# IvanPopov/video-flow-ml

Hardware: AMD Instinct MI355X
Metric: flow-fields/sec @1080p seq5 MOF_sintel (higher is better)
Workload: dtype mixed (per-layer MFMA count, f32 accumulate): {"corr": 1, "update_block.encoder.convf1": 1, "update_block.encoder.convf2": 1, "update_block.gru.convq1.iter": "2a", "update_block.gru.convzr1.iter": 1, "update_block.gru.convzr2.iter": 1, "update_block.mask.0": 1, "update_block.mask.2": 1, "update_bloc

## Files before the change

include/vfml.h:

```cpp
#ifndef VFML_H
#define VFML_H
#include <stddef.h>
#include <stdint.h>

#ifdef __cplusplus
extern "C" {
#endif

#define VFML_ABI_VERSION 27

enum {
  VFML_EPI_NONE = 0,
  VFML_EPI_RELU = 1,
  VFML_EPI_TANH = 2,
  VFML_EPI_SIGMOID = 3,
  VFML_EPI_TANH_RELU = 4,
  VFML_EPI_GRU_ZR = 5,
  VFML_EPI_GRU_Q = 6,
  VFML_EPI_ADD_AUX = 7,
};

enum { VFML_FMT_F32 = 0, VFML_FMT_S16 = 1,
       VFML_FMT_F16 = 2 };

typedef struct vfml_conv_desc {
  const float* in0; int32_t c0; int32_t ld0;
  const float* in1; int32_t c1; int32_t ld1;
  int32_t n, h, w;
  const float* weight;
  const float* bias;
  int32_t cout, kh, kw, stride, pad_h, pad_w;
  float* out; int32_t ldo;
  int32_t epilogue; int32_t split; float out_scale;
  const float* aux0; int32_t ld_aux0;
  const float* aux1; int32_t ld_aux1;
  const float* addend; int32_t ld_addend;
  float* out_t; int32_t ld_out_t;
  int32_t flags;
  double* stats_part;
  float* ksplit_ws;
  const void* proj_hi; const void* proj_lo; int32_t proj_n; int32_t proj_kp; float proj_scale;
  float* proj_out; int32_t ld_proj;
  const float* const* addend_ind;
} vfml_conv_desc;

enum { VFML_STATS_ROWS_F32 = 128, VFML_STATS_ROWS_S16 = 32 };
enum { VFML_CONV_SWAP_CROSS = 1,
       VFML_CONV_MFMA2 = 2, VFML_CONV_MFMA1 = 4, VFML_CONV_MFMA2A = 8,
       VFML_CONV_PER_TAP = 16 };

int vfml_conv2d(const vfml_conv_desc* d, void* stream);

int vfml_conv2d_variant(const vfml_conv_desc* d, char* buf, int len);
int vfml_conv2d_split_variant(const vfml_conv_desc* d, const void* w_hi, const void* w_lo, int kp, float w_scale,
                              int in_fmt, int out_fmt, int aux_fmt, int k_order, char* buf, int len);
int vfml_conv2d_split_variant_at(int index, char* buf, int len);

int vfml_conv2d_split(const vfml_conv_desc* d, const void* w_hi, const void* w_lo, int kp, float w_scale,
                      int in_fmt, int out_fmt, int aux_fmt, int k_order, void* stream);
enum { VFML_KORDER_TAP = 0, VFML_KORDER_CBLOCK = 1, VFML_KORDER_CBLOCK64 = 2 };

int vfml_to_s16(const float* src, int64_t rows, int c, int ld_src, float* dst, int ld_dst, float scale, void* stream);

int vfml_split_f16(const float* src, int64_t rows, int k, int ld, float scale, void* hi, void* lo, int kp,
                   void* stream);

int vfml_softmax_rows_s16(const float* x, int64_t rows, int cols, int64_t ld_in, float* out, int64_t ld_out, float scale,
                          void* stream);

int vfml_softmax_rows_f16(const float* x, int64_t rows, int cols, int64_t ld_in, void* out, int64_t ld_out, float scale,
                          void* stream);

int64_t vfml_attention_plane_workspace_bytes(int p);
int vfml_attention_plane_f16(const float* q, int64_t ld_q, const float* k, int64_t ld_k, int p, int d, float score_scale,
                             float prob_scale, void* plane, int64_t ld_plane, void* workspace, void* stream);

int vfml_attention_bank_planes_f16(const float* q, int64_t ld_q, const float* const* keys, int64_t ld_k, int n_seg, int p, int d,
                                   float score_scale, float prob_scale, void* const* planes, int64_t ld_plane, void* workspace,
                                   void* stream);

int vfml_axpy_f32(const float* x, float* y, int64_t n, float scale, void* stream);

int vfml_transpose_to_s16(const float* src, int rows, int c, int ld, float scale, float* dst, int64_t ld_dst, void* stream);

enum { VFML_DW_RESIDUAL = 1, VFML_DW_GELU = 2 };
int vfml_dwconv2d(const float* x, int64_t ld_x, int n, int h, int w, int c, int k, const float* weight, const float* bias,
                  float* out, int64_t ld_out, int in_fmt, int out_fmt, int flags, void* stream);

int vfml_gelu_rows(const float* x, int64_t ld_x, float* out, int64_t ld_out, int64_t rows, int c, int in_fmt, int out_fmt,
                   void* stream);

int vfml_layernorm_rows(const float* x, int64_t ld_x, float* out, int64_t ld_out, int64_t rows, int c, const float* gamma,
                        const float* beta, float eps, int in_fmt, int out_fmt, void* stream);

int vfml_window_attention(const float* qkv, int64_t ld, int n, int h, int w, int c, int heads, int ws, const float* pad_row,
                          float* out, int64_t ld_out, int in_fmt, int out_fmt, void* stream);

int vfml_attention_shared_keys(const float* q, int64_t ld_q, const float* kv, int64_t ld_kv, int n, int p, int pk, int c, int heads,
                               float* out, int64_t ld_out, int q_fmt, int kv_fmt, int out_fmt, void* stream);

int vfml_add_to_s16(const float* x, int64_t ldx, const float* aux, int64_t ld_aux, float* out, int64_t ld_out, int64_t rows,
                    int c, float scale, void* stream);

int vfml_transpose_split_f16(const float* src, int rows, int c, int ld, float scale, void* hi, void* lo, int kp,
                             void* stream);

int vfml_frames_to_nhwc4(const void* src, int kind, int n, int H, int W,
                         float scale, float shift, float* dst, void* stream);

int64_t vfml_instnorm_workspace_bytes(int n, int hw, int c);
int vfml_instnorm_stats(const float* x, int n, int hw, int c, float eps,
                        float* stats, void* workspace, void* stream);
int vfml_instnorm_apply(const float* x, const float* stats, const float* res,
                        const float* res_stats, int n, int hw, int c, float* out, int out_fmt, void* stream);

int vfml_avgpool2x2(const float* x, int n, int h, int w, int c, float* out, void* stream);

int vfml_corr_lookup(const float* const* pyr, const int32_t* hl, const int32_t* wl,
                     const int32_t* ld, int levels, int radius, int nmaps, int q_per_map,
                     const float* coords, int ld_coords, float* out, int ld_out, int out_fmt, int vol_fmt, int vol_tile,
                     void* stream);
#define VFML_VOL_F16_LEVELS(m) (0x100 | (m))

int vfml_corr_lookup_indirect(const float* const* table, const int32_t* hl, const int32_t* wl, const int32_t* ld,
                              int levels, int radius, int nmaps, int q_per_map, const float* coords, int ld_coords,
                              float* out, int ld_out, int out_fmt, int vol_fmt, int vol_tile, void* stream);
int vfml_corr_lookup_indirect_bidir(const float* const* table, const int32_t* hl, const int32_t* wl, const int32_t* ld,
                                    int levels, int radius, int nmaps, int q_per_map, const float* coords, int ld_coords,
                                    int dir_coords, float* out, int ld_out, int dir_out, int dir_tab, int out_fmt, int vol_fmt,
                                    int vol_tile, void* stream);
int vfml_ptr_table_set(void* table, const void* const* ptrs, int n, void* stream);

int vfml_corr_level0_ensure(const vfml_conv_desc* d, const void* w_hi, const void* w_lo, int kp, float w_scale, int in_fmt,
                            int out_fmt, int k_order, const void* const* cells, int centres, int dirs, int dir_cells,
                            const float* coords, int ld_coords, int dir_coords, int h, int w, int radius, int vol_tile,
                            uint32_t* counter, void* stream);

#define VFML_SEED_NONE 0
#define VFML_SEED_LOAD 1
#define VFML_SEED_STORE 2
int vfml_window_seed(const void* cells, int ncentres, int rows, int cols, float* state, int ld_state, int h_off, int mf_off,
                     int ld_ctx, void* stream);

int vfml_flow_rows7(const float* flow, int n, int h, int w, float* rows, void* stream);

int vfml_conv3x3_c64(const float* in, int ld_in, int n, int h, int w, const void* w_hi, const void* w_lo, int kp, float w_scale,
                     const float* bias, float* out, int ldo, double* stats_part, void* stream);

int vfml_flow_half(const float* flow, int n, int h, int w, const void* w1_hi, int kp1, float w1_scale, const float* b1,
                   const void* w2_hi, int kp2, float w2_scale, const float* b2, float* out, int ld_out, void* stream);

int vfml_tapsum3x3(const float* t, int ld_t, const float* bias, int n, int h, int w, float* out, int parts, int64_t part_stride,
                   void* stream);
int vfml_tapsum3x3_update(const float* t, int ld_t, const float* bias, int n, int h, int w, int parts, int64_t part_stride,
                          float* coords1, float* flow_a, int ld_a, float* flow_b, int ld_b, int fmt_b, void* stream);

int vfml_coords_update(float* coords1, const float* delta, int n, int h, int w,
                       float* flow_a, int ld_a, float* flow_b, int ld_b, int fmt_b, void* stream);

int64_t vfml_flow_forward_interpolate_workspace_bytes(int n, int h, int w);
int vfml_flow_forward_interpolate(const float* flow, int ld_in, int n, int h, int w, float* out, int ld_out, int32_t* index,
                                  void* workspace, int64_t workspace_bytes, void* stream);
int vfml_coords_init(float* coords1, int n, int h, int w, void* stream);

int vfml_convex_upsample(const float* coords1, int ch, const float* mask, int ld_mask,
                         int h, int w, float* out, void* stream);

int64_t vfml_instnorm_finalize_workspace_bytes(int chunks, int c);
int vfml_instnorm_finalize(const double* part, int n, int chunks, int c, int hw, float eps, float* stats,
                           void* workspace, int64_t workspace_bytes, void* stream);

int vfml_stem7x7s2_chunks(int h, int w);
int vfml_stem7x7s2(const float* frames, int n, int h, int w, const void* w_hi, const void* w_lo, float w_scale,
                   const float* bias, float* out, double* stats_part, void* stream);

int vfml_flow_lod(const float* flow, int h, int w, float* out, void* stream);

enum { VFML_ENCODE_GAMEDEV = 0, VFML_ENCODE_RG8 = 1, VFML_ENCODE_RGB8 = 2 };
int vfml_flow_encode(const float* flow, int h, int w, int mode, float width, float height, float scale,
                     float clamp, float two_clamp, unsigned char* out, void* stream);

enum { VFML_TAA_SIMPLE = 0, VFML_TAA_BILINEAR = 1, VFML_TAA_BILATERAL = 2 };
enum { VFML_PIX_U8 = 0, VFML_PIX_F32 = 1, VFML_PIX_F64 = 2 };
int vfml_taa_blend(const void* current, int cur_type, const float* flow, const void* history, int hist_type,
                   void* out, int out_type, int h, int w, int mode, double alpha, double sigma_color, void* stream);

int vfml_flow_quality_map(const unsigned char* frame1, const unsigned char* frame2, const float* flow, int fh, int fw,
                          int h, int w, float threshold, unsigned char* out, void* stream);

#define VFML_CORRECT_RECORD 16
size_t vfml_flow_correct_workspace_bytes(int h, int w);
int vfml_flow_correct(const unsigned char* frame1, const unsigned char* frame2, const float* flow, const float* lod,
                      int lh, int lw, int h, int w, const double* twiddles, double good_threshold,
                      double fine_threshold, double region_radius, double template_radius, double search_radius,
                      float* out_flow, int* counts, double* records, int64_t record_capacity, void* workspace,
                      size_t workspace_bytes, void* stream);

enum { VFML_COLORIZE_HSV = 0, VFML_COLORIZE_WHEEL = 1 };
int vfml_flow_colorize(const float* flow, int h, int w, int mode, void* workspace, unsigned char* out, void* stream);

int vfml_flow_decode(const unsigned char* encoded, int h, int w, int mode, float clamp, float* flow, void* stream);

int vfml_flow_diff_overlay(const float* flow_a, const float* flow_b, int h, int w, unsigned char* out, void* stream);

enum { VFML_COMPOSE_SIDE_BY_SIDE = 0, VFML_COMPOSE_STACKED = 1, VFML_COMPOSE_GRID_2X2 = 2,
       VFML_COMPOSE_GRID_2X3 = 3 };
enum { VFML_COMPOSE_BGR = 1, VFML_COMPOSE_BOTTOM_UP = 2 };
int vfml_compose_frame(const void* const* tiles, const int* tile_types, int h, int w, int layout, int flags,
                       int64_t row_stride, unsigned char* out, void* stream);

int vfml_text_draw(const int32_t* plan, int plan_words, unsigned char* img, int h, int w, int64_t row_stride, int flags,
                   void* stream);

size_t vfml_flow_turbulence_workspace_bytes(int h, int w);
int vfml_flow_turbulence_map(const float* flow, int fh, int fw, int h, int w, int ksize, void* workspace,
                             unsigned char* out_bgr, unsigned char* out_index, float* out_tv, float* out_lohi,
                             void* stream);

int vfml_resize_u8(const unsigned char* src, int n, int H, int W, int64_t src_frame_stride, unsigned char* dst, int h,
                   int w, int64_t dst_frame_stride, const int32_t* xtab, const int32_t* ytab, void* stream);

int64_t vfml_jpeg_workspace_bytes(int h, int w);
int64_t vfml_jpeg_scan_capacity(int h, int w);
int vfml_jpeg_encode_rgb(const unsigned char* rgb, int h, int w, int64_t row_stride, const unsigned char* qtables,
                         void* workspace, unsigned char* scan, int64_t scan_capacity, uint32_t* scan_bytes, void* stream);

enum {
  VFML_JPEG_ERR_INTERVALS = 1,
  VFML_JPEG_ERR_SEQUENCE = 2,
  VFML_JPEG_ERR_CODE = 4,
  VFML_JPEG_ERR_INDEX = 8,
  VFML_JPEG_ERR_DATA = 16
};
int64_t vfml_jpeg_decode_workspace_bytes(int h, int w, int64_t scan_bytes);
int vfml_jpeg_decode_rgb(const unsigned char* scan, int64_t scan_bytes, int h, int w, int restart_interval,
                         const unsigned char* qtables, const int32_t* tables, int y0, int y1, void* workspace,
                         unsigned char* rgb, int64_t row_stride, int32_t* status, void* stream);

int64_t vfml_jpeg_decode_sync_workspace_bytes(int h, int w, int64_t scan_bytes, int subseq_bytes);
int vfml_jpeg_decode_rgb_sync(const unsigned char* scan, int64_t scan_bytes, int h, int w, int restart_interval,
                              const unsigned char* qtables, const int32_t* tables, int y0, int y1, int subseq_bytes,
                              void* workspace, unsigned char* rgb, int64_t row_stride, int32_t* status, void* stream);

enum { VFML_JPEG_420 = 0, VFML_JPEG_422 = 1, VFML_JPEG_444 = 2, VFML_JPEG_GREY = 3 };
int64_t vfml_jpeg_decode_sampled_workspace_bytes(int h, int w, int sampling, int64_t scan_bytes);
int vfml_jpeg_decode_rgb_sampled(const unsigned char* scan, int64_t scan_bytes, int h, int w, int sampling,
                                 int restart_interval, const unsigned char* qtables, const int32_t* tables, int y0, int y1,
                                 void* workspace, unsigned char* rgb, int64_t row_stride, int32_t* status, void* stream);
int64_t vfml_jpeg_decode_sync_sampled_workspace_bytes(int h, int w, int sampling, int64_t scan_bytes, int subseq_bytes);
int vfml_jpeg_decode_rgb_sync_sampled(const unsigned char* scan, int64_t scan_bytes, int h, int w, int sampling,
                                      int restart_interval, const unsigned char* qtables, const int32_t* tables, int y0,
                                      int y1, int subseq_bytes, void* workspace, unsigned char* rgb, int64_t row_stride,
                                      int32_t* status, void* stream);

int64_t vfml_jpeg_sampled_workspace_bytes(int h, int w, int sampling);
int64_t vfml_jpeg_sampled_scan_capacity(int h, int w, int sampling);
int vfml_jpeg_encode_rgb_sampled(const unsigned char* rgb, int h, int w, int64_t row_stride, int sampling,
                                 const unsigned char* qtables, void* workspace, unsigned char* scan,
                                 int64_t scan_capacity, uint32_t* scan_bytes, void* stream);

int64_t vfml_deflate_capacity(int64_t raw_bytes, int chunk_bytes);
int64_t vfml_deflate_workspace_bytes(int64_t raw_bytes, int chunk_bytes);
int vfml_deflate_huffman(const unsigned char* raw, int64_t raw_bytes, int chunk_bytes, uint32_t crc_init, void* workspace,
                         unsigned char* out, int64_t capacity, uint32_t* offsets, uint32_t* stream_bytes, uint32_t* crc,
                         void* stream);

enum {
  VFML_INFLATE_ERR_CODE = 1,
  VFML_INFLATE_ERR_MATCH = 2,
  VFML_INFLATE_ERR_LENGTH = 4,
  VFML_INFLATE_ERR_BITS = 8,
  VFML_INFLATE_ERR_STORED = 16,
  VFML_INFLATE_ERR_CHUNK = 32
};
int64_t vfml_inflate_workspace_bytes(int64_t raw_bytes, int chunk_bytes);
int vfml_inflate_chunks(const unsigned char* data, int64_t data_bytes, const uint32_t* offsets, int n_chunks, int chunk_bytes,
                        int64_t raw_bytes, uint32_t crc_init, void* workspace, unsigned char* raw, uint32_t* crc,
                        int32_t* status, void* stream);

const char* vfml_last_error(void);
int vfml_abi_version(void);

#ifdef __cplusplus
}
#endif
#endif
```

video-flow-ml_amd/vfml/csrc/corr_ensure.hip:

```cpp
#include "gemm_resident_walk.h"
#include "corr_window.h"

namespace {

constexpr int ENSURE_MASK_WORDS = 64;

struct EnsureArgs {
  SplitArgs g;
  const void* const* cells;
  const float* coords;
  unsigned* counter;
  int ld_coords, dir_coords;
  int centres, dirs, dir_cells;
  int q_per_map;
  int h, w, radius, tws, ths;
  int wpr;
};

struct MaskCols {
  unsigned v;
  int nw;
  __device__ __forceinline__ unsigned word(int w) const {
    return (unsigned)__builtin_amdgcn_readlane((int)v, __builtin_amdgcn_readfirstlane(w));
  }
  __device__ __forceinline__ int from(int at) const {
    int w = at >> 5;
    if (w >= nw) return -1;
    unsigned m = word(w) & (~0u << (at & 31));
    while (!m) {
      if (++w >= nw) return -1;
      m = word(w);
    }
    return w * 32 + __builtin_ctz(m);
  }
  __device__ __forceinline__ int first() const { return from(0); }
  __device__ __forceinline__ int next(int nt) const { return from(nt + 1); }
};

__device__ __forceinline__ const void* uniform_cell(const void* const* cell) {
  const uint64_t v = reinterpret_cast<uint64_t>(*cell);
  const unsigned lo = (unsigned)__builtin_amdgcn_readfirstlane((int)(unsigned)v);
  const unsigned hi = (unsigned)__builtin_amdgcn_readfirstlane((int)(unsigned)(v >> 32));
  return reinterpret_cast<const void*>(((uint64_t)hi << 32) | lo);
}

typedef __attribute__((address_space(1))) unsigned* gu32ptr;
typedef const __attribute__((address_space(1))) float* gf32cptr;

__global__ __launch_bounds__(256, 2) void corr_ensure_kernel(const EnsureArgs e) {
  extern __shared__ __attribute__((aligned(16))) char smem[];
  unsigned* mask = reinterpret_cast<unsigned*>(smem);
  const int t = threadIdx.x, lane = t & 63;
  const int mtiles = e.g.mtiles;
  const int units = e.centres * e.dirs * mtiles;
  const int tsh = e.tws + e.ths;
  const int tpr = (e.w + (1 << e.tws) - 1) >> e.tws;
  const int side = 2 * e.radius + 2;
  for (int u = blockIdx.x; u < units; u += gridDim.x) {
    const int k = u / mtiles, mt = u - k * mtiles;
    const int dir = k / e.centres, c = k - dir * e.centres;
    const void* const* cell = e.cells + (dir * e.dir_cells + c) * 4;
    const gu32ptr bitmap = (gu32ptr)uniform_cell(cell + 3) + mt * e.wpr;
    lds_barrier();
    if (t < ENSURE_MASK_WORDS) mask[t] = 0u;
    lds_barrier();
    if (t < 128) {
      const int row = mt * 128 + t;
      const int tile = row >> tsh, in = row & ((1 << tsh) - 1);
      const int ty = tile / tpr, tx = tile - ty * tpr;
      const int y = (ty << e.ths) + (in >> e.tws), x = (tx << e.tws) + (in & ((1 << e.tws) - 1));
      if (row < e.g.M && y < e.h && x < e.w) {
        const gf32cptr cr = (gf32cptr)e.coords + ((int64_t)c * e.q_per_map + y * e.w + x) * e.ld_coords + dir * e.dir_coords;
        const int x0 = window_origin(cr[0], e.radius);
        const int y0 = window_origin(cr[1], e.radius);
        const int xlo = max(x0, 0), xhi = min(x0 + side - 1, e.w - 1);
        const int ylo = max(y0, 0), yhi = min(y0 + side - 1, e.h - 1);
        if (xlo <= xhi && ylo <= yhi) {
          for (int yy = ylo; yy <= yhi; yy = ((yy >> e.ths) + 1) << e.ths)
            for (int xx = xlo; xx <= xhi; xx = ((xx >> e.tws) + 1) << e.tws) {
              const int ct = tiled_at(yy, xx, e.w, e.tws, e.ths) >> 6;
              atomicOr(&mask[ct >> 5], 1u << (ct & 31));
            }
        }
      }
    }
    lds_barrier();
    if (t < e.wpr) mask[t] &= ~bitmap[t];
    lds_barrier();
    const unsigned need = lane < e.wpr ? mask[lane] : 0u;
    const MaskCols cols{need, e.wpr};
    int cnt = 0;
    for (int w = 0; w < e.wpr; ++w) cnt += __builtin_popcount(cols.word(w));
    if (cnt == 0) continue;

    SplitArgs a = e.g;
    a.in0 = a.in1 = reinterpret_cast<const float*>(uniform_cell(cell));
    a.wbase = reinterpret_cast<const char*>(uniform_cell(cell + 1));
    a.out = reinterpret_cast<float*>(const_cast<void*>(uniform_cell(cell + 2)));
    gemm_resident_unit<false, false>(a, smem, mt, cols);

    asm volatile("s_waitcnt vmcnt(0)" ::: "memory");
    lds_barrier();
    if (t < e.wpr && need) atomicOr((unsigned*)bitmap + t, need);
    if (t == 0 && e.counter) atomicAdd(e.counter, (unsigned)cnt);
  }
}

}

extern "C" int vfml_corr_level0_ensure(const vfml_conv_desc* d, const void* w_hi, const void* w_lo, int kp, float w_scale,
                                       int in_fmt, int out_fmt, int k_order, const void* const* cells, int centres, int dirs,
                                       int dir_cells, const float* coords, int ld_coords, int dir_coords, int h, int w,
                                       int radius, int vol_tile, uint32_t* counter, void* stream) {
  const char* who = "vfml_corr_level0_ensure";
  VFML_REQUIRE(d && cells && coords, "%s: null desc / cells / coords", who);
  EnsureArgs e;
  if (const int rc = vfml_detail::prepare_resident_gemm(d, w_hi, w_lo, kp, w_scale, in_fmt, out_fmt, k_order, who, &e.g)) return rc;
  const SplitArgs& a = e.g;
  VFML_REQUIRE(!a.bias && !a.out_t && a.epilogue == VFML_EPI_NONE && a.whi_off == 0 && a.d0off == 0 && a.tilebase,
               "%s: the level-0 call has no bias, twin or activation, its hi plane leads its planes and its rows are one "
               "split-row source", who);
  e.tws = vol_tile & 15;
  e.ths = vol_tile >> 4;
  VFML_REQUIRE(vol_tile >= 0 && e.ths <= 6 && e.tws + e.ths <= 6, "%s: vol_tile: tiles of at most 64 texels", who);
  VFML_REQUIRE(h > 0 && w > 0 && radius >= 1 && radius <= 4, "%s: empty level image, or radius outside 1..4", who);
  const int64_t tiled = (int64_t)(((h - 1) >> e.ths) + 1) * (((w - 1) >> e.tws) + 1) << (e.tws + e.ths);
  VFML_REQUIRE(tiled == a.M && tiled == a.cout, "%s: the call's rows (%d) and columns (%d) must be the %lld positions of the "
               "tiled %d x %d level image", who, a.M, a.cout, (long long)tiled, h, w);
  e.wpr = (a.ntiles + 31) / 32;
  VFML_REQUIRE(e.wpr <= ENSURE_MASK_WORDS, "%s: at most %d column tiles per volume row", who, ENSURE_MASK_WORDS * 32);
  VFML_REQUIRE(centres >= 1 && (dirs == 1 || dirs == 2) && dir_cells >= (dirs == 2 ? centres : 0) && ld_coords >= 2 &&
               dir_coords >= 0, "%s: centres >= 1, one or two directions, the second direction's cells behind the first's", who);
  VFML_REQUIRE((reinterpret_cast<uintptr_t>(cells) & 7u) == 0 && (!counter || (reinterpret_cast<uintptr_t>(counter) & 3u) == 0),
               "%s: cells are 8-byte aligned, the counter 4-byte", who);
  e.cells = cells; e.coords = coords; e.counter = counter;
  e.ld_coords = ld_coords; e.dir_coords = dir_coords;
  e.centres = centres; e.dirs = dirs; e.dir_cells = dir_cells;
  e.q_per_map = h * w; e.h = h; e.w = w; e.radius = radius;
  if (const int rc = vfml_lds_cap(reinterpret_cast<const void*>(&corr_ensure_kernel), VFML_RESIDENT_LDS, who)) return rc;
  const int64_t units = (int64_t)centres * dirs * a.mtiles;
  hipLaunchKernelGGL(corr_ensure_kernel, dim3((int)(units > 512 ? 512 : units)), dim3(256), VFML_RESIDENT_LDS,
                     reinterpret_cast<hipStream_t>(stream), e);
  return vfml_check_launch(who);
}
```

video-flow-ml_amd/vfml/csrc/corr_window.h:

```cpp
#pragma once
#include "vfml_common.h"

namespace {

__device__ __forceinline__ int tiled_at(int y, int x, int w, int tws, int ths) {
  const int tpr = (w + (1 << tws) - 1) >> tws;
  return ((((y >> ths) * tpr + (x >> tws)) << (tws + ths)) + ((y & ((1 << ths) - 1)) << tws) + (x & ((1 << tws) - 1)));
}

__device__ __forceinline__ int window_origin(float c, int radius) {
  return (int)fminf(fmaxf(floorf(c), -65536.f), 65536.f) - radius;
}

}
```

video-flow-ml_amd/vfml/csrc/flow_ops.hip:

```cpp
#include <stdlib.h>
#include "vfml_common.h"
#include "corr_window.h"

namespace {

constexpr int MAX_LEVELS = 6;
constexpr int MAX_MAPS = 8;
constexpr int MAX_RADIUS = 4;
constexpr int PATCH = 2 * MAX_RADIUS + 2;
#ifndef VFML_LOOKUP_WAVES
#define VFML_LOOKUP_WAVES 4
#endif
constexpr int LOOKUP_WAVES = VFML_LOOKUP_WAVES;
constexpr int FIXED_LEVELS = 4;
static_assert(FIXED_LEVELS == 4, "corr_lookup_fixed_kernel selects among four levels");

struct LookupArgs {
  const float* pyr[MAX_MAPS][MAX_LEVELS];
  const float* const* table;
  int hl[MAX_LEVELS], wl[MAX_LEVELS], ld[MAX_LEVELS];
  int levels, radius, nq, q_per_map;
  const float* coords; int ld_coords;
  float* out; int ld_out;
  int out16;
  int vol16;
  int tws, ths;
  int qw;
  int dir_maps, dir_coords, dir_out;
  int dir_tab;
};

__device__ __forceinline__ void lookup_rows(const LookupArgs& a, int q, int& map, int64_t& crow, int64_t& orow) {
  const int dir = a.dir_maps && map >= a.dir_maps;
  const int64_t qd = q - (dir ? a.dir_maps * a.q_per_map : 0);
  if (dir) map += a.dir_tab - a.dir_maps;
  crow = qd * a.ld_coords + (dir ? a.dir_coords : 0);
  orow = qd * a.ld_out + (dir ? a.dir_out : 0);
}


__device__ __forceinline__ float bilinear4(float nw, float ne, float sw, float se, float wx0, float fx, float wy0, float fy) {
  float v = ne * (fx * wy0);
  v = __builtin_fmaf(nw, wx0 * wy0, v);
  v = __builtin_fmaf(sw, wx0 * fy, v);
  v = __builtin_fmaf(se, fx * fy, v);
  return v;
}

__global__ __launch_bounds__(64 * LOOKUP_WAVES) void corr_lookup_kernel(const LookupArgs a) {
  __shared__ float patch[LOOKUP_WAVES][MAX_LEVELS][PATCH * PATCH];
  __shared__ float frac[LOOKUP_WAVES][MAX_LEVELS][2];
  const int lane = threadIdx.x & 63;
  const int wv = threadIdx.x >> 6;
  const int q = blockIdx.x * LOOKUP_WAVES + wv;
  const bool live = q < a.nq;
  int map = live ? q / a.q_per_map : 0;
  const int qq = q - map * a.q_per_map;
  const int side = 2 * a.radius + 2;
  const int win = 2 * a.radius + 1;
  const int psz = side * side;
  int64_t crow = 0, orow = 0;
  if (live) lookup_rows(a, q, map, crow, orow);
  if (live) {
    const float cx = a.coords[crow + 0];
    const float cy = a.coords[crow + 1];
    const int total = a.levels * psz;
    const int qrow = (a.tws | a.ths) ? tiled_at(qq / a.qw, qq % a.qw, a.qw, a.tws, a.ths) : qq;
    for (int e = lane; e < total; e += 64) {
      const int l = e / psz;
      const int idx = e - l * psz;
      const int py = idx / side, px = idx - py * side;
      const float inv = 1.0f / (float)(1 << l);
      const float x = cx * inv, y = cy * inv;
      const float fx0 = floorf(x), fy0 = floorf(y);
      const int x0 = window_origin(x, a.radius);
      const int y0 = window_origin(y, a.radius);
      const int xx = x0 + px, yy = y0 + py;
      float v = 0.f;
      if (xx >= 0 && xx < a.wl[l] && yy >= 0 && yy < a.hl[l])
        v = (a.table ? a.table[map * a.levels + l] : a.pyr[map][l])[(int64_t)qrow * a.ld[l] + tiled_at(yy, xx, a.wl[l], a.tws, a.ths)];
      patch[wv][l][idx] = v;
      if (idx == 0) {
        frac[wv][l][0] = x - fx0;
        frac[wv][l][1] = y - fy0;
      }
    }
  }
  __syncthreads();
  if (!live) return;
  const int nout = a.levels * win * win;
  float* o = a.out + orow;
  const int nwrite = a.out16 ? (nout + 7) & ~7 : nout;
  for (int c = lane; c < nwrite; c += 64) {
    if (c >= nout) {
      _Float16* u = reinterpret_cast<_Float16*>(o + (c & ~7));
      u[c & 7] = (_Float16)0.f;
      u[8 + (c & 7)] = (_Float16)0.f;
      continue;
    }
    const int l = c / (win * win);
    const int rem = c - l * win * win;
    const int i = rem / win, j = rem - i * win;
    const float fx = frac[wv][l][0], fy = frac[wv][l][1];
    const float* p = &patch[wv][l][j * side + i];
    const float wx0 = 1.f - fx, wy0 = 1.f - fy;
    const float v = bilinear4(p[0], p[1], p[side], p[side + 1], wx0, fx, wy0, fy);
    if (a.out16) {
      vfml_h16x2 hh, ll;
      vfml_split2(v, 0.f, hh, ll);
      _Float16* u = reinterpret_cast<_Float16*>(o + (c & ~7));
      u[c & 7] = hh[0];
      u[8 + (c & 7)] = ll[0];
    } else {
      o[c] = v;
    }
  }
}

__device__ __forceinline__ float bilinear4w(float nw, float ne, float sw, float se, float w00, float w10, float w01, float w11) {
  float v = ne * w10;
  v = __builtin_fmaf(nw, w00, v);
  v = __builtin_fmaf(sw, w01, v);
  v = __builtin_fmaf(se, w11, v);
  return v;
}

__device__ __forceinline__ void wave_lds_sync() {
  __builtin_amdgcn_fence(__ATOMIC_RELEASE, "workgroup");
  __builtin_amdgcn_wave_barrier();
  __builtin_amdgcn_fence(__ATOMIC_ACQUIRE, "workgroup");
}

template <int R, bool OUT16, int V16 = 0>
__global__ __launch_bounds__(64 * LOOKUP_WAVES) void corr_lookup_fixed_kernel(const LookupArgs a) {
  constexpr int SIDE = 2 * R + 2, PSZ = SIDE * SIDE, WIN = 2 * R + 1, WW = WIN * WIN;
  constexpr int NOUTPAD = (FIXED_LEVELS * WW + 7) & ~7;
  static_assert(PSZ <= 128 && FIXED_LEVELS * WIN <= 64 && NOUTPAD / 8 <= 64, "one wave: at most two gather passes per level");
  __shared__ float patch[LOOKUP_WAVES][FIXED_LEVELS][PSZ];
  __shared__ __attribute__((aligned(16))) float outs[LOOKUP_WAVES][NOUTPAD];
  const int lane = threadIdx.x & 63;
  const int wv = __builtin_amdgcn_readfirstlane(threadIdx.x >> 6);
  const int q = blockIdx.x * LOOKUP_WAVES + wv;
  if (q >= a.nq) return;
  int map = __builtin_amdgcn_readfirstlane(q / a.q_per_map);
  const int qq = q - map * a.q_per_map;
  const int qrow = __builtin_amdgcn_readfirstlane((a.tws | a.ths) ? tiled_at(qq / a.qw, qq % a.qw, a.qw, a.tws, a.ths) : qq);
  int64_t crow, orow;
  lookup_rows(a, q, map, crow, orow);
  const float cx = a.coords[crow + 0];
  const float cy = a.coords[crow + 1];
  const int pyA = lane / SIDE, pxA = lane - pyA * SIDE;
  const int pyB = (lane + 64) / SIDE, pxB = (lane + 64) - pyB * SIDE;
  const bool inB = lane + 64 < PSZ;
  const float* pl[FIXED_LEVELS];
  if (a.table) {
#pragma unroll
    for (int l = 0; l < FIXED_LEVELS; ++l) pl[l] = a.table[map * a.levels + (l < a.levels ? l : 0)];
  } else {
#pragma unroll
    for (int l = 0; l < FIXED_LEVELS; ++l) pl[l] = a.pyr[map][l < a.levels ? l : 0];
  }
  float va[FIXED_LEVELS], vb[FIXED_LEVELS];
  bool oka[FIXED_LEVELS], okb[FIXED_LEVELS];
#pragma unroll
  for (int l = 0; l < FIXED_LEVELS; ++l) {
    const bool have = l < a.levels;
    const int ll = have ? l : 0;
    const bool v16 = (V16 >> l) & 1;
    const int ES = v16 ? 2 : 4;
    const char* base = reinterpret_cast<const char*>(pl[l]) + (int64_t)qrow * a.ld[ll] * ES;
    const int wl = a.wl[ll], hl = a.hl[ll];
    const float inv = __builtin_bit_cast(float, (127 - l) << 23);
    const float x = cx * inv, y = cy * inv;
    const int x0 = window_origin(x, R);
    const int y0 = window_origin(y, R);
    auto texel = [&](int px, int py, bool in, float& out, bool& ok) {
      const int xx = x0 + px, yy = y0 + py;
      ok = have && in && xx >= 0 && xx < wl && yy >= 0 && yy < hl;
      const int at = tiled_at(min(max(yy, 0), hl - 1), min(max(xx, 0), wl - 1), wl, a.tws, a.ths);
      if (v16) out = (float)((const __attribute__((address_space(1))) _Float16*)base)[at];
      else out = ((const __attribute__((address_space(1))) float*)base)[at];
    };
    texel(pxA, pyA, true, va[l], oka[l]);
    if constexpr (PSZ > 64) texel(pxB, pyB, inB, vb[l], okb[l]);
    else { vb[l] = 0.f; okb[l] = false; }
  }
#pragma unroll
  for (int l = 0; l < FIXED_LEVELS; ++l) {
    va[l] = oka[l] ? va[l] : 0.f;
    vb[l] = okb[l] ? vb[l] : 0.f;
  }
#pragma unroll
  for (int l = 0; l < FIXED_LEVELS; ++l) {
    if (l < a.levels) {
      if (PSZ > 64 || lane < PSZ) patch[wv][l][lane] = va[l];
      if constexpr (PSZ > 64) if (inB) patch[wv][l][lane + 64] = vb[l];
    }
  }
  const int nout = a.levels * WW;
  const int nunits = (nout + 7) >> 3;
  if (lane >= 56 && nout + (lane - 56) < nunits * 8) outs[wv][nout + (lane - 56)] = 0.f;
  wave_lds_sync();
  if (lane < a.levels * WIN) {
    const int l = lane / WIN, i = lane - l * WIN;
    const float inv = __builtin_bit_cast(float, (127 - l) << 23);
    const float x = cx * inv, y = cy * inv;
    const float fx = x - floorf(x), fy = y - floorf(y);
    const float wx0 = 1.f - fx, wy0 = 1.f - fy;
    const float w00 = wx0 * wy0, w10 = fx * wy0, w01 = wx0 * fy, w11 = fx * fy;
    const float* p = &patch[wv][l][i];
    float* o = &outs[wv][l * WW + i * WIN];
    float nw = p[0], ne = p[1];
#pragma unroll
    for (int j = 0; j < WIN; ++j) {
      const float sw = p[(j + 1) * SIDE], se = p[(j + 1) * SIDE + 1];
      o[j] = bilinear4w(nw, ne, sw, se, w00, w10, w01, w11);
      nw = sw; ne = se;
    }
  }
  wave_lds_sync();
  if (lane < nunits) {
    float* o = a.out + orow + lane * 8;
    const f32x4 v0 = *reinterpret_cast<const f32x4*>(&outs[wv][lane * 8]);
    const f32x4 v1 = *reinterpret_cast<const f32x4*>(&outs[wv][lane * 8 + 4]);
    if (OUT16) {
      vfml_h16x2 h0, h1, h2, h3, l0, l1, l2, l3;
      vfml_split2(v0[0], v0[1], h0, l0);
      vfml_split2(v0[2], v0[3], h1, l1);
      vfml_split2(v1[0], v1[1], h2, l2);
      vfml_split2(v1[2], v1[3], h3, l3);
      uint4 hv, lv;
      hv.x = __builtin_bit_cast(unsigned, h0); hv.y = __builtin_bit_cast(unsigned, h1);
      hv.z = __builtin_bit_cast(unsigned, h2); hv.w = __builtin_bit_cast(unsigned, h3);
      lv.x = __builtin_bit_cast(unsigned, l0); lv.y = __builtin_bit_cast(unsigned, l1);
      lv.z = __builtin_bit_cast(unsigned, l2); lv.w = __builtin_bit_cast(unsigned, l3);
      *reinterpret_cast<uint4*>(o) = hv;
      *reinterpret_cast<uint4*>(o + 4) = lv;
    } else {
#pragma unroll
      for (int h = 0; h < 2; ++h) {
        const int c = lane * 8 + 4 * h;
        const f32x4 w = h ? v1 : v0;
        if (c + 3 < nout && (((uintptr_t)(o + 4 * h)) & 15u) == 0) {
          *reinterpret_cast<f32x4*>(o + 4 * h) = w;
        } else {
#pragma unroll
          for (int k = 0; k < 4; ++k)
            if (c + k < nout) o[4 * h + k] = w[k];
        }
      }
    }
  }
}

__global__ void coords_init_kernel(f32x4* __restrict__ coords, int h, int w, int64_t total) {
  for (int64_t p = (int64_t)blockIdx.x * blockDim.x + threadIdx.x; p < total; p += (int64_t)gridDim.x * blockDim.x) {
    const int x = (int)(p % w);
    const int y = (int)((p / w) % h);
    f32x4 v = {(float)x, (float)y, (float)x, (float)y};
    coords[p] = v;
  }
}

__global__ void flow_rows7_kernel(const f32x4* __restrict__ flow, int w, int64_t total, char* __restrict__ rows) {
  for (int64_t i = (int64_t)blockIdx.x * blockDim.x + threadIdx.x; i < total * 4; i += (int64_t)gridDim.x * blockDim.x) {
    const int64_t p = i >> 2;
    const int u = (int)(i & 3);
    const int x = (int)(p % w);
    f32x4 t0 = {0.f, 0.f, 0.f, 0.f}, t1 = {0.f, 0.f, 0.f, 0.f};
    const int x0 = x + 2 * u - 3, x1 = x0 + 1;
    if (x0 >= 0 && x0 < w) t0 = flow[p + 2 * u - 3];
    if (u < 3 && x1 >= 0 && x1 < w) t1 = flow[p + 2 * u - 2];
    vfml_h16x2 h[4], l[4];
    vfml_split2(t0[0], t0[1], h[0], l[0]);
    vfml_split2(t0[2], t0[3], h[1], l[1]);
    vfml_split2(t1[0], t1[1], h[2], l[2]);
    vfml_split2(t1[2], t1[3], h[3], l[3]);
    uint4 hv, lv;
    hv.x = __builtin_bit_cast(unsigned, h[0]); hv.y = __builtin_bit_cast(unsigned, h[1]);
    hv.z = __builtin_bit_cast(unsigned, h[2]); hv.w = __builtin_bit_cast(unsigned, h[3]);
    lv.x = __builtin_bit_cast(unsigned, l[0]); lv.y = __builtin_bit_cast(unsigned, l[1]);
    lv.z = __builtin_bit_cast(unsigned, l[2]); lv.w = __builtin_bit_cast(unsigned, l[3]);
    char* o = rows + p * 128 + u * 32;
    *reinterpret_cast<uint4*>(o) = hv;
    *reinterpret_cast<uint4*>(o + 16) = lv;
  }
}

__device__ __forceinline__ void emit_flow(int64_t p, const f32x4 c, int h, int w, float* __restrict__ fa, int lda,
                                          float* __restrict__ fb, int ldb, int b16) {
  const float x = (float)(int)(p % w);
  const float y = (float)(int)((p / w) % h);
  const f32x4 f = {c[0] - x, c[1] - y, c[2] - x, c[3] - y};
  if (fa) *reinterpret_cast<f32x4*>(fa + p * lda) = f;
  if (fb) {
    if (b16) {
      typedef vfml_h16x2 fp16x2_;
      fp16x2_ h0, h1, l0, l1;
      vfml_split2(f[0], f[1], h0, l0);
      vfml_split2(f[2], f[3], h1, l1);
      char* u = reinterpret_cast<char*>(fb + p * ldb) - 16;
      *reinterpret_cast<fp16x2_*>(u + 8) = h0;
      *reinterpret_cast<fp16x2_*>(u + 12) = h1;
      *reinterpret_cast<fp16x2_*>(u + 24) = l0;
      *reinterpret_cast<fp16x2_*>(u + 28) = l1;
    } else {
      *reinterpret_cast<f32x4*>(fb + p * ldb) = f;
    }
  }
}

__global__ void tapsum3x3_kernel(const float* __restrict__ t, int ld, const float* __restrict__ bias, int h, int w,
                                 int64_t total, f32x4* __restrict__ out, int parts, int64_t part_stride,
                                 f32x4* __restrict__ coords, float* __restrict__ fa, int lda, float* __restrict__ fb, int ldb,
                                 int b16) {
  for (int64_t p = (int64_t)blockIdx.x * blockDim.x + threadIdx.x; p < total; p += (int64_t)gridDim.x * blockDim.x) {
    const int x = (int)(p % w), y = (int)((p / w) % h);
    f32x4 s = {0.f, 0.f, 0.f, 0.f};
    if (bias) s = f32x4{bias[0], bias[1], bias[2], bias[3]};
#pragma unroll
    for (int ky = 0; ky < 3; ++ky)
#pragma unroll
      for (int kx = 0; kx < 3; ++kx) {
        const int yy = y + ky - 1, xx = x + kx - 1;
        if (yy >= 0 && yy < h && xx >= 0 && xx < w) {
          const float* q = t + (p + (int64_t)(ky - 1) * w + (kx - 1)) * ld + (ky * 3 + kx) * 4;
          f32x4 v = *reinterpret_cast<const f32x4*>(q);
          for (int k = 1; k < parts; ++k) v = v + *reinterpret_cast<const f32x4*>(q + k * part_stride);
          s = s + v;
        }
      }
    if (out) out[p] = s;
    if (coords) {
      const f32x4 c = coords[p] + s;
      coords[p] = c;
      emit_flow(p, c, h, w, fa, lda, fb, ldb, b16);
    }
  }
}

__global__ void coords_update_kernel(f32x4* __restrict__ coords, const f32x4* __restrict__ delta, int h, int w,
                                     int64_t total, float* __restrict__ fa, int lda, float* __restrict__ fb, int ldb,
                                     int b16) {
  for (int64_t p = (int64_t)blockIdx.x * blockDim.x + threadIdx.x; p < total; p += (int64_t)gridDim.x * blockDim.x) {
    f32x4 c = coords[p];
    if (delta) {
      c = c + delta[p];
      coords[p] = c;
    }
    emit_flow(p, c, h, w, fa, lda, fb, ldb, b16);
  }
}

__global__ __launch_bounds__(256) void convex_upsample_kernel(const float* __restrict__ coords, int ch,
                                                             const float* __restrict__ mask, int ld_mask, int h,
                                                             int w, float* __restrict__ out) {
  const int lane = threadIdx.x & 63;
  const int p = blockIdx.x * 4 + (threadIdx.x >> 6);
  if (p >= h * w) return;
  const int y = p / w, x = p - y * w;
  const float* m = mask + (int64_t)p * ld_mask + lane;
  float logit[9], fxv[9], fyv[9];
  float mx = -INFINITY;
#pragma unroll
  for (int k = 0; k < 9; ++k) {
    logit[k] = m[k * 64];
    mx = fmaxf(mx, logit[k]);
    const int yy = y + k / 3 - 1, xx = x + k % 3 - 1;
    float u = 0.f, v = 0.f;
    if (yy >= 0 && yy < h && xx >= 0 && xx < w) {
      const float* c = coords + ((int64_t)yy * w + xx) * 4 + ch;
      u = 8.f * (c[0] - (float)xx);
      v = 8.f * (c[1] - (float)yy);
    }
    fxv[k] = u;
    fyv[k] = v;
  }
  float s = 0.f;
#pragma unroll
  for (int k = 0; k < 9; ++k) {
    logit[k] = expf(logit[k] - mx);
    s += logit[k];
  }
  float ax = 0.f, ay = 0.f;
#pragma unroll
  for (int k = 0; k < 9; ++k) {
    const float pk = logit[k] / s;
    ax += pk * fxv[k];
    ay += pk * fyv[k];
  }
  const int sy = lane >> 3, sx = lane & 7;
  float2* o = reinterpret_cast<float2*>(out) + ((int64_t)(8 * y + sy) * (8 * w) + 8 * x + sx);
  *o = make_float2(ax, ay);
}

__global__ void flow_lod_kernel(const float2* __restrict__ flow, int h, int w, int ho, int wo, float2* __restrict__ out) {
  for (int64_t i = (int64_t)blockIdx.x * blockDim.x + threadIdx.x; i < (int64_t)ho * wo;
       i += (int64_t)gridDim.x * blockDim.x) {
    const int oy = (int)(i / wo), ox = (int)(i - (int64_t)oy * wo);
    const int y0 = 2 * oy, x0 = 2 * ox;
    const bool y1 = y0 + 1 < h, x1 = x0 + 1 < w;
    const float2 a = flow[(int64_t)y0 * w + x0];
    const float2 b = x1 ? flow[(int64_t)y0 * w + x0 + 1] : make_float2(0.f, 0.f);
    const float2 c = y1 ? flow[(int64_t)(y0 + 1) * w + x0] : make_float2(0.f, 0.f);
    const float2 d = (y1 && x1) ? flow[(int64_t)(y0 + 1) * w + x0 + 1] : make_float2(0.f, 0.f);
    const float wt = ((1.f + (x1 ? 1.f : 0.f)) + (y1 ? 1.f : 0.f)) + ((y1 && x1) ? 1.f : 0.f);
    const float sx = ((a.x + b.x) + c.x) + d.x, sy = ((a.y + b.y) + c.y) + d.y;
    out[i] = make_float2(sx / wt * 0.5f, sy / wt * 0.5f);
  }
}

inline int grid_for(int64_t items, int block) {
  int64_t g = (items + block - 1) / block;
  return (int)(g < 1 ? 1 : (g > 8192 ? 8192 : g));
}

constexpr int MAX_TABLE = MAX_MAPS * MAX_LEVELS;
struct PtrTable { const void* p[MAX_TABLE]; };
__global__ void ptr_table_kernel(const PtrTable t, int n, const void** dst) {
  if ((int)threadIdx.x < n) dst[threadIdx.x] = t.p[threadIdx.x];
}

__global__ void window_seed_kernel(const int64_t* __restrict__ cells, int rows, int quads, float* __restrict__ state,
                                   int ld_state, int h_off, int mf_off, int ld_ctx) {
  const int c = blockIdx.y;
  const float* ctx = reinterpret_cast<const float*>(cells[3 * c]);
  float* slot = reinterpret_cast<float*>(cells[3 * c + 1]);
  const int64_t mode = slot ? cells[3 * c + 2] : 0;
  const int total = rows * quads;
  for (int i = blockIdx.x * blockDim.x + threadIdx.x; i < total; i += gridDim.x * blockDim.x) {
    const int r = i / quads, k = 4 * (i - r * quads);
    float* srow = state + ((int64_t)c * rows + r) * ld_state;
    if (ctx) *reinterpret_cast<f32x4*>(srow + h_off + k) = *reinterpret_cast<const f32x4*>(ctx + (int64_t)r * ld_ctx + k);
    if (mode == VFML_SEED_LOAD)
      *reinterpret_cast<f32x4*>(srow + mf_off + k) = *reinterpret_cast<const f32x4*>(slot + (int64_t)r * 4 * quads + k);
    else if (mode == VFML_SEED_STORE)
      *reinterpret_cast<f32x4*>(slot + (int64_t)r * 4 * quads + k) = *reinterpret_cast<const f32x4*>(srow + mf_off + k);
  }
}

}

extern "C" int vfml_ptr_table_set(void* table, const void* const* ptrs, int n, void* stream) {
  VFML_REQUIRE(table && ptrs && n >= 1 && n <= MAX_TABLE, "vfml_ptr_table_set: 1..%d pointers", MAX_TABLE);
  PtrTable t;
  for (int i = 0; i < MAX_TABLE; ++i) t.p[i] = i < n ? ptrs[i] : nullptr;
  hipLaunchKernelGGL(ptr_table_kernel, dim3(1), dim3(64), 0, reinterpret_cast<hipStream_t>(stream), t, n,
                     reinterpret_cast<const void**>(table));
  return vfml_check_launch("vfml_ptr_table_set");
}

extern "C" int vfml_window_seed(const void* cells, int ncentres, int rows, int cols, float* state, int ld_state, int h_off,
                                int mf_off, int ld_ctx, void* stream) {
  VFML_REQUIRE(cells && (reinterpret_cast<uintptr_t>(cells) & 7u) == 0, "vfml_window_seed: null / misaligned cells");
  VFML_REQUIRE(ncentres >= 1 && 3 * ncentres <= MAX_TABLE, "vfml_window_seed: ncentres=%d out of [1,%d]", ncentres, MAX_TABLE / 3);
  VFML_REQUIRE(state && vfml_aligned16(state), "vfml_window_seed: null / misaligned state");
  VFML_REQUIRE(rows >= 1 && cols >= 4 && cols % 4 == 0 && (int64_t)rows * (cols / 4) <= (1 << 30),
               "vfml_window_seed: rows >= 1, cols a multiple of 4, rows * cols / 4 <= 2^30");
  VFML_REQUIRE(ld_state % 4 == 0 && h_off >= 0 && mf_off >= 0 && h_off % 4 == 0 && mf_off % 4 == 0 && h_off + cols <= ld_state &&
               mf_off + cols <= ld_state && (h_off + cols <= mf_off || mf_off + cols <= h_off),
               "vfml_window_seed: the two column blocks lie apart inside a state row, at multiples of 4 floats");
  VFML_REQUIRE(ld_ctx >= cols && ld_ctx % 4 == 0, "vfml_window_seed: ld_ctx=%d (>= cols, a multiple of 4)", ld_ctx);
  const int quads = cols / 4;
  hipLaunchKernelGGL(window_seed_kernel, dim3(grid_for((int64_t)rows * quads, 256), ncentres), dim3(256), 0,
                     reinterpret_cast<hipStream_t>(stream), reinterpret_cast<const int64_t*>(cells), rows, quads, state,
                     ld_state, h_off, mf_off, ld_ctx);
  return vfml_check_launch("vfml_window_seed");
}

static int corr_lookup_impl(const float* const* pyr, const float* const* table, const int32_t* hl, const int32_t* wl,
                            const int32_t* ld, int levels, int radius, int nmaps, int q_per_map, const float* coords,
                            int ld_coords, float* out, int ld_out, int out_fmt, int vol_fmt, int vol_tile, void* stream,
                            int dir_maps = 0, int dir_coords = 0, int dir_out = 0, int dir_tab = 0);

extern "C" int vfml_corr_lookup(const float* const* pyr, const int32_t* hl, const int32_t* wl, const int32_t* ld,
                                int levels, int radius, int nmaps, int q_per_map, const float* coords, int ld_coords,
                                float* out, int ld_out, int out_fmt, int vol_fmt, int vol_tile, void* stream) {
  VFML_REQUIRE(pyr, "vfml_corr_lookup: null pointer");
  return corr_lookup_impl(pyr, nullptr, hl, wl, ld, levels, radius, nmaps, q_per_map, coords, ld_coords, out, ld_out, out_fmt,
                          vol_fmt, vol_tile, stream);
}

extern "C" int vfml_corr_lookup_indirect(const float* const* table, const int32_t* hl, const int32_t* wl, const int32_t* ld,
                                         int levels, int radius, int nmaps, int q_per_map, const float* coords,
                                         int ld_coords, float* out, int ld_out, int out_fmt, int vol_fmt, int vol_tile, void* stream) {
  VFML_REQUIRE(table && (reinterpret_cast<uintptr_t>(table) & 7u) == 0, "vfml_corr_lookup_indirect: null / misaligned table");
  return corr_lookup_impl(nullptr, table, hl, wl, ld, levels, radius, nmaps, q_per_map, coords, ld_coords, out, ld_out,
                          out_fmt, vol_fmt, vol_tile, stream);
}

extern "C" int vfml_corr_lookup_indirect_bidir(const float* const* table, const int32_t* hl, const int32_t* wl, const int32_t* ld,
                                               int levels, int radius, int nmaps, int q_per_map, const float* coords,
                                               int ld_coords, int dir_coords, float* out, int ld_out, int dir_out, int dir_tab,
                                               int out_fmt, int vol_fmt, int vol_tile, void* stream) {
  VFML_REQUIRE(table && (reinterpret_cast<uintptr_t>(table) & 7u) == 0, "vfml_corr_lookup_indirect_bidir: null / misaligned table");
  VFML_REQUIRE(nmaps >= 1 && 2 * nmaps <= MAX_MAPS, "vfml_corr_lookup_indirect_bidir: nmaps=%d out of [1,%d]", nmaps, MAX_MAPS / 2);
  VFML_REQUIRE(dir_coords >= 0 && dir_coords + 2 <= ld_coords && dir_out >= 0 && (out_fmt != VFML_FMT_S16 || dir_out % 8 == 0),
               "vfml_corr_lookup_indirect_bidir: dir_coords within a coords row, dir_out >= 0 (a multiple of 8 floats for split rows)");
  VFML_REQUIRE(dir_tab >= nmaps && (dir_tab + nmaps) * levels <= MAX_TABLE,
               "vfml_corr_lookup_indirect_bidir: dir_tab=%d (the second direction's first map in the table) out of range", dir_tab);
  return corr_lookup_impl(nullptr, table, hl, wl, ld, levels, radius, 2 * nmaps, q_per_map, coords, ld_coords, out, ld_out,
                          out_fmt, vol_fmt, vol_tile, stream, nmaps, dir_coords, dir_out, dir_tab);
}

static int corr_lookup_impl(const float* const* pyr, const float* const* table, const int32_t* hl, const int32_t* wl,
                            const int32_t* ld, int levels, int radius, int nmaps, int q_per_map, const float* coords,
                            int ld_coords, float* out, int ld_out, int out_fmt, int vol_fmt, int vol_tile, void* stream,
                            int dir_maps, int dir_coords, int dir_out, int dir_tab) {
  VFML_REQUIRE(nmaps >= 1 && nmaps <= MAX_MAPS && q_per_map > 0, "vfml_corr_lookup: nmaps=%d out of [1,%d] or empty maps", nmaps, MAX_MAPS);
// ... 232 lines not shown
```

video-flow-ml_amd/vfml/hip.py:

```python
import ctypes
import os
import subprocess
from ctypes import POINTER, c_char_p, c_double, c_float, c_int, c_int32, c_int64, c_void_p

import torch

_HERE = os.path.dirname(os.path.abspath(__file__))
LIB_PATH = os.environ.get("VFML_LIB") or os.path.join(_HERE, "libvfml_hip.so")
CSRC = os.path.join(_HERE, "csrc")
SOURCES = ["api.hip", "conv_gemm.hip", "conv_gemm_split.hip", "corr_ensure.hip", "conv_gemm_tapx.hip", "conv_split_plan.hip", "stem.hip", "flow_half.hip", "enc_conv.hip", "norm_pool.hip", "flow_ops.hip", "effects.hip", "correct.hip", "render.hip", "text.hip", "turbulence.hip", "resize.hip", "jpeg.hip", "jpeg_decode.hip", "jpeg_decode_sync.hip", "deflate.hip", "attention.hip", "dwconv.hip", "twins.hip", "warm_start.hip"]

STATS_ROWS_F32, STATS_ROWS_S16 = 128, 32
EPI_NONE, EPI_RELU, EPI_TANH, EPI_SIGMOID, EPI_TANH_RELU, EPI_GRU_ZR, EPI_GRU_Q, EPI_ADD_AUX = range(8)
FMT_F32, FMT_S16, FMT_F16 = 0, 1, 2


def vol_f16_levels(mask):
    return 0x100 | mask


def _vol_mask(vol_fmt, levels):
    return (15 if vol_fmt == FMT_F16 else (vol_fmt & 15 if vol_fmt & 0x100 else 0)) & ((1 << levels) - 1)

KORDER_TAP, KORDER_CBLOCK, KORDER_CBLOCK64 = 0, 1, 2
CONV_SWAP_CROSS, CONV_MFMA2, CONV_MFMA1, CONV_MFMA2A, CONV_PER_TAP = 1, 2, 4, 8, 16


class ConvDesc(ctypes.Structure):
    _fields_ = [
        ("in0", c_void_p), ("c0", c_int32), ("ld0", c_int32),
        ("in1", c_void_p), ("c1", c_int32), ("ld1", c_int32),
        ("n", c_int32), ("h", c_int32), ("w", c_int32),
        ("weight", c_void_p), ("bias", c_void_p),
        ("cout", c_int32), ("kh", c_int32), ("kw", c_int32), ("stride", c_int32),
        ("pad_h", c_int32), ("pad_w", c_int32),
        ("out", c_void_p), ("ldo", c_int32),
        ("epilogue", c_int32), ("split", c_int32), ("out_scale", c_float),
        ("aux0", c_void_p), ("ld_aux0", c_int32),
        ("aux1", c_void_p), ("ld_aux1", c_int32),
        ("addend", c_void_p), ("ld_addend", c_int32),
        ("out_t", c_void_p), ("ld_out_t", c_int32),
        ("flags", c_int32),
        ("stats_part", c_void_p),
        ("ksplit_ws", c_void_p),
        ("proj_hi", c_void_p), ("proj_lo", c_void_p), ("proj_n", c_int32), ("proj_kp", c_int32), ("proj_scale", c_float),
        ("proj_out", c_void_p), ("ld_proj", c_int32),
        ("addend_ind", c_void_p),
    ]


COMMON_FLAGS = ["-fno-slp-vectorize"]
EXTRA_FLAGS = {}


def build(force=False, verbose=False):
    srcs = [os.path.join(CSRC, s) for s in SOURCES]
    hdrs = [os.path.join(CSRC, "vfml_common.h"), os.path.join(CSRC, "conv_split_common.h"),
            os.path.join(CSRC, "gemm_resident_walk.h"), os.path.join(CSRC, "corr_window.h"),
            os.path.join(CSRC, "jet_table.inc"), os.path.join(CSRC, "jpeg_tables.inc"), os.path.join(CSRC, "jpeg_decode_common.h"),
            os.path.join(CSRC, "jpeg_sync_steps.h"), os.path.join(CSRC, "deflate_code.h"), os.path.join(_HERE, "..", "..", "include", "vfml.h")]
    deps = srcs + hdrs
    if not force and os.path.exists(LIB_PATH) and all(
            os.path.getmtime(LIB_PATH) >= os.path.getmtime(d) for d in deps):
        return LIB_PATH
    objdir = os.path.join(CSRC, "_obj")
    os.makedirs(objdir, exist_ok=True)
    newest_hdr = max(os.path.getmtime(h) for h in hdrs)
    jobs = []
    for src in srcs:
        obj = os.path.join(objdir, os.path.basename(src) + ".o")
        if force or not os.path.exists(obj) or os.path.getmtime(obj) < max(os.path.getmtime(src), newest_hdr):
            cmd = ["hipcc", "--offload-arch=gfx950", "-O3", "-std=c++17", "-fPIC"] + COMMON_FLAGS + EXTRA_FLAGS.get(os.path.basename(src), []) + [
                "-c", src, "-o", obj]
            if verbose:
                print(" ".join(cmd))
            jobs.append((cmd, subprocess.Popen(cmd)))
    for cmd, p in jobs:
        if p.wait() != 0:
            raise subprocess.CalledProcessError(p.returncode, cmd)
    cmd = ["hipcc", "--offload-arch=gfx950", "-fPIC", "-shared", "-o", LIB_PATH] + [
        os.path.join(objdir, os.path.basename(src) + ".o") for src in srcs]
    if verbose:
        print(" ".join(cmd))
    subprocess.run(cmd, check=True)
    return LIB_PATH


_lib = None


def lib():
    global _lib
    if _lib is not None:
        return _lib
    if not os.path.exists(LIB_PATH):
        raise RuntimeError(
            f"vfml HIP extension not built: {LIB_PATH} is missing. Run `python -c 'import __graft_entry__ as g; "
            f"g.build()'` (needs hipcc). There is no CPU fallback for the flow engine.")
    L = ctypes.CDLL(LIB_PATH)
    L.vfml_last_error.restype = c_char_p
    L.vfml_abi_version.restype = c_int
    L.vfml_conv2d.argtypes = [POINTER(ConvDesc), c_void_p]
    L.vfml_conv2d_split.argtypes = [POINTER(ConvDesc), c_void_p, c_void_p, c_int, c_float, c_int, c_int, c_int, c_int,
                                    c_void_p]
    L.vfml_conv2d_variant.argtypes = [POINTER(ConvDesc), c_char_p, c_int]
    L.vfml_conv2d_split_variant.argtypes = L.vfml_conv2d_split.argtypes[:-1] + [c_char_p, c_int]
    L.vfml_conv2d_split_variant_at.argtypes = [c_int, c_char_p, c_int]
    L.vfml_to_s16.argtypes = [c_void_p, c_int64, c_int, c_int, c_void_p, c_int, c_float, c_void_p]
    L.vfml_softmax_rows_s16.argtypes = [c_void_p, c_int64, c_int, c_int64, c_void_p, c_int64, c_float, c_void_p]
    L.vfml_transpose_split_f16.argtypes = [c_void_p, c_int, c_int, c_int, c_float, c_void_p, c_void_p, c_int, c_void_p]
    L.vfml_split_f16.argtypes = [c_void_p, c_int64, c_int, c_int, c_float, c_void_p, c_void_p, c_int, c_void_p]
    L.vfml_frames_to_nhwc4.argtypes = [c_void_p, c_int, c_int, c_int, c_int, c_float, c_float, c_void_p, c_void_p]
    L.vfml_instnorm_workspace_bytes.restype = c_int64
    L.vfml_instnorm_workspace_bytes.argtypes = [c_int, c_int, c_int]
    L.vfml_instnorm_stats.argtypes = [c_void_p, c_int, c_int, c_int, c_float, c_void_p, c_void_p, c_void_p]
    L.vfml_softmax_rows_f16.argtypes = [c_void_p, c_int64, c_int, c_int64, c_void_p, c_int64, c_float, c_void_p]
    L.vfml_attention_plane_workspace_bytes.restype = c_int64
    L.vfml_attention_plane_workspace_bytes.argtypes = [c_int]
    L.vfml_attention_plane_f16.argtypes = [c_void_p, c_int64, c_void_p, c_int64, c_int, c_int, c_float, c_float, c_void_p, c_int64,
                                           c_void_p, c_void_p]
    L.vfml_attention_bank_planes_f16.argtypes = [c_void_p, c_int64, POINTER(c_void_p), c_int64, c_int, c_int, c_int, c_float, c_float,
                                                 POINTER(c_void_p), c_int64, c_void_p, c_void_p]
    L.vfml_axpy_f32.argtypes = [c_void_p, c_void_p, c_int64, c_float, c_void_p]
    L.vfml_dwconv2d.argtypes = [c_void_p, c_int64, c_int, c_int, c_int, c_int, c_int, c_void_p, c_void_p, c_void_p, c_int64, c_int, c_int,
                                c_int, c_void_p]
    L.vfml_gelu_rows.argtypes = [c_void_p, c_int64, c_void_p, c_int64, c_int64, c_int, c_int, c_int, c_void_p]
    L.vfml_layernorm_rows.argtypes = [c_void_p, c_int64, c_void_p, c_int64, c_int64, c_int, c_void_p, c_void_p, c_float, c_int, c_int,
                                      c_void_p]
    L.vfml_window_attention.argtypes = [c_void_p, c_int64, c_int, c_int, c_int, c_int, c_int, c_int, c_void_p, c_void_p, c_int64,
                                        c_int, c_int, c_void_p]
    L.vfml_attention_shared_keys.argtypes = [c_void_p, c_int64, c_void_p, c_int64, c_int, c_int, c_int, c_int, c_int, c_void_p,
                                             c_int64, c_int, c_int, c_int, c_void_p]
    L.vfml_transpose_to_s16.argtypes = [c_void_p, c_int, c_int, c_int, c_float, c_void_p, c_int64, c_void_p]
    L.vfml_add_to_s16.argtypes = [c_void_p, c_int64, c_void_p, c_int64, c_void_p, c_int64, c_int64, c_int, c_float, c_void_p]
    L.vfml_instnorm_finalize.argtypes = [c_void_p, c_int, c_int, c_int, c_int, c_float, c_void_p, c_void_p, c_int64, c_void_p]
    L.vfml_instnorm_finalize_workspace_bytes.restype = c_int64
    L.vfml_instnorm_finalize_workspace_bytes.argtypes = [c_int, c_int]
    L.vfml_stem7x7s2_chunks.argtypes = [c_int, c_int]
    L.vfml_stem7x7s2.argtypes = [c_void_p, c_int, c_int, c_int, c_void_p, c_void_p, c_float, c_void_p, c_void_p, c_void_p, c_void_p]
    L.vfml_instnorm_apply.argtypes = [c_void_p, c_void_p, c_void_p, c_void_p, c_int, c_int, c_int, c_void_p, c_int, c_void_p]
    L.vfml_avgpool2x2.argtypes = [c_void_p, c_int, c_int, c_int, c_int, c_void_p, c_void_p]
    L.vfml_corr_lookup.argtypes = [POINTER(c_void_p), POINTER(c_int32), POINTER(c_int32), POINTER(c_int32),
                                   c_int, c_int, c_int, c_int, c_void_p, c_int, c_void_p, c_int, c_int, c_int, c_int, c_void_p]
    L.vfml_corr_lookup_indirect.argtypes = [c_void_p, POINTER(c_int32), POINTER(c_int32), POINTER(c_int32),
                                            c_int, c_int, c_int, c_int, c_void_p, c_int, c_void_p, c_int, c_int, c_int, c_int,
                                            c_void_p]
    L.vfml_corr_lookup_indirect_bidir.argtypes = [c_void_p, POINTER(c_int32), POINTER(c_int32), POINTER(c_int32),
                                                  c_int, c_int, c_int, c_int, c_void_p, c_int, c_int, c_void_p, c_int, c_int,
                                                  c_int, c_int, c_int, c_int, c_void_p]
    L.vfml_ptr_table_set.argtypes = [c_void_p, POINTER(c_void_p), c_int, c_void_p]
    L.vfml_corr_level0_ensure.argtypes = L.vfml_conv2d_split.argtypes[:5] + [c_int, c_int, c_int] + [
        c_void_p, c_int, c_int, c_int, c_void_p, c_int, c_int, c_int, c_int, c_int, c_int, c_void_p, c_void_p]
    L.vfml_window_seed.argtypes = [c_void_p, c_int, c_int, c_int, c_void_p, c_int, c_int, c_int, c_int, c_void_p]
    L.vfml_tapsum3x3_update.argtypes = [c_void_p, c_int, c_void_p, c_int, c_int, c_int, c_int, ctypes.c_int64, c_void_p, c_void_p,
                                        c_int, c_void_p, c_int, c_int, c_void_p]
    L.vfml_conv3x3_c64.argtypes = [c_void_p, c_int, c_int, c_int, c_int, c_void_p, c_void_p, c_int, c_float, c_void_p, c_void_p,
                                   c_int, c_void_p, c_void_p]
    L.vfml_flow_half.argtypes = [c_void_p, c_int, c_int, c_int, c_void_p, c_int, c_float, c_void_p, c_void_p, c_int, c_float,
                                 c_void_p, c_void_p, c_int, c_void_p]
    L.vfml_coords_init.argtypes = [c_void_p, c_int, c_int, c_int, c_void_p]
    L.vfml_flow_rows7.argtypes = [c_void_p, c_int, c_int, c_int, c_void_p, c_void_p]
    L.vfml_tapsum3x3.argtypes = [c_void_p, c_int, c_void_p, c_int, c_int, c_int, c_void_p, c_int, ctypes.c_int64, c_void_p]
    L.vfml_coords_update.argtypes = [c_void_p, c_void_p, c_int, c_int, c_int, c_void_p, c_int, c_void_p, c_int,
                                     c_int, c_void_p]
    L.vfml_flow_forward_interpolate_workspace_bytes.restype = c_int64
    L.vfml_flow_forward_interpolate_workspace_bytes.argtypes = [c_int, c_int, c_int]
    L.vfml_flow_forward_interpolate.argtypes = [c_void_p, c_int, c_int, c_int, c_int, c_void_p, c_int, c_void_p, c_void_p, c_int64,
                                                c_void_p]
    L.vfml_flow_lod.argtypes = [c_void_p, c_int, c_int, c_void_p, c_void_p]
    L.vfml_flow_encode.argtypes = [c_void_p, c_int, c_int, c_int, c_float, c_float, c_float, c_float, c_float, c_void_p,
                                   c_void_p]
    L.vfml_taa_blend.argtypes = [c_void_p, c_int, c_void_p, c_void_p, c_int, c_void_p, c_int, c_int, c_int, c_int, c_double,
                                 c_double, c_void_p]
    L.vfml_flow_quality_map.argtypes = [c_void_p, c_void_p, c_void_p, c_int, c_int, c_int, c_int, c_float, c_void_p, c_void_p]
    L.vfml_flow_correct_workspace_bytes.argtypes = [c_int, c_int]
    L.vfml_flow_correct_workspace_bytes.restype = ctypes.c_size_t
    L.vfml_flow_correct.argtypes = [c_void_p, c_void_p, c_void_p, c_void_p, c_int, c_int, c_int, c_int, c_void_p,
                                    c_double, c_double, c_double, c_double, c_double, c_void_p, c_void_p, c_void_p,
                                    ctypes.c_int64, c_void_p, ctypes.c_size_t, c_void_p]
    L.vfml_flow_colorize.argtypes = [c_void_p, c_int, c_int, c_int, c_void_p, c_void_p, c_void_p]
    L.vfml_flow_decode.argtypes = [c_void_p, c_int, c_int, c_int, c_float, c_void_p, c_void_p]
    L.vfml_flow_diff_overlay.argtypes = [c_void_p, c_void_p, c_int, c_int, c_void_p, c_void_p]
    L.vfml_compose_frame.argtypes = [POINTER(c_void_p), POINTER(c_int32), c_int, c_int, c_int, c_int, c_int64, c_void_p,
                                     c_void_p]
    L.vfml_text_draw.argtypes = [c_void_p, c_int, c_void_p, c_int, c_int, c_int64, c_int, c_void_p]
    L.vfml_flow_turbulence_workspace_bytes.argtypes = [c_int, c_int]
    L.vfml_flow_turbulence_workspace_bytes.restype = ctypes.c_size_t
    L.vfml_flow_turbulence_map.argtypes = [c_void_p, c_int, c_int, c_int, c_int, c_int, c_void_p, c_void_p, c_void_p, c_void_p,
                                           c_void_p, c_void_p]
    L.vfml_resize_u8.argtypes = [c_void_p, c_int, c_int, c_int, c_int64, c_void_p, c_int, c_int, c_int64, c_void_p, c_void_p,
                                 c_void_p]
    L.vfml_jpeg_workspace_bytes.restype = c_int64
    L.vfml_jpeg_workspace_bytes.argtypes = [c_int, c_int]
    L.vfml_jpeg_scan_capacity.restype = c_int64
    L.vfml_jpeg_scan_capacity.argtypes = [c_int, c_int]
    L.vfml_jpeg_encode_rgb.argtypes = [c_void_p, c_int, c_int, c_int64, c_void_p, c_void_p, c_void_p, c_int64, c_void_p,
                                       c_void_p]
    L.vfml_jpeg_sampled_workspace_bytes.restype = c_int64
    L.vfml_jpeg_sampled_workspace_bytes.argtypes = [c_int, c_int, c_int]
    L.vfml_jpeg_sampled_scan_capacity.restype = c_int64
    L.vfml_jpeg_sampled_scan_capacity.argtypes = [c_int, c_int, c_int]
    L.vfml_jpeg_encode_rgb_sampled.argtypes = [c_void_p, c_int, c_int, c_int64, c_int, c_void_p, c_void_p, c_void_p, c_int64,
                                               c_void_p, c_void_p]
    L.vfml_jpeg_decode_workspace_bytes.restype = c_int64
    L.vfml_jpeg_decode_workspace_bytes.argtypes = [c_int, c_int, c_int64]
    L.vfml_jpeg_decode_rgb.argtypes = [c_void_p, c_int64, c_int, c_int, c_int, c_void_p, c_void_p, c_int, c_int, c_void_p,
                                       c_void_p, c_int64, c_void_p, c_void_p]
    L.vfml_jpeg_decode_sync_workspace_bytes.restype = c_int64
    L.vfml_jpeg_decode_sync_workspace_bytes.argtypes = [c_int, c_int, c_int64, c_int]
    L.vfml_jpeg_decode_rgb_sync.argtypes = [c_void_p, c_int64, c_int, c_int, c_int, c_void_p, c_void_p, c_int, c_int, c_int,
                                            c_void_p, c_void_p, c_int64, c_void_p, c_void_p]
    L.vfml_jpeg_decode_sampled_workspace_bytes.restype = c_int64
    L.vfml_jpeg_decode_sampled_workspace_bytes.argtypes = [c_int, c_int, c_int, c_int64]
    L.vfml_jpeg_decode_rgb_sampled.argtypes = [c_void_p, c_int64, c_int, c_int, c_int, c_int, c_void_p, c_void_p, c_int, c_int,
                                               c_void_p, c_void_p, c_int64, c_void_p, c_void_p]
    L.vfml_jpeg_decode_sync_sampled_workspace_bytes.restype = c_int64
    L.vfml_jpeg_decode_sync_sampled_workspace_bytes.argtypes = [c_int, c_int, c_int, c_int64, c_int]
    L.vfml_jpeg_decode_rgb_sync_sampled.argtypes = [c_void_p, c_int64, c_int, c_int, c_int, c_int, c_void_p, c_void_p, c_int,
                                                    c_int, c_int, c_void_p, c_void_p, c_int64, c_void_p, c_void_p]
    for fn in (L.vfml_deflate_capacity, L.vfml_deflate_workspace_bytes, L.vfml_inflate_workspace_bytes):
        fn.restype = c_int64
        fn.argtypes = [c_int64, c_int]
    L.vfml_deflate_huffman.argtypes = [c_void_p, c_int64, c_int, ctypes.c_uint32, c_void_p, c_void_p, c_int64, c_void_p, c_void_p,
                                       c_void_p, c_void_p]
    L.vfml_inflate_chunks.argtypes = [c_void_p, c_int64, c_void_p, c_int, c_int, c_int64, ctypes.c_uint32, c_void_p, c_void_p,
                                      c_void_p, c_void_p, c_void_p]
    L.vfml_convex_upsample.argtypes = [c_void_p, c_int, c_void_p, c_int, c_int, c_int, c_void_p, c_void_p]
    for name in EXPORTS:
        getattr(L, name)
    if L.vfml_abi_version() != 27:
        raise RuntimeError("libvfml_hip.so ABI version mismatch")
    _lib = L
    return L


EXPORTS = [
    "vfml_conv2d", "vfml_conv2d_split", "vfml_conv2d_variant", "vfml_conv2d_split_variant", "vfml_conv2d_split_variant_at", "vfml_split_f16", "vfml_to_s16", "vfml_softmax_rows_s16", "vfml_softmax_rows_f16", "vfml_attention_plane_workspace_bytes", "vfml_attention_plane_f16", "vfml_attention_bank_planes_f16", "vfml_axpy_f32", "vfml_dwconv2d", "vfml_gelu_rows", "vfml_layernorm_rows", "vfml_window_attention", "vfml_attention_shared_keys", "vfml_transpose_to_s16", "vfml_add_to_s16",
    "vfml_transpose_split_f16", "vfml_frames_to_nhwc4", "vfml_instnorm_workspace_bytes", "vfml_instnorm_stats",
    "vfml_instnorm_apply", "vfml_instnorm_finalize", "vfml_instnorm_finalize_workspace_bytes", "vfml_avgpool2x2", "vfml_corr_lookup", "vfml_corr_lookup_indirect", "vfml_corr_lookup_indirect_bidir",
    "vfml_ptr_table_set", "vfml_corr_level0_ensure", "vfml_window_seed", "vfml_coords_update", "vfml_coords_init", "vfml_tapsum3x3", "vfml_tapsum3x3_update", "vfml_flow_rows7", "vfml_flow_half", "vfml_conv3x3_c64",
    "vfml_flow_forward_interpolate_workspace_bytes", "vfml_flow_forward_interpolate",
    "vfml_convex_upsample", "vfml_stem7x7s2", "vfml_stem7x7s2_chunks", "vfml_flow_lod", "vfml_flow_encode", "vfml_taa_blend", "vfml_flow_quality_map", "vfml_flow_correct_workspace_bytes", "vfml_flow_correct",
    "vfml_flow_colorize", "vfml_compose_frame", "vfml_flow_decode", "vfml_flow_diff_overlay", "vfml_text_draw",
    "vfml_flow_turbulence_workspace_bytes", "vfml_flow_turbulence_map", "vfml_resize_u8",
    "vfml_jpeg_workspace_bytes", "vfml_jpeg_scan_capacity", "vfml_jpeg_encode_rgb",
    "vfml_jpeg_sampled_workspace_bytes", "vfml_jpeg_sampled_scan_capacity", "vfml_jpeg_encode_rgb_sampled",
    "vfml_jpeg_decode_workspace_bytes", "vfml_jpeg_decode_rgb",
    "vfml_jpeg_decode_sync_workspace_bytes", "vfml_jpeg_decode_rgb_sync",
    "vfml_jpeg_decode_sampled_workspace_bytes", "vfml_jpeg_decode_rgb_sampled",
    "vfml_jpeg_decode_sync_sampled_workspace_bytes", "vfml_jpeg_decode_rgb_sync_sampled",
    "vfml_deflate_capacity", "vfml_deflate_workspace_bytes", "vfml_deflate_huffman",
    "vfml_inflate_workspace_bytes", "vfml_inflate_chunks",
    "vfml_last_error", "vfml_abi_version",
]


def _check(rc, what):
    if rc != 0:
        raise RuntimeError(f"{what} failed (rc={rc}): {lib().vfml_last_error().decode()}")


def _stream():
    return c_void_p(torch.cuda.current_stream().cuda_stream)


def _ptr(t, offset=0):
    if t is None:
        return None
    return c_void_p(t.data_ptr() + 4 * offset)


def _dev(t, dtype=torch.float32):
    if not (t.is_cuda and t.dtype == dtype and t.is_contiguous()):
        raise ValueError(f"expected a contiguous {dtype} device tensor, got {t.dtype} {t.device} "
                         f"contiguous={t.is_contiguous()}")
    return t


_PROFILE = None


_PROFILE_HBM = None


def profile_begin():
    global _PROFILE, _PROFILE_HBM
    _PROFILE = []
    _PROFILE_HBM = []


def profile_end_hbm():
    rec = _PROFILE_HBM or []
    torch.cuda.synchronize()
    out = {}
    for name, nbytes, e0, e1 in rec:
        d = out.setdefault(name, {"launches": 0, "bytes": 0.0, "ms": 0.0})
        d["launches"] += 1
        d["bytes"] += nbytes
        d["ms"] += e0.elapsed_time(e1)
    return out


def profile_end():
    global _PROFILE, _PROFILE_HBM
    rec, _PROFILE = _PROFILE or [], None
    _PROFILE_HBM = None
    torch.cuda.synchronize()
    out = {}
    for variant, flops, nbytes, e0, e1, shape in rec:
        d = out.setdefault(variant, {"launches": 0, "flops": 0.0, "bytes": 0.0, "ms": 0.0, "shapes": {}})
        ms = e0.elapsed_time(e1)
        for t in (d, d["shapes"].setdefault(shape, {"launches": 0, "flops": 0.0, "bytes": 0.0, "ms": 0.0})):
            t["launches"] += 1
            t["flops"] += flops
            t["bytes"] += nbytes
            t["ms"] += ms
    return out


class SplitWeight:

    def __init__(self, rows, k, device):
        self.rows, self.k, self.kp = rows, k, (k + 31) // 32 * 32
        self.scale = 1.0
        self.order = KORDER_TAP
        self.planes = torch.empty(2 * rows * self.kp, dtype=torch.float16, device=device)
        self.hi, self.lo = self.planes[:rows * self.kp], self.planes[rows * self.kp:]

    @staticmethod
    def auto_scale(absmax):
        import math
        if not (absmax > 0.0) or not math.isfinite(absmax):
            return 1.0
        return 2.0 ** math.floor(math.log2(16384.0 / absmax))

    def fill_transposed(self, src, rows_src, ld=None, scale=1.0, src_off=0):
        self.scale = float(scale)
        _check(lib().vfml_transpose_split_f16(_ptr(_dev(src), src_off), rows_src, self.rows, ld or self.rows,
                                              self.scale, c_void_p(self.hi.data_ptr()), c_void_p(self.lo.data_ptr()),
                                              self.kp, _stream()), "vfml_transpose_split_f16")
        return self

    def fill(self, src, src_off=0, ld=None, scale=1.0):
        self.scale = float(scale)
        _check(lib().vfml_split_f16(_ptr(_dev(src), src_off), self.rows, self.k, ld or self.k, self.scale,
                                    c_void_p(self.hi.data_ptr()), c_void_p(self.lo.data_ptr()), self.kp, _stream()),
               "vfml_split_f16")
        return self


def conv2d(in0, c0, ld0, n, h, w, weight, bias, cout, kh, kw, out, ldo, *, stride=1, pad_h=0, pad_w=0,
           in0_off=0, weight_off=0, in1=None, c1=0, ld1=0, in1_off=0, out_off=0, epilogue=EPI_NONE, split=0, out_scale=1.0,
           aux0=None, ld_aux0=0, aux0_off=0, aux1=None, ld_aux1=0, aux1_off=0,
           in_fmt=FMT_F32, out_fmt=FMT_F32, aux_fmt=FMT_F32, addend=None, ld_addend=0, addend_off=0,
           out_t=None, ld_out_t=0, out_t_off=0, swap_cross=False, stats_part=None, mfma=3, per_tap=False, ksplit_ws=None,
           proj=None, proj_out=None, ld_proj=0, addend_ind=None, variant_only=False):
    d = ConvDesc()
    d.in0, d.c0, d.ld0 = _ptr(_dev(in0), in0_off), c0, ld0
    d.in1, d.c1, d.ld1 = (_ptr(_dev(in1), in1_off) if in1 is not None else None), c1, ld1
    d.n, d.h, d.w = n, h, w
    is_split = isinstance(weight, (SplitWeight, PlainWeight))
    d.weight = None if is_split else _ptr(_dev(weight), weight_off)
    d.bias = _ptr(_dev(bias)) if bias is not None else None
    d.cout, d.kh, d.kw, d.stride, d.pad_h, d.pad_w = cout, kh, kw, stride, pad_h, pad_w
    d.out, d.ldo = _ptr(_dev(out), out_off), ldo
    d.epilogue, d.split, d.out_scale = epilogue, split, out_scale
    d.aux0, d.ld_aux0 = (_ptr(_dev(aux0), aux0_off) if aux0 is not None else None), ld_aux0
    d.aux1, d.ld_aux1 = (_ptr(_dev(aux1), aux1_off) if aux1 is not None else None), ld_aux1
    d.addend, d.ld_addend = (_ptr(_dev(addend), addend_off) if addend is not None else None), ld_addend
    d.out_t, d.ld_out_t = (_ptr(_dev(out_t), out_t_off) if out_t is not None else None), ld_out_t
    if mfma == "2w":
        mfma = 2
    if mfma not in (1, 2, 3, "2a") or (swap_cross and mfma != 3):
        raise ValueError(f"mfma={mfma!r}: 1, 2 ('2w'), '2a' or 3 (3 with swap_cross)")
    d.flags = (CONV_SWAP_CROSS if swap_cross else 0) | {3: 0, 2: CONV_MFMA2, "2a": CONV_MFMA2A, 1: CONV_MFMA1}[mfma] | (CONV_PER_TAP if per_tap else 0)
    d.stats_part = c_void_p(stats_part.data_ptr()) if stats_part is not None else None
    d.ksplit_ws = _ptr(_dev(ksplit_ws)) if ksplit_ws is not None else None
    if addend_ind is not None:
        tab, ent = addend_ind
        d.addend_ind = c_void_p(tab.data_ptr() + 8 * ent)
    if proj is not None:
        if not isinstance(proj, SplitWeight) or proj.lo is None or proj_out is None:
            raise ValueError("proj: a SplitWeight with both planes, and proj_out")
        d.proj_hi, d.proj_lo = c_void_p(proj.hi.data_ptr()), c_void_p(proj.lo.data_ptr())
        d.proj_n, d.proj_kp, d.proj_scale = proj.rows, proj.kp, proj.scale
        d.proj_out, d.ld_proj = _ptr(_dev(proj_out)), ld_proj
    if is_split:
        wargs = (c_void_p(weight.hi.data_ptr() + 2 * weight_off * weight.kp),
                 c_void_p(weight.lo.data_ptr() + 2 * weight_off * weight.kp) if weight.lo is not None else None, weight.kp,
                 weight.scale, in_fmt, out_fmt, aux_fmt, weight.order)

        def launch():
            _check(lib().vfml_conv2d_split(ctypes.byref(d), *wargs, _stream()), "vfml_conv2d_split")

        def variant():
            buf = ctypes.create_string_buffer(160)
            _check(lib().vfml_conv2d_split_variant(ctypes.byref(d), *wargs, buf, len(buf)), "vfml_conv2d_split_variant")
            return buf.value.decode()
    else:
        if in_fmt != FMT_F32 or out_fmt != FMT_F32 or aux_fmt != FMT_F32:
            raise ValueError("the exact-f32 kernel (vfml_conv2d) takes and writes plain f32 activations only")

        def launch():
            _check(lib().vfml_conv2d(ctypes.byref(d), _stream()), "vfml_conv2d")

        def variant():
            buf = ctypes.create_string_buffer(160)
            _check(lib().vfml_conv2d_variant(ctypes.byref(d), buf, len(buf)), "vfml_conv2d_variant")
            return buf.value.decode()
    if variant_only:
        return variant()
    if _PROFILE is None:
        launch()
        return
    ho = (h + 2 * pad_h - kh) // stride + 1
    wo = (w + 2 * pad_w - kw) // stride + 1
    e0, e1 = torch.cuda.Event(enable_timing=True), torch.cuda.Event(enable_timing=True)
    e0.record()
    launch()
    e1.record()
    _PROFILE.append((variant(),
                     2.0 * n * ho * wo * (kh * kw * (c0 + c1) * cout + (cout * proj.rows if proj is not None else 0)),
                     4.0 * (n * h * w * (c0 + c1) + n * ho * wo * cout * (2 if out_t is not None else 1)
                            + cout * kh * kw * (c0 + c1) * (0.5 if is_split and weight.lo is None else 1.0)), e0, e1,
                     f"{kh}x{kw} {c0 + c1}->{cout}" + (f"->{proj.rows}" if proj is not None else "")))


def frames_to_nhwc4(src, n, H, W, scale, shift, dst):
    if src.dtype == torch.uint8:
        kind = 0
    elif src.dtype == torch.float32:
        kind = 1
    else:
        raise ValueError(f"frames must be uint8 HWC or float32 CHW, got {src.dtype}")
    if not (src.is_cuda and src.is_contiguous()):
        raise ValueError("frames must be a contiguous device tensor")
    _check(lib().vfml_frames_to_nhwc4(c_void_p(src.data_ptr()), kind, n, H, W, scale, shift, _ptr(_dev(dst)),
                                      _stream()), "vfml_frames_to_nhwc4")


def instnorm_workspace_bytes(n, hw, c):
    return int(lib().vfml_instnorm_workspace_bytes(n, hw, c))


def instnorm_stats(x, n, hw, c, stats, workspace, eps=1e-5):
    _check(lib().vfml_instnorm_stats(_ptr(_dev(x)), n, hw, c, eps, _ptr(_dev(stats)),
                                     c_void_p(workspace.data_ptr()), _stream()), "vfml_instnorm_stats")


def instnorm_finalize_workspace_bytes(chunks, c):
    return int(lib().vfml_instnorm_finalize_workspace_bytes(chunks, c))


def instnorm_finalize(part, n, chunks, c, hw, stats, eps=1e-5, workspace=None):
    need = instnorm_finalize_workspace_bytes(chunks, c)
    if need and (workspace is None or workspace.numel() * 8 < need):
        workspace = torch.empty(min(n, 8) * need // 8, dtype=torch.float64, device=stats.device)
    _check(lib().vfml_instnorm_finalize(c_void_p(part.data_ptr()), n, chunks, c, hw, eps, _ptr(_dev(stats)),
                                        c_void_p(workspace.data_ptr()) if workspace is not None else None,
                                        workspace.numel() * 8 if workspace is not None else 0, _stream()),
           "vfml_instnorm_finalize")


def stem_chunks(h, w):
    return int(lib().vfml_stem7x7s2_chunks(h, w))


def pack_stem_weight(w, device):
    w = w.detach().to(device=device, dtype=torch.float32)
    cout, cin = w.shape[0], w.shape[1]
    if cout != 64 or cin not in (3, 4) or tuple(w.shape[2:]) != (7, 7):
        raise ValueError(f"pack_stem_weight: a [64, 3|4, 7, 7] weight expected, got {tuple(w.shape)}")
    k = torch.zeros(cout, 7, 8, 4, device=device)
    k[:, :, :7, :cin] = w.permute(0, 2, 3, 1)
    sw = SplitWeight(cout, 224, device)
    return sw.fill(k.reshape(-1).contiguous(), scale=SplitWeight.auto_scale(float(w.abs().max())))


def stem7x7s2(frames, n, h, w, weight, bias, out, stats_part=None):
    if not isinstance(weight, SplitWeight) or weight.rows != 64 or weight.kp != 224:
        raise ValueError("stem7x7s2: weight must come from pack_stem_weight")
    _check(lib().vfml_stem7x7s2(_ptr(_dev(frames)), n, h, w, c_void_p(weight.hi.data_ptr()), c_void_p(weight.lo.data_ptr()),
                                weight.scale, _ptr(_dev(bias)) if bias is not None else None, _ptr(_dev(out)),
                                c_void_p(stats_part.data_ptr()) if stats_part is not None else None, _stream()), "vfml_stem7x7s2")


def instnorm_apply(x, stats, n, hw, c, out, res=None, res_stats=None, out_fmt=FMT_F32):
    _check(lib().vfml_instnorm_apply(_ptr(_dev(x)), _ptr(_dev(stats)), _ptr(res), _ptr(res_stats), n, hw, c,
                                     _ptr(_dev(out)), out_fmt, _stream()), "vfml_instnorm_apply")


def avgpool2x2(x, n, h, w, c, out):
    _check(lib().vfml_avgpool2x2(_ptr(_dev(x)), n, h, w, c, _ptr(_dev(out)), _stream()), "vfml_avgpool2x2")


def softmax_rows_s16(x, rows, cols, ld_in, out, ld_out, x_off=0, out_off=0, scale=1.0):
    _check(lib().vfml_softmax_rows_s16(_ptr(_dev(x), x_off), rows, cols, ld_in, _ptr(_dev(out), out_off), ld_out,
                                       float(scale), _stream()), "vfml_softmax_rows_s16")


class PlainWeight:
    lo = None
    order = KORDER_TAP

    def __init__(self, rows, kp, device, scale=1.0):
        if kp % 32:
            raise ValueError("PlainWeight: kp must be a multiple of 32")
        self.rows, self.k, self.kp, self.scale = rows, kp, kp, float(scale)
        self.hi = torch.empty(rows * kp, dtype=torch.float16, device=device)


def softmax_rows_f16(x, rows, cols, ld_in, weight, x_off=0):
    _check(lib().vfml_softmax_rows_f16(_ptr(_dev(x), x_off), rows, cols, ld_in, c_void_p(weight.hi.data_ptr()), weight.kp,
                                       weight.scale, _stream()), "vfml_softmax_rows_f16")


def attention_plane_workspace_bytes(p):
    return int(lib().vfml_attention_plane_workspace_bytes(p))


def attention_plane(q, k, p, plane, score_scale=None, d=128, ld_q=None, ld_k=None, q_off=0, k_off=0, workspace=None):
    if not isinstance(plane, PlainWeight):
        raise ValueError("attention_plane: plane must be a PlainWeight")
    if workspace is None:
        workspace = torch.empty(max(1, attention_plane_workspace_bytes(p) // 4), dtype=torch.float32, device=plane.hi.device)
    if workspace.dtype != torch.float32 or workspace.numel() * 4 < attention_plane_workspace_bytes(p) or plane.rows < p:
        raise ValueError("attention_plane: workspace of 2 p floats and a plane of at least p rows")
    _check(lib().vfml_attention_plane_f16(_ptr(_dev(q), q_off), ld_q or d, _ptr(_dev(k), k_off), ld_k or d, p, d,
                                          float(score_scale if score_scale is not None else 1.0 / d ** 0.5), plane.scale,
                                          c_void_p(plane.hi.data_ptr()), plane.kp, c_void_p(workspace.data_ptr()), _stream()),
           "vfml_attention_plane_f16")


ATT_BANK_MAX = 9


def attention_bank_planes(q, keys, p, planes, score_scale=None, d=128, ld_q=None, ld_k=None, q_off=0, k_offs=None,
                          workspace=None):
    n = len(keys)
    if len(planes) != n or not all(isinstance(a, PlainWeight) for a in planes):
        raise ValueError("attention_bank_planes: one PlainWeight per key set")
    if n and any(a.kp != planes[0].kp or a.scale != planes[0].scale or a.rows < p for a in planes):
        raise ValueError("attention_bank_planes: planes of one row stride and one scale, at least p rows each")
    dev = planes[0].hi.device if n else q.device
    if workspace is None:
        workspace = torch.empty(max(1, attention_plane_workspace_bytes(p) // 4), dtype=torch.float32, device=dev)
    if workspace.dtype != torch.float32 or workspace.numel() * 4 < attention_plane_workspace_bytes(p):
        raise ValueError("attention_bank_planes: workspace of 2 p floats")
    k_offs = k_offs or [0] * n
    kptr = (c_void_p * max(1, n))(*[_dev(k).data_ptr() + 4 * o for k, o in zip(keys, k_offs)])
    pptr = (c_void_p * max(1, n))(*[a.hi.data_ptr() for a in planes])
    _check(lib().vfml_attention_bank_planes_f16(_ptr(_dev(q), q_off), ld_q or d, kptr, ld_k or d, n, p, d,
                                                float(score_scale if score_scale is not None else 1.0 / d ** 0.5),
                                                planes[0].scale if n else 1.0, pptr, planes[0].kp if n else 0,
                                                c_void_p(workspace.data_ptr()), _stream()),
           "vfml_attention_bank_planes_f16")


def axpy_f32(x, y, n, scale=1.0, x_off=0, y_off=0):
    _check(lib().vfml_axpy_f32(_ptr(_dev(x), x_off), _ptr(_dev(y), y_off), n, float(scale), _stream()), "vfml_axpy_f32")


DW_RESIDUAL, DW_GELU = 1, 2


def dwconv2d(x, ld_x, n, h, w, c, k, weight, bias, out, ld_out, x_off=0, out_off=0, in_fmt=FMT_F32, out_fmt=FMT_F32,
             residual=False, gelu=False):
    _check(lib().vfml_dwconv2d(_ptr(_dev(x), x_off), ld_x, n, h, w, c, k, _ptr(_dev(weight)), _ptr(_dev(bias)),
                               _ptr(_dev(out), out_off), ld_out, in_fmt, out_fmt,
                               (DW_RESIDUAL if residual else 0) | (DW_GELU if gelu else 0), _stream()), "vfml_dwconv2d")


def gelu_rows(x, ld_x, out, ld_out, rows, c, x_off=0, out_off=0, in_fmt=FMT_F32, out_fmt=FMT_F32):
    _check(lib().vfml_gelu_rows(_ptr(_dev(x), x_off), ld_x, _ptr(_dev(out), out_off), ld_out, rows, c, in_fmt, out_fmt,
                                _stream()), "vfml_gelu_rows")


def layernorm_rows(x, ld_x, out, ld_out, rows, c, gamma, beta, eps=1e-5, x_off=0, out_off=0, in_fmt=FMT_F32, out_fmt=FMT_F32):
    _check(lib().vfml_layernorm_rows(_ptr(_dev(x), x_off), ld_x, _ptr(_dev(out), out_off), ld_out, rows, c, _ptr(_dev(gamma)),
                                     _ptr(_dev(beta)), float(eps), in_fmt, out_fmt, _stream()), "vfml_layernorm_rows")


def window_attention(qkv, ld, n, h, w, c, heads, ws, pad_row, out, ld_out, qkv_off=0, out_off=0, in_fmt=FMT_F32, out_fmt=FMT_F32):
    _check(lib().vfml_window_attention(_ptr(_dev(qkv), qkv_off), ld, n, h, w, c, heads, ws, _ptr(_dev(pad_row)),
                                       _ptr(_dev(out), out_off), ld_out, in_fmt, out_fmt, _stream()), "vfml_window_attention")


def attention_shared_keys(q, ld_q, kv, ld_kv, n, p, pk, c, heads, out, ld_out, q_off=0, kv_off=0, out_off=0, q_fmt=FMT_F32,
                          kv_fmt=FMT_F32, out_fmt=FMT_F32):
    _check(lib().vfml_attention_shared_keys(_ptr(_dev(q), q_off), ld_q, _ptr(_dev(kv), kv_off), ld_kv, n, p, pk, c, heads,
                                            _ptr(_dev(out), out_off), ld_out, q_fmt, kv_fmt, out_fmt, _stream()),
           "vfml_attention_shared_keys")


def transpose_to_s16(src, rows, c, ld, dst, ld_dst, scale=1.0, src_off=0, dst_off=0):
    _check(lib().vfml_transpose_to_s16(_ptr(_dev(src), src_off), rows, c, ld, float(scale), _ptr(_dev(dst), dst_off), ld_dst,
                                       _stream()), "vfml_transpose_to_s16")


def add_to_s16(x, ldx, aux, ld_aux, out, ld_out, rows, c, scale=1.0, x_off=0, aux_off=0, out_off=0):
    _check(lib().vfml_add_to_s16(_ptr(_dev(x), x_off), ldx, _ptr(_dev(aux), aux_off), ld_aux, _ptr(_dev(out), out_off), ld_out,
                                 rows, c, float(scale), _stream()), "vfml_add_to_s16")


def to_s16(src, rows, c, ld_src, dst, ld_dst, src_off=0, dst_off=0, scale=1.0):
    _check(lib().vfml_to_s16(_ptr(_dev(src), src_off), rows, c, ld_src, _ptr(_dev(dst), dst_off), ld_dst, float(scale),
                             _stream()), "vfml_to_s16")


def ptr_table_set(table, tensors):
    n = len(tensors)
    if not (table.is_cuda and table.dtype == torch.int64 and table.numel() >= n):
        raise ValueError("ptr_table_set: table must be an int64 device tensor with room for the pointers")
    ptrs = (c_void_p * n)(*[t if isinstance(t, int) else t.data_ptr() for t in tensors])
    _check(lib().vfml_ptr_table_set(c_void_p(table.data_ptr()), ptrs, n, _stream()), "vfml_ptr_table_set")


def corr_bitmap_words(rows, cols):
    return ((rows + 127) // 128) * (((cols + 63) // 64 + 31) // 32)


def corr_level0_ensure(rows, c, weight, level0, n_rows, n_cols, ldo, out_scale, cells, centres, dirs, dir_cells, coords,
                       coords_off, ld_coords, dir_coords, h, w, radius, vol_tile, counter=None, in_fmt=FMT_S16, mfma=1):
    if not isinstance(weight, SplitWeight) or weight.lo is None:
        raise ValueError("corr_level0_ensure: the target operand is a SplitWeight")
    ndirs = 2 if dirs == 2 else 1
    if not (cells.is_cuda and cells.dtype == torch.int64 and cells.numel() >= 4 * ((ndirs - 1) * dir_cells + centres)):
        raise ValueError("corr_level0_ensure: cells must be an int64 device tensor, four per direction and centre frame")
    if counter is not None and not (counter.is_cuda and counter.dtype == torch.int32):
        raise ValueError("corr_level0_ensure: the counter is an int32 device tensor")
    d = ConvDesc()
    d.in0, d.c0, d.ld0 = _ptr(_dev(rows)), c, c
    d.n, d.h, d.w = 1, 1, n_rows
    d.cout, d.kh, d.kw, d.stride, d.pad_h, d.pad_w = n_cols, 1, 1, 1, 0, 0
    d.out, d.ldo = _ptr(_dev(level0)), ldo
    d.epilogue, d.split, d.out_scale = EPI_NONE, 0, out_scale
    d.flags = {3: 0, 2: CONV_MFMA2, 1: CONV_MFMA1}[mfma]
    _check(lib().vfml_corr_level0_ensure(ctypes.byref(d), c_void_p(weight.hi.data_ptr()), c_void_p(weight.lo.data_ptr()),
                                         weight.kp, weight.scale, in_fmt, FMT_F32, weight.order, c_void_p(cells.data_ptr()),
                                         centres, ndirs, dir_cells, _ptr(_dev(coords), coords_off), ld_coords, dir_coords, h, w,
                                         radius, vol_tile, c_void_p(counter.data_ptr()) if counter is not None else None,
                                         _stream()), "vfml_corr_level0_ensure")


SEED_NONE, SEED_LOAD, SEED_STORE = 0, 1, 2


def window_seed(cells, ncentres, rows, cols, state, ld_state, h_off, mf_off, ld_ctx):
    if not (cells.is_cuda and cells.dtype == torch.int64 and cells.numel() >= 3 * ncentres):
        raise ValueError("window_seed: cells must be an int64 device tensor, three per centre frame")
    _check(lib().vfml_window_seed(c_void_p(cells.data_ptr()), ncentres, rows, cols, _ptr(_dev(state)), ld_state, h_off, mf_off,
                                  ld_ctx, _stream()), "vfml_window_seed")


def corr_lookup(pyrs, hl, wl, ld, radius, q_per_map, coords, coords_off, ld_coords, out, out_off, ld_out,
                out_fmt=FMT_F32, table=None, nmaps=None, vol_fmt=FMT_F32, vol_tile=0, bidir=None):
    L = len(hl)
    if bidir is not None:
        dir_coords, dir_out, dir_tab = bidir

        def launch():
            _check(lib().vfml_corr_lookup_indirect_bidir(c_void_p(table.data_ptr()), (c_int32 * L)(*hl), (c_int32 * L)(*wl),
                                                         (c_int32 * L)(*ld), L, radius, nmaps, q_per_map,
                                                         _ptr(_dev(coords), coords_off), ld_coords, dir_coords,
                                                         _ptr(_dev(out), out_off), ld_out, dir_out, dir_tab, out_fmt, vol_fmt,
                                                         vol_tile, _stream()), "vfml_corr_lookup_indirect_bidir")
    elif table is not None:
        def launch():
            _check(lib().vfml_corr_lookup_indirect(c_void_p(table.data_ptr()), (c_int32 * L)(*hl), (c_int32 * L)(*wl),
                                                   (c_int32 * L)(*ld), L, radius, nmaps, q_per_map,
                                                   _ptr(_dev(coords), coords_off), ld_coords, _ptr(_dev(out), out_off),
                                                   ld_out, out_fmt, vol_fmt, vol_tile, _stream()), "vfml_corr_lookup_indirect")
    else:
        if pyrs and torch.is_tensor(pyrs[0]):
            pyrs = [pyrs]
        nmaps, L = len(pyrs), len(pyrs[0])
        ptrs = (c_void_p * (nmaps * L))(*[p.data_ptr() for m in pyrs for p in m])

        def launch():
            _check(lib().vfml_corr_lookup(ptrs, (c_int32 * L)(*hl), (c_int32 * L)(*wl), (c_int32 * L)(*ld), L, radius,
                                          nmaps, q_per_map, _ptr(_dev(coords), coords_off), ld_coords,
                                          _ptr(_dev(out), out_off), ld_out, out_fmt, vol_fmt, vol_tile, _stream()), "vfml_corr_lookup")
    if _PROFILE_HBM is None:
        launch()
        return
    e0, e1 = torch.cuda.Event(enable_timing=True), torch.cuda.Event(enable_timing=True)
    e0.record()
    launch()
    e1.record()
    q = (2 if bidir is not None else 1) * nmaps * q_per_map
    m16 = _vol_mask(vol_fmt, L)
    texel_bytes = sum(2.0 if (m16 >> l) & 1 else 4.0 for l in range(L))
    _PROFILE_HBM.append(("corr_lookup", q * ((2 * radius + 2) ** 2 * texel_bytes + L * (2 * radius + 1) ** 2 * 4.0), e0, e1))


class VolTile:

    def __init__(self, tws, ths):
        self.tws, self.ths = tws, ths
        self.code = tws + 16 * ths
        self._pos = {}

    def count(self, h, w):
        return ((((h - 1) >> self.ths) + 1) * (((w - 1) >> self.tws) + 1)) << (self.tws + self.ths)

    def position(self, h, w, dev):
        key = (h, w, str(dev))
        if key not in self._pos:
            y = torch.arange(h, device=dev, dtype=torch.int64).view(h, 1)
            x = torch.arange(w, device=dev, dtype=torch.int64).view(1, w)
            tpr = ((w - 1) >> self.tws) + 1
            pos = ((((y >> self.ths) * tpr + (x >> self.tws)) << (self.tws + self.ths))
                   + ((y & ((1 << self.ths) - 1)) << self.tws) + (x & ((1 << self.tws) - 1)))
            self._pos[key] = pos.reshape(-1).contiguous()
        return self._pos[key]

    def rows(self, x, h, w, c):
        n = self.count(h, w)
        out = torch.zeros(n, c, device=x.device, dtype=x.dtype)
        out.index_copy_(0, self.position(h, w, x.device), x.view(h * w, c))
        return out.view(-1)


def coords_init(coords1, n, h, w):
    _check(lib().vfml_coords_init(_ptr(_dev(coords1)), n, h, w, _stream()), "vfml_coords_init")


def flow_rows7(flow, n, h, w, rows):
    _check(lib().vfml_flow_rows7(_ptr(_dev(flow)), n, h, w, _ptr(_dev(rows)), _stream()), "vfml_flow_rows7")


def tapsum3x3(t, ld_t, bias, n, h, w, out, parts=1, part_stride=0):
    _check(lib().vfml_tapsum3x3(_ptr(_dev(t)), ld_t, _ptr(bias) if bias is not None else None, n, h, w, _ptr(_dev(out)),
                                parts, part_stride, _stream()), "vfml_tapsum3x3")


def conv3x3_c64(src, ld_in, n, h, w, weight, bias, out, ldo, stats_part=None, src_off=0):
    _check(lib().vfml_conv3x3_c64(_ptr(_dev(src), src_off), ld_in, n, h, w, c_void_p(weight.hi.data_ptr()),
                                  c_void_p(weight.lo.data_ptr()), weight.kp, weight.scale,
                                  _ptr(_dev(bias)) if bias is not None else None, _ptr(_dev(out)), ldo,
                                  c_void_p(stats_part.data_ptr()) if stats_part is not None else None, _stream()),
           "vfml_conv3x3_c64")


def flow_half(flow, n, h, w, w1, b1, w2, b2, out, ld_out, out_off=0):
    _check(lib().vfml_flow_half(_ptr(_dev(flow)), n, h, w, c_void_p(w1.hi.data_ptr()), w1.kp, w1.scale, _ptr(_dev(b1)),
                                c_void_p(w2.hi.data_ptr()), w2.kp, w2.scale, _ptr(_dev(b2)), _ptr(_dev(out), out_off), ld_out,
                                _stream()), "vfml_flow_half")


def tapsum3x3_update(t, ld_t, bias, n, h, w, coords1, parts=1, part_stride=0, flow_a=None, ld_a=0, flow_a_off=0, flow_b=None,
                     ld_b=0, flow_b_off=0, fmt_b=FMT_F32):
    _check(lib().vfml_tapsum3x3_update(_ptr(_dev(t)), ld_t, _ptr(bias) if bias is not None else None, n, h, w, parts, part_stride,
                                       _ptr(_dev(coords1)), _ptr(flow_a, flow_a_off), ld_a, _ptr(flow_b, flow_b_off), ld_b,
                                       fmt_b, _stream()), "vfml_tapsum3x3_update")


def coords_update(coords1, delta, n, h, w, flow_a=None, ld_a=0, flow_a_off=0, flow_b=None, ld_b=0, flow_b_off=0,
                  fmt_b=FMT_F32):
    _check(lib().vfml_coords_update(_ptr(_dev(coords1)), _ptr(delta), n, h, w,
                                    _ptr(flow_a, flow_a_off), ld_a, _ptr(flow_b, flow_b_off), ld_b, fmt_b, _stream()),
           "vfml_coords_update")


def flow_forward_interpolate_workspace(n, h, w, device):
    nbytes = lib().vfml_flow_forward_interpolate_workspace_bytes(n, h, w)
    return torch.empty(max(1, nbytes // 8), dtype=torch.int64, device=device)


def flow_forward_interpolate(flow, h=None, w=None, n=1, ld_in=None, out=None, ld_out=None, index=None, workspace=None):
    _dev(flow)
    shape = None
    if h is None or w is None:
        if flow.dim() not in (3, 4) or flow.shape[-1] not in (2, 4):
            raise ValueError(f"flow_forward_interpolate: flow [h, w, 2] or [n, h, w, c] expected (or flat rows with h, w), "
                             f"got {tuple(flow.shape)}")
        shape = tuple(flow.shape)
        h, w, ld_in = shape[-3], shape[-2], shape[-1]
        n = shape[0] if flow.dim() == 4 else 1
    ld_in = ld_in or 2
    ld_out = ld_out or ld_in
    if flow.numel() < n * h * w * ld_in:
        raise ValueError(f"flow_forward_interpolate: flow holds {flow.numel()} floats, {n} x {h} x {w} x {ld_in} expected")
    if out is None:
        out = torch.empty(shape[:-1] + (ld_out,) if shape else (n * h * w * ld_out,), dtype=torch.float32, device=flow.device)
    if _dev(out).device != flow.device or out.numel() < n * h * w * ld_out:
        raise ValueError(f"flow_forward_interpolate: out of {n} x {h} x {w} x {ld_out} floats on {flow.device} expected")
    if index is not None and (_dev(index, torch.int32).device != flow.device or index.numel() < n * h * w):
        raise ValueError(f"flow_forward_interpolate: index of {n} x {h} x {w} int32 on {flow.device} expected")
    if workspace is None:
        workspace = flow_forward_interpolate_workspace(n, h, w, flow.device)
    if _dev(workspace, torch.int64).device != flow.device:
        raise ValueError(f"flow_forward_interpolate: workspace on {flow.device} expected")
    _check(lib().vfml_flow_forward_interpolate(_ptr(flow), ld_in, n, h, w, _ptr(out), ld_out,
                                               None if index is None else c_void_p(index.data_ptr()),
                                               c_void_p(workspace.data_ptr()), workspace.numel() * 8, _stream()),
           "vfml_flow_forward_interpolate")
    return out


def flow_lods(flow, num_lods=5):
    lods = [_dev(flow.contiguous())]
    for _ in range(1, num_lods):
        h, w = lods[-1].shape[:2]
        out = torch.empty((h + 1) // 2, (w + 1) // 2, 2, device=flow.device, dtype=torch.float32)
        _check(lib().vfml_flow_lod(_ptr(lods[-1]), h, w, _ptr(out), _stream()), "vfml_flow_lod")
        lods.append(out)
    return lods


ENCODE_GAMEDEV, ENCODE_RG8, ENCODE_RGB8 = 0, 1, 2


def flow_encode(flow, mode, clamp_range, width=1.0, height=1.0, scale=1.0):
    import numpy as np
    f = _dev(flow.contiguous())
    h, w = f.shape[:2]
    out = torch.empty((h, w, 3), dtype=torch.uint8, device=f.device)
    _check(lib().vfml_flow_encode(_ptr(f), h, w, mode, float(np.float32(width)), float(np.float32(height)),
                                  float(np.float32(scale)), float(np.float32(clamp_range)),
                                  float(np.float32(2 * clamp_range)), c_void_p(out.data_ptr()), _stream()),
           "vfml_flow_encode")
    return out


TAA_SIMPLE, TAA_BILINEAR, TAA_BILATERAL = 0, 1, 2
_PIX = {torch.uint8: 0, torch.float32: 1, torch.float64: 2}


def taa_blend(current, flow, history, mode, alpha, sigma_color=25.0):
    cur, hist = current.contiguous(), history.contiguous()
    if not (cur.is_cuda and hist.is_cuda and cur.dtype in (torch.uint8, torch.float32)
            and hist.dtype in (torch.float32, torch.float64)):
        raise ValueError(f"taa_blend: device tensors u8/f32 + f32/f64 expected, got {cur.dtype} {hist.dtype}")
    h, w = cur.shape[:2]
    if tuple(cur.shape) != (h, w, 3) or tuple(hist.shape) != (h, w, 3):
        raise ValueError(f"taa_blend: [H,W,3] images expected, got {tuple(cur.shape)} {tuple(hist.shape)}")
    if mode != TAA_SIMPLE:
        flow = _dev(flow.contiguous())
        if tuple(flow.shape) != (h, w, 2):
            raise ValueError(f"taa_blend: flow {tuple(flow.shape)} does not match the frame {h}x{w}")
    out_dtype = hist.dtype if mode == TAA_SIMPLE else (torch.float32 if mode == TAA_BILINEAR else torch.float64)
    out = torch.empty((h, w, 3), dtype=out_dtype, device=cur.device)
    _check(lib().vfml_taa_blend(c_void_p(cur.data_ptr()), _PIX[cur.dtype], None if mode == TAA_SIMPLE else _ptr(flow),
                                c_void_p(hist.data_ptr()), _PIX[hist.dtype], c_void_p(out.data_ptr()), _PIX[out_dtype],
                                h, w, mode, float(alpha), float(sigma_color), _stream()), "vfml_taa_blend")
    return out


COLORIZE_HSV, COLORIZE_WHEEL = 0, 1


def flow_colorize(flow, mode):
    f = _dev(flow.contiguous())
    if f.dim() != 3 or f.shape[2] != 2:
        raise ValueError(f"flow_colorize: [H,W,2] flow expected, got {tuple(f.shape)}")
    h, w = f.shape[:2]
    out = torch.empty((h, w, 3), dtype=torch.uint8, device=f.device)
    cell = torch.empty(1, dtype=torch.int32, device=f.device)
    _check(lib().vfml_flow_colorize(_ptr(f), h, w, mode, c_void_p(cell.data_ptr()), c_void_p(out.data_ptr()), _stream()),
           "vfml_flow_colorize")
    return out


def flow_decode(encoded, mode, clamp_range):
    import numpy as np
    e = _dev(encoded, torch.uint8)
    if e.dim() != 3 or e.shape[2] != 3:
        raise ValueError(f"flow_decode: [H,W,3] picture expected, got {tuple(e.shape)}")
    h, w = e.shape[:2]
    out = torch.empty((h, w, 2), dtype=torch.float32, device=e.device)
    _check(lib().vfml_flow_decode(c_void_p(e.data_ptr()), h, w, mode, float(np.float32(clamp_range)), _ptr(out),
                                  _stream()), "vfml_flow_decode")
    return out


def flow_diff_overlay(flow_a, flow_b):
    a, b = _dev(flow_a.contiguous()), _dev(flow_b.contiguous())
    if a.dim() != 3 or a.shape[2] != 2 or a.shape != b.shape:
        raise ValueError(f"flow_diff_overlay: two [H,W,2] flows of one size expected, got {tuple(a.shape)} "
                         f"{tuple(b.shape)}")
    h, w = a.shape[:2]
    out = torch.empty((h, w, 3), dtype=torch.uint8, device=a.device)
    _check(lib().vfml_flow_diff_overlay(_ptr(a), _ptr(b), h, w, c_void_p(out.data_ptr()), _stream()),
           "vfml_flow_diff_overlay")
    return out


COMPOSE_SIDE_BY_SIDE, COMPOSE_STACKED, COMPOSE_GRID_2X2, COMPOSE_GRID_2X3 = 0, 1, 2, 3
COMPOSE_BGR, COMPOSE_BOTTOM_UP = 1, 2


def compose_frame(tiles, layout, bgr=True, bottom_up=False, row_stride=None, out=None):
    nt = {COMPOSE_GRID_2X2: 4, COMPOSE_GRID_2X3: 6}.get(layout, 2)
    if len(tiles) != nt:
        raise ValueError(f"compose_frame: layout {layout} takes {nt} tiles, got {len(tiles)}")
    ts = [t.contiguous() for t in tiles]
    h, w = ts[0].shape[:2]
    for t in ts:
        if not (t.is_cuda and t.dtype in _PIX and tuple(t.shape) == (h, w, 3)):
            raise ValueError(f"compose_frame: device [H,W,3] u8/f32/f64 tiles of one size expected, got "
                             f"{t.dtype} {tuple(t.shape)} on {t.device}")
    ow = w if layout == COMPOSE_STACKED else 2 * w
    oh = h if layout == COMPOSE_SIDE_BY_SIDE else (3 * h if layout == COMPOSE_GRID_2X3 else 2 * h)
    stride = 3 * ow if row_stride is None else int(row_stride)
    if out is None:
        out = torch.empty((oh, stride), dtype=torch.uint8, device=ts[0].device)
    elif not (out.is_cuda and out.dtype == torch.uint8 and out.is_contiguous() and out.numel() >= oh * stride):
        raise ValueError(f"compose_frame: out must be a contiguous uint8 device tensor of >= {oh * stride} bytes")
    ptrs = (c_void_p * nt)(*[t.data_ptr() for t in ts])
    types = (c_int32 * nt)(*[_PIX[t.dtype] for t in ts])
    flags = (COMPOSE_BGR if bgr else 0) | (COMPOSE_BOTTOM_UP if bottom_up else 0)
    _check(lib().vfml_compose_frame(ptrs, types, h, w, layout, flags, stride, c_void_p(out.data_ptr()), _stream()),
           "vfml_compose_frame")
    return out


class TextPlan:

    def __init__(self, words, device):
        import numpy as np
        self.host = np.array(words, dtype=np.int32)
        if self.host.ndim != 1 or self.host.size < 8:
            raise ValueError("TextPlan: a one-dimensional int32 plan of at least 8 words expected")
        self.dev = torch.empty(self.host.size, dtype=torch.int32, device=device)
        addr = self.dev.data_ptr()
        self.host[2:4] = np.array([addr & 0xffffffff, addr >> 32], dtype=np.uint32).view(np.int32)
        self.dev.copy_(torch.from_numpy(self.host))

    @property
    def boxes(self):
        return int(self.host[4])


def text_draw(plan, img, h, w, row_stride=None, bottom_up=False):
    stride = 3 * w if row_stride is None else int(row_stride)
    if not (img.is_cuda and img.dtype == torch.uint8 and img.is_contiguous() and img.numel() >= h * stride):
        raise ValueError(f"text_draw: img must be a contiguous uint8 device tensor of >= {h * stride} bytes")
    if plan.dev.device != img.device:
        raise ValueError(f"text_draw: the plan lives on {plan.dev.device}, the frame on {img.device}")
    _check(lib().vfml_text_draw(plan.host.ctypes.data_as(c_void_p), plan.host.size, c_void_p(img.data_ptr()), h, w, stride,
                                COMPOSE_BOTTOM_UP if bottom_up else 0, _stream()), "vfml_text_draw")
    return img


# ... 439 lines not shown
```

video-flow-ml_amd/vfml/network.py:

```python
import os
import types

import torch
import torch.nn as nn

from . import hip, update_block
from .weights import (BASE_CORR_LEVELS, BASE_CORR_RADIUS, GMA_NO_BIAS, TWINS_STAGES, TWINS_WS, conv_spec, corr_channel_subset,
                      is_depthwise, pack_conv_weight, pcblock_hidden, sk_blocks, twins_spec)

ATT_SCALE = 16384.0


def cor_pad(cor, split):
    return (cor + 15) // 16 * 16 if split else (cor + 3) // 4 * 4


def take_frames(src, idx):
    idx = list(idx)
    if all(b == a + 1 for a, b in zip(idx, idx[1:])):
        return src[idx[0]:idx[0] + len(idx)]
    return torch.stack([src[i] for i in idx])


class _Holder(nn.Module):
# ... 570 lines not shown
        st = self._att_store
        if st is None or st["key"] != (str(dev), Pn) or st["R"] < M + 2:
            self._join_prefetch()
            self._graphs.clear()
            self._att_store = None
            P8, ldA, plain = self._attention_geometry(Pn)
            R = M + 2
            st = self._att_store = {
                "key": (str(dev), Pn), "R": R, "next": 0, "owner": [None] * R, "live": set(), "plain": plain,
                "P8": P8, "ldA": ldA, "serial": getattr(self, "_att_serial", 0) + 1,
                "k": None if plain else hip.SplitWeight(Pn, self.ATT_DIM, dev),
                "vt": None if plain else hip.SplitWeight(self.ATT_DIM, P8, dev),
                "A": [hip.PlainWeight(Pn, ldA, dev, scale=ATT_SCALE) if plain else torch.empty(Pn * ldA, device=dev)
                      for _ in range(R)]}
            self._att_serial = st["serial"]
        return st

    def _attention_slot(self, st, cache_key, busy):
        busy = set(busy) | st["live"]
        for _ in range(st["R"]):
            s = st["next"]
            st["next"] = (s + 1) % st["R"]
            if s not in busy:
                break
        else:
            raise RuntimeError("attention store: every slot is in use by the current window")
        old = st["owner"][s]
        if old is not None and old != cache_key:
            self._feat_cache.pop(old, None)
        st["owner"][s] = cache_key
        return s

    def _build_attention(self, st, slot, cx, h8, w8, Pn, P, dev, AF):
        AD, ldA = self.ATT_DIM, st["ldA"]
        wgt, _ = P["att.to_qk"]
        nmq = self._nm("att.to_qk")
        if st["plain"]:
            qk = self._buf("att_qk", Pn * 2 * AD, dev)
            hip.conv2d(cx, 128, 256, 1, h8, w8, wgt, None, 2 * AD, 1, 1, qk, 2 * AD, in0_off=128, in_fmt=AF, mfma=nmq)
            hip.attention_plane(qk, qk, Pn, st["A"][slot], score_scale=1.0 / float(AD) ** 0.5, d=AD, ld_q=2 * AD, ld_k=2 * AD,
                                k_off=AD, workspace=self._buf("att_stats", 2 * Pn, dev))
            return
        qmap = self._buf("att_q", Pn * AD, dev)
        kmap = self._buf("att_k", Pn * AD, dev)
        hip.conv2d(cx, 128, 256, 1, h8, w8, wgt, None, AD, 1, 1, qmap, AD, in0_off=128, in_fmt=AF, out_fmt=AF, mfma=nmq)
        hip.conv2d(cx, 128, 256, 1, h8, w8, wgt, None, AD, 1, 1, kmap, AD, in0_off=128, weight_off=AD, in_fmt=AF, mfma=nmq)
        kw_ = st["k"].fill(kmap, scale=16.0)
        scores = self._buf("att_scores", Pn * ldA, dev)
        hip.conv2d(qmap, AD, AD, 1, 1, Pn, kw_, None, Pn, 1, 1, scores, ldA, out_scale=1.0 / float(AD) ** 0.5, in_fmt=AF)
        hip.softmax_rows_s16(scores, Pn, Pn, ldA, st["A"][slot], ldA, scale=ATT_SCALE)

    ITER0_RING = 8
    iter0_store = True

    def _iter0_store(self, dev, Pn, M):
        st = getattr(self, "_it0_store", None)
        if st is None or st["key"] != (str(dev), Pn) or st["ring"].R < M + 1:
            self._join_prefetch()
            for k in [k for k in self._feat_cache if k[0] == "m"]:
                del self._feat_cache[k]
            R = max(self.ITER0_RING, M + 1)
            st = self._it0_store = {"key": (str(dev), Pn), "ring": Iter0Ring(R, self._feat_cache),
                                    "S": torch.empty(R * Pn * 128, device=dev)}
        return st

    GRAPHS_KEPT = 8

    def _use_graph(self):
        use = getattr(self.cfg, "use_graph", None)
        if use is None:
            use = os.environ.get("VFML_GRAPH", "1") != "0"
        return bool(use) and hip._PROFILE is None

    def _run_body(self, body, key, dev):
        if not self._use_graph():
            body()
            return
        st = self._graphs.get(key)
        if st is None:
            body()
            while len(self._graphs) >= self.GRAPHS_KEPT:
                self._graphs.pop(next(iter(self._graphs)))
            self._graphs[key] = "seen"
            return
        if st == "seen":
            g = torch.cuda.CUDAGraph()
            with torch.cuda.graph(g, capture_error_mode="thread_local"):
                body()
            self._graphs[key] = st = g
        st.replay()

    def _encoder(self, prefix, x, n, H, W, P, dev, out, ldo, out_off, epilogue, split, out_fmt=hip.FMT_F32):
        h2, w2 = H // 2, W // 2
        big = n * h2 * w2 * 64
        raw = self._buf("enc_raw", big, dev)
        raw2 = self._buf("enc_raw2", big, dev)
        act = [self._buf("enc_act0", big, dev), self._buf("enc_act1", big, dev), self._buf("enc_act2", big, dev)]
        st = self._buf("enc_stats", 3 * n * 128 * 2, dev)
        nws = hip.instnorm_workspace_bytes(n, h2 * w2, 128)
        ws = self._buf("enc_statws", (nws + 7) // 8, dev, torch.float64)

        def stats_of(t, hw, c, slot):
            s = st[slot * n * 128 * 2:]
            hip.instnorm_stats(t, n, hw, c, s, ws)
            return s

        split_prec = self._split()
        AF = hip.FMT_S16 if split_prec else hip.FMT_F32
        part_len = n * ((h2 * w2 + 31) // 32) * 64 * 2
        parts = self._buf("enc_part", 3 * part_len, dev, torch.float64) if split_prec else None
        fold_ws = self._buf("enc_foldws", min(n, 8) * 64 * 128 * 2, dev, torch.float64) if split_prec else None

        def conv_stats(src, c, hh_, ww_, name, planes, dst, slot, k, stride=1, pad=0, src_fmt=hip.FMT_F32):
            wgt, b = P[name]
            nm = self._nm(name) if split_prec else 3
            ho_, wo_ = (hh_ + 2 * pad - k) // stride + 1, (ww_ + 2 * pad - k) // stride + 1
            hw = ho_ * wo_
            rows = hip.STATS_ROWS_S16 if src_fmt == hip.FMT_S16 else hip.STATS_ROWS_F32
            if not (split_prec and (n == 1 or hw % rows == 0)):
                hip.conv2d(src, c, c, n, hh_, ww_, wgt, b, planes, k, k, dst, planes, stride=stride, pad_h=pad, pad_w=pad,
                           mfma=nm, in_fmt=src_fmt)
                return stats_of(dst, hw, planes, slot)
            chunks = (hw + rows - 1) // rows
            part = parts[slot * part_len:]
            if (c == 64 and planes == 64 and k == 3 and stride == 1 and pad == 1 and nm == 3 and src_fmt == hip.FMT_S16
                    and ww_ % 32 == 0 and getattr(wgt, "order", None) == hip.KORDER_CBLOCK and wgt.kp == 576 and wgt.lo is not None):
                hip.conv3x3_c64(src, c, n, hh_, ww_, wgt, b, dst, planes, stats_part=part)
            else:
                hip.conv2d(src, c, c, n, hh_, ww_, wgt, b, planes, k, k, dst, planes, stride=stride, pad_h=pad, pad_w=pad,
                           stats_part=part, mfma=nm, in_fmt=src_fmt)
            s = st[slot * n * 128 * 2:]
            hip.instnorm_finalize(part, n, chunks, planes, hw, s, workspace=fold_ws)
            return s

        stem = P.get(f"{prefix}.conv1.stem")
        if stem is not None and split_prec and self._nm(f"{prefix}.conv1") == 3:
            chunks = hip.stem_chunks(H, W)
            part = parts[0:]
            hip.stem7x7s2(x, n, H, W, stem[0], stem[1], raw, stats_part=part)
            s0 = st[0:]
            hip.instnorm_finalize(part, n, chunks, 64, h2 * w2, s0, workspace=fold_ws)
        else:
            s0 = conv_stats(x, 4, H, W, f"{prefix}.conv1", 64, raw, 0, 7, stride=2, pad=3)
        cur = act[0]
        hip.instnorm_apply(raw, s0, n, h2 * w2, 64, cur, out_fmt=AF)
        ch, hh, ww, ci = 64, h2, w2, 0
        for li, (planes, stride) in enumerate([(64, 1), (96, 2), (128, 2)], start=1):
            for bi in range(2):
                stv = stride if bi == 0 else 1
                ho, wo = (hh, ww) if stv == 1 else ((hh - 1) // 2 + 1, (ww - 1) // 2 + 1)
                name = f"{prefix}.layer{li}.{bi}"
                y = act[(ci + 1) % 3]
                nxt = act[(ci + 2) % 3]
                s1 = conv_stats(cur, ch, hh, ww, f"{name}.conv1", planes, raw, 0, 3, stride=stv, pad=1, src_fmt=AF)
                hip.instnorm_apply(raw, s1, n, ho * wo, planes, y, out_fmt=AF)
                s2 = conv_stats(y, planes, ho, wo, f"{name}.conv2", planes, raw, 1, 3, pad=1, src_fmt=AF)
                if stv != 1:
                    s3 = conv_stats(cur, ch, hh, ww, f"{name}.downsample.0", planes, raw2, 2, 1, stride=stv, src_fmt=AF)
                    hip.instnorm_apply(raw, s2, n, ho * wo, planes, nxt, res=raw2, res_stats=s3, out_fmt=AF)
                else:
                    hip.instnorm_apply(raw, s2, n, ho * wo, planes, nxt, res=cur, out_fmt=AF)
                cur, ci = nxt, (ci + 2) % 3
                ch, hh, ww = planes, ho, wo
        wgt, b = P[f"{prefix}.conv2"]
        hip.conv2d(cur, 128, 128, n, hh, ww, wgt, b, 256, 1, 1, out, ldo, out_off=out_off, epilogue=epilogue,
                   split=split, out_fmt=out_fmt, in_fmt=AF, mfma=self._nm(f"{prefix}.conv2") if split_prec else 3)
        return hh, ww

    @torch.no_grad()
    def forward(self, images, data=None, return_lowres=True):
        if not isinstance(images, torch.Tensor) or not images.is_cuda:
            raise RuntimeError("MOFNetHIP runs on an MI355X (HIP) device only; got "
                               f"{getattr(images, 'device', type(images))}. There is no CPU fallback in the shipped engine.")
        if images.dim() != 5 or images.shape[2] != 3:
            raise ValueError(f"images must be [B,N,3,H,W], got {tuple(images.shape)}")
        if images.shape[0] != 1:
            raise ValueError(f"Batch size must be 1, got {images.shape[0]}")
        src = images[0]
        if src.dtype != torch.float32:
            src = src.float()
        return self._run(src.contiguous(), src.shape[0], src.shape[2], src.shape[3], return_lowres)

    @torch.no_grad()
    def forward_u8(self, frames, return_lowres=True, frame_keys=None, tri_batch=False, pick_only=False, dense_corr=False):
        if not (isinstance(frames, torch.Tensor) and frames.is_cuda and frames.dtype == torch.uint8
                and frames.dim() == 4 and frames.shape[3] == 3):
            raise ValueError("forward_u8 expects a uint8 [N,H,W,3] device tensor")
        if frame_keys is not None and len(frame_keys) != frames.shape[0]:
            raise ValueError("frame_keys must have one entry per frame")
        if tri_batch and not self.tri_frame:
            raise ValueError("tri_batch applies to tri-frame (BOF) networks")
        return self._run(frames.contiguous(), frames.shape[0], frames.shape[1], frames.shape[2], return_lowres,
                         frame_keys, tri_batch, pick_only and not return_lowres, dense_corr)

    FEATURE_CACHE_FRAMES = 12
    FMAP_ROW_SCALE = 16.0

    def clear_feature_cache(self):
        self._join_prefetch()
        self._feat_cache.clear()
        self._pyr_free = []

    def prefetch_frames(self, frames, frame_keys):
        if (frame_keys is None or self._pre_body is None or os.environ.get("VFML_PREFETCH", "1") == "0" or self.tri_frame):
            return
        cfg = self.cfg
        N, H, W = frames.shape[0], frames.shape[1], frames.shape[2]
        if N < 3 or H % 8 or W % 8 or len(frame_keys) != N:
            return
        L, dev = cfg.corr_levels, frames.device
        h, w = H // 8, W // 8
        AF = hip.FMT_S16 if self._split() else hip.FMT_F32
        geo = self._volume_geometry(H, W, L, AF)
        hl, wl, Sl = geo.hl, geo.wl, geo.Sl
        keys = [(k, H, W, L, self._plan_key(), self._packed_serial) for k in frame_keys]
        need_f = [j for j in range(N) if ("f", keys[j]) not in self._feat_cache]
        need_c = [j for j in range(1, N - 1) if ("c", keys[j]) not in self._feat_cache]
        if not need_f and not need_c:
            return
        main = torch.cuda.current_stream(dev)
        side = self._side.get(dev)
        if side is None:
            side = self._side[dev] = torch.cuda.Stream(device=dev)
        P = self._pack(dev)
        if "serial" in os.environ.get("VFML_PREFETCH_DBG", ""):
            side.wait_stream(main)
        else:
            side.wait_event(self._pre_body)
        frames.record_stream(side)
        with torch.cuda.stream(side):
            new = []
            if need_f:
                new += list(self._frame_features(frames, need_f, keys, H, W, P, dev, L, hl, wl, Sl, vt=geo.VT).values())
            if need_c:
                new += list(self._frame_context(frames, need_c, keys, H, W, P, dev, h * w, N - 2).values())
            done = torch.cuda.Event()
            done.record(side)

        def walk(x):
            if isinstance(x, torch.Tensor):
                x.record_stream(main)
            elif isinstance(x, (list, tuple)):
                for y in x:
                    walk(y)
            elif isinstance(x, dict):
                for y in x.values():
                    walk(y)
            elif hasattr(x, "planes") and isinstance(getattr(x, "planes"), torch.Tensor):
                x.planes.record_stream(main)
        walk(new)
        self._prefetch_done, self._prefetch_dev = done, dev

    def _pyramid_buffers(self, sizes, dev, limit):
        while sum(1 for k in self._feat_cache if k[0] == "p") >= limit:
            oldest = next(k for k in self._feat_cache if k[0] == "p")
            self._pyr_free.append(self._feat_cache.pop(oldest))
        for i, bufs in enumerate(self._pyr_free):
            if [b.numel() for b in bufs] == sizes and bufs[0].device == dev:
                return self._pyr_free.pop(i)
        del self._pyr_free[:]
        return [torch.empty(n, device=dev) for n in sizes]

    def _cache_get(self, kind, key):
        ent = self._feat_cache.get((kind, key))
        if ent is not None:
            self._feat_cache.move_to_end((kind, key))
        return ent

    def _cache_put(self, kind, key, value, limit=None):
        self._feat_cache[(kind, key)] = value
        while sum(1 for k in self._feat_cache if k[0] == kind) > (limit or self.FEATURE_CACHE_FRAMES):
            oldest = next(k for k in self._feat_cache if k[0] == kind)
            del self._feat_cache[oldest]

    def _volume_geometry(self, H, W, L, AF):
        cfg = self.cfg
        h, w = H // 8, W // 8
        hl, wl = [h], [w]
        for l in range(1, L):
            hl.append(hl[-1] // 2)
            wl.append(wl[-1] // 2)
        Sl = [hl[l] * wl[l] for l in range(L)]
        VT = self._tile()
        Nl = [VT.count(hl[l], wl[l]) for l in range(L)] if VT is not None else Sl
        Pv = Nl[0]
        TILE = VT.code if VT is not None else 0
        mask = self.CORR_VOLUMES[getattr(cfg, "corr_volume", "f32")] & ((1 << L) - 1)
        if not (mask and AF == hip.FMT_S16 and Pv % 4 == 0 and all(s % 4 == 0 for s in Nl) and L <= 4
                and cfg.corr_radius in (3, 4)):
            mask = 0
        v16 = [bool((mask >> l) & 1) for l in range(L)]
        VFl = [hip.FMT_F16 if v16[l] else hip.FMT_F32 for l in range(L)]
        VF = (hip.FMT_F32 if not mask else hip.FMT_F16 if mask == (1 << L) - 1 else hip.vol_f16_levels(mask))
        ldl = []
        for l in range(L):
            unit = 64 if v16[l] else 32
            n = (Nl[l] + unit - 1) // unit * unit
            ldl.append(n if (n // unit) % 2 else n + unit)
        psz = [(Pv * ldl[l] + 1) // 2 if v16[l] else Pv * ldl[l] for l in range(L)]
        return types.SimpleNamespace(L=L, AF=AF, hl=hl, wl=wl, Sl=Sl, VT=VT, Nl=Nl, Pv=Pv, TILE=TILE, vol16=mask, VF=VF,
                                     VFl=VFl, ldl=ldl, psz=psz)

    corr_on_demand = True

    def _corr_scale(self, AF):
        scale = 1.0 / float(self.cfg.feat_dim) ** 0.5
        if AF == hip.FMT_S16:
            scale /= self.FMAP_ROW_SCALE
        return scale

    def _level0_on_demand(self, keys, N, geo, dense_corr=False):
        return (self.corr_on_demand and not dense_corr and keys is not None and self._split() and not self.tri_frame
                and not self.gma and not self.sk and geo.AF == hip.FMT_S16 and geo.Pv % 4 == 0 and geo.Nl[0] >= 1024
                and geo.VT is not None and geo.Pv == geo.Nl[0] and geo.VFl[0] == hip.FMT_F32 and self._nm("corr") == 1
                and self.cfg.feat_dim <= 256 and 2 * (N - 2) <= 8 and (geo.Nl[0] + 63) // 64 <= 2048)

    @staticmethod
    def _pyramid_bitmap(pyr, L):
        return pyr[L].view(torch.int32)

    def corr_tiles_computed(self, reset=True):
        count = self._ws.get("ensure_count")
        if count is None:
            return 0
        n = int(count.item())
        if reset:
            count.zero_()
        return n

    def _window_pyramids(self, feats, keys, N, geo, dev, on_demand=False):
        D, L = self.cfg.feat_dim, geo.L
        AF, VFl, Nl, Pv, ldl, psz = geo.AF, geo.VFl, geo.Nl, geo.Pv, geo.ldl, geo.psz
        scale = self._corr_scale(AF)
        lim = 2 * (N - 2) + 2
        pyrs = {"f": [], "b": []}
        od = ("od",) if on_demand else ()
        if on_demand:
            psz = psz + [hip.corr_bitmap_words(Pv, Nl[0])]
        first = 1 if on_demand else 0
        for c in range(1, N - 1):
            for d, tgt in (("f", c + 1), ("b", c - 1)):
                pk = ("p", keys[c], keys[tgt]) + od if keys is not None else None
                if pk is not None and self.gma and d == "b" and keys[c] == keys[tgt]:
                    pk += ("b",)
                pyr = self._cache_get("p", pk) if pk is not None else None
                if pyr is None:
                    if pk is None:
                        pyr = [self._buf(f"pyr_{d}{c}_{l}", psz[l], dev) for l in range(L)]
                    else:
                        pyr = self._pyramid_buffers(psz, dev, limit=lim)
                        self._cache_put("p", pk, pyr, limit=lim)
                    rk = ("p", keys[tgt], keys[c]) + od if pk is not None else None
                    gemm_form = AF == hip.FMT_S16 and Pv % 4 == 0 and Nl[0] >= 1024
                    dual = rk is not None and d == "f" and gemm_form and ("p", rk) not in self._feat_cache
                    rev = None
                    if dual:
                        rev = self._pyramid_buffers(psz, dev, limit=lim)
                        self._cache_put("p", rk, rev, limit=lim)
                    cnm = self._nm("corr") if self._split() else 3
                    for l in range(first, L):
                        hip.conv2d(feats[c][0], D, D, 1, 1, Pv, feats[tgt][1][l], None, Nl[l], 1, 1, pyr[l],
                                   ldl[l], out_scale=scale, in_fmt=AF, out_fmt=VFl[l],
                                   swap_cross=(d == "b" and l == 0 and gemm_form and cnm == 3),
                                   out_t=rev[0] if dual and l == 0 else None, ld_out_t=ldl[0] if dual and l == 0 else 0,
                                   mfma=cnm)
                    if dual:
                        for l in range(1, L):
                            hip.conv2d(feats[tgt][0], D, D, 1, 1, Pv, feats[c][1][l], None, Nl[l], 1, 1, rev[l],
                                       ldl[l], out_scale=scale, in_fmt=AF, out_fmt=VFl[l], mfma=cnm)
                    if on_demand:
                        for p in (pyr, rev) if dual else (pyr,):
                            self._pyramid_bitmap(p, L).zero_()
                pyrs[d].append(pyr)
        return pyrs

    def _ensure_plan(self, pyrs, feats, N, geo, dev):
        M = N - 2
        cells = self._buf("ensure_cells", 64, dev, torch.int64)
        ptrs = []
        for d, step in (("f", 1), ("b", -1)):
            for i, c in enumerate(range(1, N - 1)):
                pyr = pyrs[d][i]
                ptrs += [feats[c][0], feats[c + step][1][0].hi, pyr[0], self._pyramid_bitmap(pyr, geo.L)]
        hip.ptr_table_set(cells, ptrs)
        count = self._buf("ensure_count", 1, dev, torch.int32, zero=True)
        return types.SimpleNamespace(cells=cells, M=M, rows=feats[1][0], weight=feats[2][1][0], level0=pyrs["f"][0][0],
                                     D=self.cfg.feat_dim, scale=self._corr_scale(geo.AF), counter=count)

    def _frame_features(self, src, sel, keys, H, W, P, dev, L, hl, wl, Sl, vt=None):
        D = self.cfg.feat_dim
        split = self._split()
        out, todo = {}, []
        for j in sel:
            ent = self._cache_get("f", keys[j]) if keys is not None else None
            if ent is not None:
                out[j] = ent
            else:
                todo.append(j)
        if todo:
            m, Pn = len(todo), hl[0] * wl[0]
            frames = self._buf("frames", m * H * W * 4, dev)
            hip.frames_to_nhwc4(take_frames(src, todo).contiguous(), m, H, W, float(self.cfg.input_scale), float(self.cfg.input_shift),
                                frames)
            fmap = torch.empty(m * Pn * D, device=dev)
            (self._twins_encoder if self.twins else self._encoder)("fnet", frames, m, H, W, P, dev, fmap, D, 0, hip.EPI_NONE, 0)
            levels = [fmap]
            for l in range(1, L):
                t = torch.empty(m * Sl[l] * D, device=dev)
                hip.avgpool2x2(levels[-1], m, hl[l - 1], wl[l - 1], D, t)
                levels.append(t)
            for i, j in enumerate(todo):
                tg = []
                for l in range(L):
                    f = levels[l][i * Sl[l] * D:(i + 1) * Sl[l] * D]
                    nl = Sl[l]
                    if vt is not None:
                        f, nl = vt.rows(f, hl[l], wl[l], D), vt.count(hl[l], wl[l])
                    tg.append(hip.SplitWeight(nl, D, dev).fill(f, scale=16.0) if split else f)
                fm = fmap[i * Pn * D:(i + 1) * Pn * D]
                if vt is not None:
                    fm, Pn_rows = vt.rows(fm, hl[0], wl[0], D), vt.count(hl[0], wl[0])
                else:
                    Pn_rows = Pn
                if split:
                    fm16 = torch.empty(Pn_rows * D, device=dev)
                    hip.to_s16(fm, Pn_rows, D, D, fm16, D, scale=self.FMAP_ROW_SCALE)
                    fm = fm16
                ent = (fm, tg)
                out[j] = ent
                if keys is not None:
                    self._cache_put("f", keys[j], ent)
        return out

    def _frame_context(self, src, sel, keys, H, W, P, dev, Pn, M=1):
        out, todo = {}, []
        st = self._context_store(dev, Pn, max(M, len(sel)))
        att = self._attention_store(dev, Pn, max(M, len(sel))) if self.gma else None
        for j in sel:
            ent = self._cache_get("c", keys[j]) if keys is not None else None
            if ent is not None and ent[3] == st["serial"] and (att is None or ent[5] == att["serial"]):
                out[j] = ent
            else:
                todo.append(j)
        if todo:
            m = len(todo)
            frames = self._buf("frames", m * H * W * 4, dev)
            hip.frames_to_nhwc4(take_frames(src, todo).contiguous(), m, H, W,
                                float(self.cfg.input_scale), float(self.cfg.input_shift), frames)
            ctx = torch.empty(m * Pn * 256, device=dev)
            AF = hip.FMT_S16 if self._split() else hip.FMT_F32
            (self._twins_encoder if self.twins else self._encoder)("cnet", frames, m, H, W, P, dev, ctx, 256, 0, hip.EPI_TANH_RELU,
                                                                   self.hidden_dim, out_fmt=AF)
            h8, w8 = H // 8, W // 8
            R, Mst = st["R"], st["M"]
            for i, j in enumerate(todo):
                cx = ctx[i * Pn * 256:(i + 1) * Pn * 256]
                busy = {e[2] for e in out.values()}
                slot = self._context_slot(st, ("c", keys[j]) if keys is not None else None, busy)
                add = {}
                for k, (kh, kw) in () if self.sk else (("1", (1, 5)), ("2", (5, 1))):
                    for g, co in (("zr", 256), ("q", 128)):
                        wgt, b = P[f"update_block.gru.conv{g}{k}.ctx"]
                        S = st["S"][g + k]
                        hip.conv2d(cx, 128, 256, 1, h8, w8, wgt, b, co, kh, kw, S, co, in0_off=128, out_off=slot * Pn * co,
                                   pad_h=kh // 2, pad_w=kw // 2, in_fmt=AF,
                                   mfma=self._nm(f"update_block.gru.conv{g}{k}.ctx") if self._split() else 3)
                        add[g + k] = S[slot * Pn * co:(slot + 1) * Pn * co]
                        if slot < Mst - 1:
                            S[(R + slot) * Pn * co:(R + slot + 1) * Pn * co].copy_(add[g + k])
                ent = (cx, add, slot, st["serial"])
                if att is not None:
                    aslot = self._attention_slot(att, ("c", keys[j]) if keys is not None else None,
                                                 {e[4] for e in out.values()})
                    self._build_attention(att, aslot, cx, h8, w8, Pn, P, dev, AF)
                    ent += (aslot, att["serial"])
                out[j] = ent
                if keys is not None:
                    self._cache_put("c", keys[j], out[j])
        return out

    def _state_columns(self):
        GLD, cols = 768, dict(Z=0, RH=128, HH=256, INP=384, MF=512, MT=640, MG=None, XC=256)
        if self.gma:
            GLD = 896
            cols.update(MG=768, XC=384)
        if self.sk:
            GLD = 640 if self.gma else 512
            cols.update(HH=0, INP=128, MF=256, MT=384, MG=512)
        return GLD, cols

    def _window_state(self, P, dev, M, h, w, geo, R, AF, cor_p):
        MP = M * h * w
        GLD, cols = self._state_columns()
        if self.gma and self._att_store is not None:
            self._att_store["live"] = set()

        def rows(name, c):
            return self._buf(name, MP * c, dev)
        return update_block.window_state(
            P, self._nm if self._split() else (lambda layer: 3),
            AF, h, w, geo, R, rows("gru_state", GLD), GLD, cols, 2 * cor_p, cor_p, self._rows7, self._tapsum,
            corr=self._buf("corr", MP * 2 * cor_p, dev, zero=True),
            c1=rows("c1", 256), cf=rows("cf", 256), f1=rows("f1", 128), fh=rows("fh", 256), flow4=rows("flow4", 4),
            delta=rows("delta", 4), fh_taps=rows("fh_taps", 2 * 36),
            frows=rows("flow_rows7", 32), coords1=rows("coords1", 4))

    def _seed_plan(self, s, ctx, keys, dev, M, R, pick_only):
        cfg, it0 = self.cfg, None
        if (self.iter0_store and not self.sk and keys is not None and self._split() and not self.tri_frame and M >= 2
                and cfg.decoder_depth >= 1 and not (pick_only and cfg.decoder_depth + 1 < M)):
            it0 = self._iter0_store(dev, s.Pn, M)
            warm, seeds, it0_new = it0["ring"].plan(keys, tail=(R,))
            self.iter0_stats["warm" if warm else "cold"] += 1
            self.iter0_last = (warm, [slot for slot, _ in seeds])
        else:
            warm, seeds, it0_new = False, [(None, hip.SEED_NONE)] * M, []
        seed_cells = self._buf("seed_cells", 64, dev, torch.int64)
        hip.ptr_table_set(seed_cells, [v for i, (slot, mode) in enumerate(seeds) for v in
                                       (ctx[i + 1][0], it0["S"][slot * s.Pn * 128:] if slot is not None else 0, mode)])
        return it0, warm, it0_new, seed_cells

    def _gate_addends(self, ctx, dev, Pn, M):
        st = self._ctx_store
        RING, Mst = st["R"], st["M"]
        slots = [ctx[c][2] for c in range(1, M + 1)]
        st["live"] = set(slots)
        first = slots[0]
        if not self.sk and (not self._split() or os.environ.get("VFML_CTX_GATHER", "0") == "1" or
                            not all(s == first + i or (first + i >= RING and s == first + i - RING and s < Mst - 1)
                                    for i, s in enumerate(slots))):
            first = RING + Mst - 1
            for i, c in enumerate(range(1, M + 1)):
                for name, co in self.CTX_GATES:
                    st["S"][name][(first + i) * Pn * co:(first + i + 1) * Pn * co].copy_(ctx[c][1][name])
        gate_add = {name: st["S"].get(name) for name, _ in self.CTX_GATES}
        gate_off = {name: first * Pn * co for name, co in self.CTX_GATES}
        gate_ind = None
        if self._split() and not self.sk:
            cells = self._buf("gate_add_cells", 8, dev, torch.int64)
            hip.ptr_table_set(cells, [st["S"][name][gate_off[name]:] for name, _ in self.CTX_GATES])
            gate_ind = {name: (cells, i) for i, (name, _) in enumerate(self.CTX_GATES)}
        return gate_add, gate_off, gate_ind

    def _pyramid_tables(self, pyrs, dev, M, L, cor_p):
        if 2 * M <= 8 and 2 * M * L <= 48:
            tab_fb = self._buf("pyr_table_fb", 64, dev, torch.int64)
            hip.ptr_table_set(tab_fb, [p for d in ("f", "b") for m in pyrs[d] for p in m[:L]])
            return (tab_fb,), (2, cor_p, M)
        tab_f = self._buf("pyr_table_f", 64, dev, torch.int64)
        tab_b = self._buf("pyr_table_b", 64, dev, torch.int64)
        hip.ptr_table_set(tab_f, [p for m in pyrs["f"] for p in m[:L]])
        hip.ptr_table_set(tab_b, [p for m in pyrs["b"] for p in m[:L]])
        return (tab_f, tab_b), None

    def _gma_readout(self, s, win, ng):
        att = self._att_store
        update_block.attention_readout(s, "update_block.aggregator.to_v", [att["A"][k] for k in win.att_slots[:ng]],
                                       att["plain"], att["ldA"], att["P8"], self._gamma, ATT_SCALE, s.MF, s.MG, win.readout)

    def _iteration(self, s, win, it, ng, nm, branch):
        ub = update_block
        ne, r0 = (1, (win.M - 1) * s.Pn) if win.warm and it == 0 else (nm, 0)
        join = None
        if branch is not None:
            fork = torch.cuda.Event()
            fork.record()
            with torch.cuda.stream(branch):
                branch.wait_event(fork)
                ub.flow_half(s, ne, r0)
                join = torch.cuda.Event()
                join.record()
        if win.ensure is not None:
            ub.ensure_level0(s, ne, r0, win.ensure)
        ub.lookup(s, ne, r0, win.tables, win.bidir)
        ub.convc1(s, ne, r0)
        ub.convc2(s, ne, r0)
        if join is None:
            ub.flow_half(s, ne, r0)
        else:
            torch.cuda.current_stream(win.dev).wait_event(join)
        ub.encoder_conv(s, ne, r0)
        if it == 0:
            hip.window_seed(win.seed_cells, win.M, s.Pn, 128, s.G, s.GLD, s.HH, s.MF, 256)
        if self.gma:
            self._gma_readout(s, win, ng)
        update_block.temporal_fusion(s, win.M if self.tri_frame else nm, stack=not self.tri_frame)
        ub.sep_conv_gru(s, ng, *win.gates)
        ub.flow_head(s, ng)

    def _sk_iteration(self, s, win, ng, nm):
        ub, P, h, w, G, GLD, ws = "update_block", s.P, s.h, s.w, s.G, s.GLD, win.sk_ws
        blk = self._pcblock
        update_block.lookup(s, nm, 0, win.tables, win.bidir)
        blk(f"{ub}.encoder.convc1", P, s.corr, s.ld_corr, 0, nm, h, w, s.c1, 256, 0, ws, gelu_out=True)
        blk(f"{ub}.encoder.convc2", P, s.c1, 256, 0, nm, h, w, s.cf, 256, 0, ws)
        wgt, b = P[f"{ub}.encoder.convf1"]
        hip.conv2d(s.flow4, 4, 4, nm, h, w, wgt, b, 128, 1, 1, s.f1, 128, out_fmt=s.AF, mfma=s.nm(f"{ub}.encoder.convf1"))
        blk(f"{ub}.encoder.convf2", P, s.f1, 128, 0, nm, h, w, s.cf, 256, 192, ws)
        blk(f"{ub}.encoder.conv", P, s.cf, 256, 0, nm, h, w, G, GLD, s.MF, ws)
        if self.gma:
            self._gma_readout(s, win, ng)
        update_block.temporal_fusion(s, win.M if self.tri_frame else nm, stack=not self.tri_frame)
        blk(f"{ub}.gru", P, G, GLD, 0, ng, h, w, G, GLD, s.HH, ws)
        blk(f"{ub}.flow_head", P, G, GLD, s.HH, ng, h, w, s.delta, 4, 0, ws, out_fmt=hip.FMT_F32)
        update_block.update_coords(s, ng)

    def _run(self, src, N, H, W, return_lowres, frame_keys=None, tri_batch=False, pick_only=False, dense_corr=False):
        cfg = self.cfg
        if N < 3:
            raise ValueError(f"need at least 3 frames, got {N}")
        if self.tri_frame and N > 3 and not tri_batch:
            lo = N // 2 - 1
            src = src[lo:lo + 3].contiguous()
            frame_keys = frame_keys[lo:lo + 3] if frame_keys is not None else None
            N = 3
        if H % 8 or W % 8:
            raise ValueError("H and W must be multiples of 8 (use InputPadder)")
        L, R = cfg.corr_levels, cfg.corr_radius
        h, w = H // 8, W // 8
        if (h >> (L - 1)) < 2 or (w >> (L - 1)) < 2:
            raise ValueError(f"frame {H}x{W} too small for a {L}-level correlation pyramid")
        dev = src.device
        self._join_prefetch()
        M = N - 2
        Pn = h * w
        if self.gma and Pn > 32768:
            raise ValueError(f"frame {H}x{W}: the GMA aggregator attends over all {Pn} cells of a frame and is built for at "
                             f"most 32768; process larger frames in tiles (--tile)")
        MP = M * Pn
        P = self._pack(dev)
        AF = hip.FMT_S16 if self._split() else hip.FMT_F32
        cor_p = cor_pad(L * (2 * R + 1) ** 2, AF == hip.FMT_S16)
        short = pick_only and not self.tri_frame

        with torch.cuda.device(dev):
            geo = self._volume_geometry(H, W, L, AF)
            keys = None
            if frame_keys is not None:
                keys = [(k, H, W, L, self._plan_key(), self._packed_serial) for k in frame_keys]

            feats = self._frame_features(src, list(range(N)), keys, H, W, P, dev, L, geo.hl, geo.wl, geo.Sl, vt=geo.VT)
            on_demand = self._level0_on_demand(keys, N, geo, dense_corr)
            pyrs = self._window_pyramids(feats, keys, N, geo, dev, on_demand)
            s = self._window_state(P, dev, M, h, w, geo, R, AF, cor_p)
            ctx = self._frame_context(src, list(range(1, N - 1)), keys, H, W, P, dev, Pn, M)
            win = types.SimpleNamespace(M=M, dev=dev, att_slots=(), readout=None)
            if self.gma:
                att = self._att_store
                win.att_slots = tuple(ctx[c][4] for c in range(1, N - 1))
                att["live"] = set(win.att_slots)
                win.readout = update_block.readout_scratch(self._buf, dev, MP, Pn, self.ATT_DIM, att["ldA"], att["plain"],
                                                           att["vt"])
            it0, win.warm, it0_new, win.seed_cells = self._seed_plan(s, ctx, keys, dev, M, R, pick_only)
            win.gates = self._gate_addends(ctx, dev, Pn, M)
            win.sk_ws = self._sk_workspace(MP, dev) if self.sk else None
            win.tables, win.bidir = self._pyramid_tables(pyrs, dev, M, L, cor_p)
            win.ensure = self._ensure_plan(pyrs, feats, N, geo, dev) if on_demand else None
            no, nflows = (1, 1) if short else (M, 2 * M)
            up_fixed = self._buf("up_out", nflows * H * W * 2, dev)
            mask = self._buf("mask", MP * 1152, dev)

            def body():
                update_block.init_coords(s, M)
                branch = None
                if os.environ.get("VFML_FLOW_BRANCH", "0") == "1" and self._split():
                    branch = self._side2.get(dev)
                    if branch is None:
                        branch = self._side2[dev] = torch.cuda.Stream(device=dev)
                if self.sk:
                    hip.window_seed(win.seed_cells, M, Pn, 256, s.G, s.GLD, s.HH, s.MF, 256)
                for it in range(cfg.decoder_depth):
                    left = cfg.decoder_depth - 1 - it
                    ng = min(M, left + 1) if short else M
                    nm = min(M, left + 2) if short else M
                    if self.sk:
                        self._sk_iteration(s, win, ng, nm)
                    else:
                        self._iteration(s, win, it, ng, nm, branch)
                if cfg.decoder_depth == 0 and not self.sk:
                    hip.window_seed(win.seed_cells, M, Pn, 128, s.G, s.GLD, s.HH, s.MF, 256)
                update_block.mask_head(s, no, mask, 1152)
                if short:
                    hip.convex_upsample(s.coords1, 0, 2, mask, 576, 1152, h, w, up_fixed)
                else:
                    for d in range(2):
                        for c in range(M):
                            hip.convex_upsample(s.coords1, c * Pn * 4, 2 * d, mask, c * Pn * 1152 + d * 576, 1152, h, w,
                                                up_fixed, out_off=(d * M + c) * H * W * 2)

            gkey = (H, W, N, M, bool(tri_batch), bool(pick_only), cfg.decoder_depth, L, R, self._plan_key(), geo.vol16,
                    self._packed_serial, str(dev), os.environ.get("VFML_FLOW_BRANCH", "0"), win.warm, win.att_slots, on_demand)
            if self.sk:
                gkey += ("sk",)
            self._pre_body = torch.cuda.Event()
            self._pre_body.record(torch.cuda.current_stream(dev))
            try:
                self._run_body(body, gkey, dev)
            except BaseException:
                if it0_new:
                    it0["ring"].forget(it0_new)
                raise
            up = up_fixed.clone().view(nflows, H, W, 2)
            flow = up.permute(0, 3, 1, 2).unsqueeze(0)
            if short:
                return flow, None
            low = s.flow4.view(M, h, w, 4)[..., :].clone() if return_lowres else None
        return flow, low


def build_network(cfg):
    return MOFNetHIP(cfg)
```

video-flow-ml_amd/vfml/update_block.py:

```python
import types

from . import hip

UB = "update_block"


def window_state(P, nm, AF, h, w, geo, R, G, GLD, cols, ld_corr, cor_p, rows7, tapsum, **maps):
    return types.SimpleNamespace(P=P, nm=nm, AF=AF, h=h, w=w, Pn=h * w, geo=geo, R=R, G=G, GLD=GLD, ld_corr=ld_corr, cor_p=cor_p,
                                 rows7=rows7, tapsum=tapsum,
                                 fuse=AF == hip.FMT_S16,
                                 **cols, **maps)


def _put_flow(s):
    return dict(flow_a=s.flow4, ld_a=4, flow_b=s.G, ld_b=s.GLD, flow_b_off=s.MF + 124, fmt_b=s.AF)


def init_coords(s, n, flow_init=None):
    hip.coords_init(s.coords1, n, s.h, s.w)
    hip.coords_update(s.coords1, flow_init, n, s.h, s.w, **_put_flow(s))


def lookup(s, n, r0, tables=(), bidir=None, pyrs=None):
    g = s.geo
    if pyrs is not None:
        hip.corr_lookup(pyrs, g.hl, g.wl, g.ldl, s.R, s.Pn, s.coords1, r0 * 4, 4, s.corr, r0 * s.ld_corr, s.ld_corr,
                        out_fmt=s.AF, vol_fmt=g.VF, vol_tile=g.TILE)
        return
    t0 = r0 // s.Pn * g.L
    for d, tab in enumerate(tables):
        hip.corr_lookup(None, g.hl, g.wl, g.ldl, s.R, s.Pn, s.coords1, r0 * 4 + 2 * d, 4, s.corr, r0 * s.ld_corr + d * s.cor_p,
                        s.ld_corr, out_fmt=s.AF, table=tab[t0:], nmaps=n, vol_fmt=g.VF, vol_tile=g.TILE, bidir=bidir)


def ensure_level0(s, n, r0, en):
    g = s.geo
    c0 = r0 // s.Pn
    hip.corr_level0_ensure(en.rows, en.D, en.weight, en.level0, g.Pv, g.Nl[0], g.ldl[0], en.scale, en.cells[4 * c0:], n, 2,
                           en.M, s.coords1, r0 * 4, 4, 2, g.hl[0], g.wl[0], s.R, g.TILE, counter=en.counter, in_fmt=s.AF)


def convc1(s, n, r0):
    wgt, b = s.P[f"{UB}.encoder.convc1"]
    hip.conv2d(s.corr, s.ld_corr, s.ld_corr, n, s.h, s.w, wgt, b, 256, 1, 1, s.c1, 256, epilogue=hip.EPI_RELU,
               in0_off=r0 * s.ld_corr, out_off=r0 * 256, in_fmt=s.AF, out_fmt=s.AF, mfma=s.nm(f"{UB}.encoder.convc1"))


def convc2(s, n, r0):
    wgt, b = s.P[f"{UB}.encoder.convc2"]
    hip.conv2d(s.c1, 256, 256, n, s.h, s.w, wgt, b, 192, 3, 3, s.cf, 256, in0_off=r0 * 256, out_off=r0 * 256,
               pad_h=1, pad_w=1, epilogue=hip.EPI_RELU, in_fmt=s.AF, out_fmt=s.AF, mfma=s.nm(f"{UB}.encoder.convc2"))


def flow_half(s, n, r0):
    nm1, nm2 = s.nm(f"{UB}.encoder.convf1"), s.nm(f"{UB}.encoder.convf2")
    wgt, b = s.P[f"{UB}.encoder.convf1"]
    wgt2, b2 = s.P[f"{UB}.encoder.convf2"]
    if (s.fuse and s.rows7 and nm1 == 1 and nm2 == 1
            and getattr(wgt2, "order", None) == hip.KORDER_CBLOCK64 and wgt.kp == 224 and wgt2.kp == 1152):
        hip.flow_half(s.flow4[r0 * 4:], n, s.h, s.w, wgt, b, wgt2, b2, s.cf, 256, out_off=r0 * 256 + 192)
        return
    if s.rows7:
        hip.flow_rows7(s.flow4[r0 * 4:], n, s.h, s.w, s.frows[r0 * 32:])
        hip.conv2d(s.frows, 32, 32, n, s.h, s.w, wgt, b, 128, 7, 1, s.f1, 128, pad_h=3, epilogue=hip.EPI_RELU,
                   in0_off=r0 * 32, out_off=r0 * 128, in_fmt=s.AF, out_fmt=s.AF, mfma=nm1)
    else:
        hip.conv2d(s.flow4, 4, 4, n, s.h, s.w, wgt, b, 128, 7, 7, s.f1, 128, pad_h=3, pad_w=3, epilogue=hip.EPI_RELU,
                   in0_off=r0 * 4, out_off=r0 * 128, out_fmt=s.AF, mfma=nm1)
    hip.conv2d(s.f1, 128, 128, n, s.h, s.w, wgt2, b2, 64, 3, 3, s.cf, 256, in0_off=r0 * 128, out_off=r0 * 256 + 192,
               pad_h=1, pad_w=1, epilogue=hip.EPI_RELU, in_fmt=s.AF, out_fmt=s.AF, mfma=nm2)


def encoder_conv(s, n, r0):
    wgt, b = s.P[f"{UB}.encoder.conv"]
    hip.conv2d(s.cf, 256, 256, n, s.h, s.w, wgt, b, 124, 3, 3, s.G, s.GLD, in0_off=r0 * 256, out_off=r0 * s.GLD + s.MF,
               pad_h=1, pad_w=1, epilogue=hip.EPI_RELU, in_fmt=s.AF, out_fmt=s.AF, mfma=s.nm(f"{UB}.encoder.conv"))


def readout_scratch(buf, dev, rows, Pn, AD, ldA, plain, vt=None):
    ro = types.SimpleNamespace(AD=AD, vt=vt, val=buf("att_v", rows * AD, dev))
    if plain:
        ro.vrows = buf("att_vt", AD * ldA, dev)
        ro.out = buf("att_ro", AD * ldA, dev)
        ro.out_t = buf("att_ro_t", Pn * AD, dev)
        ro.ws = buf("att_ro_ws", AD * ldA + Pn * AD, dev)
    return ro


def plane_readout(s, a, ldA, ro, val, val_off=0):
    hip.transpose_to_s16(val, s.Pn, ro.AD, ro.AD, ro.vrows, ldA, scale=16.0, src_off=val_off)
    hip.conv2d(ro.vrows, ldA, ldA, ro.AD, 1, 1, a, None, s.Pn, 1, 1, ro.out, ldA, out_scale=1.0 / 16.0,
               in_fmt=s.AF, out_t=ro.out_t, ld_out_t=ro.AD, mfma=1, ksplit_ws=ro.ws)


def attention_readout(s, layer, planes, plain, ldA, P8, gamma, att_scale, src, dst, ro, addend=None):
    if addend is not None and not (plain and len(planes) == 1):
        raise ValueError("attention_readout: an addend needs the plane form and a single frame")
    n, Pn, AD, G, GLD, AF = len(planes), s.Pn, ro.AD, s.G, s.GLD, s.AF
    wgt, b = s.P[layer]
    hip.conv2d(G, 128, GLD, n, s.h, s.w, wgt, b, AD, 1, 1, ro.val, AD, in0_off=src, in_fmt=AF, mfma=s.nm(layer))
    for k, a in enumerate(planes):
        if plain:
            plane_readout(s, a, ldA, ro, ro.val, k * Pn * AD)
            if addend is not None:
                hip.axpy_f32(addend, ro.out_t, Pn * AD)
            hip.add_to_s16(ro.out_t, AD, G, GLD, G, GLD, Pn, AD, scale=gamma, aux_off=k * Pn * GLD + src,
                           out_off=k * Pn * GLD + dst)
        else:
            vt = ro.vt.fill_transposed(ro.val, Pn, ld=AD, scale=16.0, src_off=k * Pn * AD)
            hip.conv2d(a, P8, ldA, Pn, 1, 1, vt, None, AD, 1, 1, G, GLD, out_off=k * Pn * GLD + dst,
                       out_scale=gamma / att_scale, epilogue=hip.EPI_ADD_AUX, aux0=G, ld_aux0=GLD,
                       aux0_off=k * Pn * GLD + src, in_fmt=AF, out_fmt=AF, aux_fmt=AF,
                       mfma=s.nm(layer.rsplit(".", 1)[0] + ".readout"))


def temporal_fusion(s, n, stack):
    wgt, b = s.P[f"{UB}.tprop"]
    nb, nh = (1, n) if stack else (n, 1)
    hip.conv2d(s.G, 128, s.GLD, nb, nh, s.Pn, wgt, b, 128, 3, 1, s.G, s.GLD, in0_off=s.MF, out_off=s.MT, pad_h=1,
               epilogue=hip.EPI_RELU, in_fmt=s.AF, out_fmt=s.AF, mfma=s.nm(f"{UB}.tprop"))


def sep_conv_gru(s, n, gate_add, gate_off, gate_ind=None):
    G, GLD, AF = s.G, s.GLD, s.AF
    for k, (kh, kw) in (("1", (1, 5)), ("2", (5, 1))):
        ind = {g: gate_ind[g + k] if gate_ind else None for g in ("zr", "q")}
        off = {g: 0 if gate_ind else gate_off[g + k] for g in ("zr", "q")}
        wgt, _ = s.P[f"{UB}.gru.convzr{k}.iter"]
        hip.conv2d(G, 128, GLD, n, s.h, s.w, wgt, None, 256, kh, kw, G, GLD, in0_off=s.HH, out_off=s.Z,
                   in1=G, c1=s.XC, ld1=GLD, in1_off=s.MF, pad_h=kh // 2, pad_w=kw // 2,
                   epilogue=hip.EPI_GRU_ZR, split=128, aux0=G, ld_aux0=GLD, aux0_off=s.HH,
                   addend=gate_add["zr" + k], ld_addend=256, in_fmt=AF, out_fmt=AF, aux_fmt=AF,
                   addend_off=off["zr"], addend_ind=ind["zr"], mfma=s.nm(f"{UB}.gru.convzr{k}.iter"))
        wgt, _ = s.P[f"{UB}.gru.convq{k}.iter"]
        hip.conv2d(G, 128, GLD, n, s.h, s.w, wgt, None, 128, kh, kw, G, GLD, in0_off=s.RH, out_off=s.HH,
                   in1=G, c1=s.XC, ld1=GLD, in1_off=s.MF, pad_h=kh // 2, pad_w=kw // 2,
                   epilogue=hip.EPI_GRU_Q, aux0=G, ld_aux0=GLD, aux0_off=s.Z,
                   aux1=G, ld_aux1=GLD, aux1_off=s.HH, addend=gate_add["q" + k], ld_addend=128,
                   addend_off=off["q"], addend_ind=ind["q"],
                   in_fmt=AF, out_fmt=AF, aux_fmt=AF, mfma=s.nm(f"{UB}.gru.convq{k}.iter"))


def flow_head(s, n, cout=4):
    G, GLD, AF = s.G, s.GLD, s.AF
    wgt, b = s.P[f"{UB}.flow_head.conv1"]
    wgt2, b2 = s.P[f"{UB}.flow_head.conv2"]
    nm1, nm2 = s.nm(f"{UB}.flow_head.conv1"), s.nm(f"{UB}.flow_head.conv2")
    if s.tapsum and s.fuse and nm1 in (3, "2a") and nm2 == nm1:
        hip.conv2d(G, 128, GLD, n, s.h, s.w, wgt, b, 256, 3, 3, s.fh, 256, in0_off=s.HH, pad_h=1, pad_w=1,
                   epilogue=hip.EPI_RELU, in_fmt=AF, out_fmt=AF, mfma=nm1, proj=wgt2, proj_out=s.fh_taps, ld_proj=36)
        hip.tapsum3x3_update(s.fh_taps, 36, b2, n, s.h, s.w, s.coords1, parts=2, part_stride=n * s.Pn * 36, **_put_flow(s))
        return
    hip.conv2d(G, 128, GLD, n, s.h, s.w, wgt, b, 256, 3, 3, s.fh, 256, in0_off=s.HH, pad_h=1, pad_w=1,
               epilogue=hip.EPI_RELU, in_fmt=AF, out_fmt=AF, mfma=nm1)
    if s.tapsum:
        hip.conv2d(s.fh, 256, 256, n, s.h, s.w, wgt2, None, 36, 1, 1, s.fh_taps, 36, in_fmt=AF, mfma=nm2)
        hip.tapsum3x3_update(s.fh_taps, 36, b2, n, s.h, s.w, s.coords1, **_put_flow(s))
        return
    hip.conv2d(s.fh, 256, 256, n, s.h, s.w, wgt2, b2, cout, 3, 3, s.delta, 4, pad_h=1, pad_w=1, in_fmt=AF, mfma=nm2)
    update_coords(s, n)


def update_coords(s, n):
    hip.coords_update(s.coords1, s.delta, n, s.h, s.w, **_put_flow(s))


def mask_head(s, n, mask, width):
    wgt, b = s.P[f"{UB}.mask.0"]
    hip.conv2d(s.G, 128, s.GLD, n, s.h, s.w, wgt, b, 256, 3, 3, s.fh, 256, in0_off=s.HH, pad_h=1, pad_w=1,
               epilogue=hip.EPI_RELU, in_fmt=s.AF, out_fmt=s.AF, mfma=s.nm(f"{UB}.mask.0"))
    wgt, b = s.P[f"{UB}.mask.2"]
    hip.conv2d(s.fh, 256, 256, n, s.h, s.w, wgt, b, width, 1, 1, mask, width, out_scale=0.25, in_fmt=s.AF,
               mfma=s.nm(f"{UB}.mask.2"))
```

Measured before the change: 49.22.

## Extend on-demand correlation volume computation from level 0 to level 1

Measured after the change: 50.34, median of 6. 2.3% higher.

```diff
diff --git a/include/vfml.h b/include/vfml.h
--- a/include/vfml.h
+++ b/include/vfml.h
@@ -136,6 +136,19 @@
                             const float* coords, int ld_coords, int dir_coords, int h, int w, int radius, int vol_tile,
                             uint32_t* counter, void* stream);
 
+typedef struct vfml_corr_level_desc {
+  const vfml_conv_desc* d;
+  const void* w_hi;
+  const void* w_lo;
+  int32_t kp;
+  float w_scale;
+  int32_t out_fmt, level, h, w;
+} vfml_corr_level_desc;
+int vfml_corr_levels_ensure(const vfml_corr_level_desc* levels, int nlevels, int in_fmt, int k_order,
+                            const void* const* cells, int centres, int dirs, int dir_cells, const float* coords,
+                            int ld_coords, int dir_coords, int h, int w, int radius, int vol_tile, uint32_t* counters,
+                            void* stream);
+
 #define VFML_SEED_NONE 0
 #define VFML_SEED_LOAD 1
 #define VFML_SEED_STORE 2
diff --git a/video-flow-ml_amd/vfml/csrc/corr_ensure.hip b/video-flow-ml_amd/vfml/csrc/corr_ensure.hip
--- a/video-flow-ml_amd/vfml/csrc/corr_ensure.hip
+++ b/video-flow-ml_amd/vfml/csrc/corr_ensure.hip
@@ -4,9 +4,18 @@
 namespace {
 
 constexpr int ENSURE_MASK_WORDS = 64;
+constexpr int ENSURE_MAX_LEVELS = 3;
+
+struct EnsureLevel {
+  SplitArgs g;
+  int h, w;
+  int wpr;
+  int level;
+};
 
 struct EnsureArgs {
-  SplitArgs g;
+  EnsureLevel lv[ENSURE_MAX_LEVELS];
+  int nlev;
   const void* const* cells;
   const float* coords;
   unsigned* counter;
@@ -14,8 +23,8 @@
   int centres, dirs, dir_cells;
   int q_per_map;
   int h, w, radius, tws, ths;
-  int wpr;
 };
+static_assert(sizeof(EnsureArgs) <= 4096, "the levels' arguments travel as kernel arguments");
 
 struct MaskCols {
   unsigned v;
@@ -47,65 +56,146 @@
 typedef __attribute__((address_space(1))) unsigned* gu32ptr;
 typedef const __attribute__((address_space(1))) float* gf32cptr;
 
-__global__ __launch_bounds__(256, 2) void corr_ensure_kernel(const EnsureArgs e) {
+typedef const __attribute__((address_space(4))) EnsureArgs* ensure_kargs_t;
+
+__global__ __launch_bounds__(256, 2) void corr_ensure_kernel(const EnsureArgs) {
   extern __shared__ __attribute__((aligned(16))) char smem[];
   unsigned* mask = reinterpret_cast<unsigned*>(smem);
   const int t = threadIdx.x, lane = t & 63;
-  const int mtiles = e.g.mtiles;
-  const int units = e.centres * e.dirs * mtiles;
-  const int tsh = e.tws + e.ths;
-  const int tpr = (e.w + (1 << e.tws) - 1) >> e.tws;
-  const int side = 2 * e.radius + 2;
+  const ensure_kargs_t kargs = (ensure_kargs_t)__builtin_amdgcn_kernarg_segment_ptr();
+  const int mtiles = kargs->lv[0].g.mtiles;
+  const int units = kargs->centres * kargs->dirs * mtiles;
   for (int u = blockIdx.x; u < units; u += gridDim.x) {
+    ensure_kargs_t fresh = kargs;
+    asm volatile("" : "+s"(fresh));
+    const EnsureArgs& e = *(const EnsureArgs*)fresh;
+    const int tsh = e.tws + e.ths;
+    const int tpr = (e.w + (1 << e.tws) - 1) >> e.tws;
+    const int side = 2 * e.radius + 2;
+    const int ucells = 1 + 3 * e.nlev;
     const int k = u / mtiles, mt = u - k * mtiles;
     const int dir = k / e.centres, c = k - dir * e.centres;
-    const void* const* cell = e.cells + (dir * e.dir_cells + c) * 4;
-    const gu32ptr bitmap = (gu32ptr)uniform_cell(cell + 3) + mt * e.wpr;
-    lds_barrier();
-    if (t < ENSURE_MASK_WORDS) mask[t] = 0u;
-    lds_barrier();
+    const void* const* cell = e.cells + (dir * e.dir_cells + c) * ucells;
+    bool live = false;
+    float cx = 0.f, cy = 0.f;
     if (t < 128) {
       const int row = mt * 128 + t;
       const int tile = row >> tsh, in = row & ((1 << tsh) - 1);
       const int ty = tile / tpr, tx = tile - ty * tpr;
       const int y = (ty << e.ths) + (in >> e.tws), x = (tx << e.tws) + (in & ((1 << e.tws) - 1));
-      if (row < e.g.M && y < e.h && x < e.w) {
+      if (row < e.lv[0].g.M && y < e.h && x < e.w) {
         const gf32cptr cr = (gf32cptr)e.coords + ((int64_t)c * e.q_per_map + y * e.w + x) * e.ld_coords + dir * e.dir_coords;
-        const int x0 = window_origin(cr[0], e.radius);
-        const int y0 = window_origin(cr[1], e.radius);
-        const int xlo = max(x0, 0), xhi = min(x0 + side - 1, e.w - 1);
-        const int ylo = max(y0, 0), yhi = min(y0 + side - 1, e.h - 1);
+        live = true;
+        cx = cr[0];
+        cy = cr[1];
+      }
+    }
+    for (int i = 0; i < e.nlev; ++i) {
+      const EnsureLevel& lv = e.lv[i];
+      const int wpr = lv.wpr;
+      const gu32ptr bitmap = (gu32ptr)uniform_cell(cell + 3 + 3 * i) + mt * wpr;
+      lds_barrier();
+      if (t < ENSURE_MASK_WORDS) mask[t] = 0u;
+      lds_barrier();
+      if (live) {
+        const int x0 = window_origin(level_coord(cx, lv.level), e.radius);
+        const int y0 = window_origin(level_coord(cy, lv.level), e.radius);
+        const int xlo = max(x0, 0), xhi = min(x0 + side - 1, lv.w - 1);
+        const int ylo = max(y0, 0), yhi = min(y0 + side - 1, lv.h - 1);
         if (xlo <= xhi && ylo <= yhi) {
           for (int yy = ylo; yy <= yhi; yy = ((yy >> e.ths) + 1) << e.ths)
             for (int xx = xlo; xx <= xhi; xx = ((xx >> e.tws) + 1) << e.tws) {
-              const int ct = tiled_at(yy, xx, e.w, e.tws, e.ths) >> 6;
+              const int ct = tiled_at(yy, xx, lv.w, e.tws, e.ths) >> 6;
               atomicOr(&mask[ct >> 5], 1u << (ct & 31));
             }
         }
       }
+      lds_barrier();
+      if (t < wpr) mask[t] &= ~bitmap[t];
+      lds_barrier();
+      const unsigned need = lane < wpr ? mask[lane] : 0u;
+      const MaskCols cols{need, wpr};
+      int cnt = 0;
+      for (int w = 0; w < wpr; ++w) cnt += __builtin_popcount(cols.word(w));
+      if (cnt == 0) continue;
+
+      SplitArgs a = lv.g;
+      a.in0 = a.in1 = reinterpret_cast<const float*>(uniform_cell(cell));
+      a.wbase = reinterpret_cast<const char*>(uniform_cell(cell + 1 + 3 * i));
+      a.out = reinterpret_cast<float*>(const_cast<void*>(uniform_cell(cell + 2 + 3 * i)));
+      gemm_resident_unit<false, false>(a, smem, mt, cols);
+
+      asm volatile("s_waitcnt vmcnt(0)" ::: "memory");
+      lds_barrier();
+      if (t < wpr && need) atomicOr((unsigned*)bitmap + t, need);
+      if (t == 0 && e.counter) atomicAdd(e.counter + lv.level, (unsigned)cnt);
     }
-    lds_barrier();
-    if (t < e.wpr) mask[t] &= ~bitmap[t];
-    lds_barrier();
-    const unsigned need = lane < e.wpr ? mask[lane] : 0u;
-    const MaskCols cols{need, e.wpr};
-    int cnt = 0;
-    for (int w = 0; w < e.wpr; ++w) cnt += __builtin_popcount(cols.word(w));
-    if (cnt == 0) continue;
-
-    SplitArgs a = e.g;
-    a.in0 = a.in1 = reinterpret_cast<const float*>(uniform_cell(cell));
-    a.wbase = reinterpret_cast<const char*>(uniform_cell(cell + 1));
-    a.out = reinterpret_cast<float*>(const_cast<void*>(uniform_cell(cell + 2)));
-    gemm_resident_unit<false, false>(a, smem, mt, cols);
-
-    asm volatile("s_waitcnt vmcnt(0)" ::: "memory");
-    lds_barrier();
-    if (t < e.wpr && need) atomicOr((unsigned*)bitmap + t, need);
-    if (t == 0 && e.counter) atomicAdd(e.counter, (unsigned)cnt);
-  }
-}
-
+  }
+}
+
+int ensure_levels(const char* who, const vfml_corr_level_desc* lv, int nlev, int in_fmt, int k_order, const void* const* cells,
+                  int centres, int dirs, int dir_cells, const float* coords, int ld_coords, int dir_coords, int h, int w,
+                  int radius, int vol_tile, uint32_t* counter, void* stream) {
+  VFML_REQUIRE(nlev >= 1 && nlev <= ENSURE_MAX_LEVELS, "%s: one to %d levels", who, ENSURE_MAX_LEVELS);
+  EnsureArgs e;
+  e.tws = vol_tile & 15;
+  e.ths = vol_tile >> 4;
+  VFML_REQUIRE(vol_tile >= 0 && e.ths <= 6 && e.tws + e.ths <= 6, "%s: vol_tile: tiles of at most 64 texels", who);
+  VFML_REQUIRE(h > 0 && w > 0 && radius >= 1 && radius <= 4, "%s: empty level image, or radius outside 1..4", who);
+  const auto tiled_count = [&](int hh, int ww) {
+    return (int64_t)(((hh - 1) >> e.ths) + 1) * (((ww - 1) >> e.tws) + 1) << (e.tws + e.ths);
+  };
+  const int64_t rows = tiled_count(h, w);
+  for (int i = 0; i < nlev; ++i) {
+    EnsureLevel& l = e.lv[i];
+    VFML_REQUIRE(lv[i].d, "%s: null desc / cells / coords", who);
+    if (const int rc = vfml_detail::prepare_resident_gemm(lv[i].d, lv[i].w_hi, lv[i].w_lo, lv[i].kp, lv[i].w_scale, in_fmt,
+                                                          lv[i].out_fmt, k_order, who, &l.g))
+      return rc;
+    const SplitArgs& a = l.g;
+    VFML_REQUIRE(!a.bias && !a.out_t && a.epilogue == VFML_EPI_NONE && a.whi_off == 0 && a.d0off == 0 && a.tilebase,
+                 "%s: the level-0 call has no bias, twin or activation, its hi plane leads its planes and its rows are one "
+                 "split-row source", who);
+    VFML_REQUIRE(lv[i].level >= 0 && lv[i].level <= 7 && (i == 0 || lv[i].level > lv[i - 1].level) && lv[i].h > 0 && lv[i].w > 0,
+                 "%s: levels 0..7 in ascending order, no empty level image", who);
+    const int64_t tiled = tiled_count(lv[i].h, lv[i].w);
+    VFML_REQUIRE(rows == a.M, "%s: the call's rows (%d) must be the %lld positions of the tiled %d x %d query map", who, a.M,
+                 (long long)rows, h, w);
+    VFML_REQUIRE(tiled == a.cout, "%s: the call's columns (%d) must be the %lld positions of the tiled %d x %d level image", who,
+                 a.cout, (long long)tiled, lv[i].h, lv[i].w);
+    VFML_REQUIRE(i == 0 || (a.c0 == e.lv[0].g.c0 && a.ld0 == e.lv[0].g.ld0 && a.Kp == e.lv[0].g.Kp),
+                 "%s: every level's call has the same query rows", who);
+    l.h = lv[i].h; l.w = lv[i].w; l.level = lv[i].level;
+    l.wpr = (a.ntiles + 31) / 32;
+    VFML_REQUIRE(l.wpr <= ENSURE_MASK_WORDS, "%s: at most %d column tiles per volume row", who, ENSURE_MASK_WORDS * 32);
+  }
+  VFML_REQUIRE(centres >= 1 && (dirs == 1 || dirs == 2) && dir_cells >= (dirs == 2 ? centres : 0) && ld_coords >= 2 &&
+               dir_coords >= 0, "%s: centres >= 1, one or two directions, the second direction's cells behind the first's", who);
+  VFML_REQUIRE((reinterpret_cast<uintptr_t>(cells) & 7u) == 0 && (!counter || (reinterpret_cast<uintptr_t>(counter) & 3u) == 0),
+               "%s: cells are 8-byte aligned, the counter 4-byte", who);
+  for (int i = nlev; i < ENSURE_MAX_LEVELS; ++i) e.lv[i] = e.lv[0];
+  e.nlev = nlev;
+  e.cells = cells; e.coords = coords; e.counter = counter;
+  e.ld_coords = ld_coords; e.dir_coords = dir_coords;
+  e.centres = centres; e.dirs = dirs; e.dir_cells = dir_cells;
+  e.q_per_map = h * w; e.h = h; e.w = w; e.radius = radius;
+  if (const int rc = vfml_lds_cap(reinterpret_cast<const void*>(&corr_ensure_kernel), VFML_RESIDENT_LDS, who)) return rc;
+  const int64_t units = (int64_t)centres * dirs * e.lv[0].g.mtiles;
+  hipLaunchKernelGGL(corr_ensure_kernel, dim3((int)(units > 512 ? 512 : units)), dim3(256), VFML_RESIDENT_LDS,
+                     reinterpret_cast<hipStream_t>(stream), e);
+  return vfml_check_launch(who);
+}
+
+}
+
+extern "C" int vfml_corr_levels_ensure(const vfml_corr_level_desc* levels, int nlevels, int in_fmt, int k_order,
+                                       const void* const* cells, int centres, int dirs, int dir_cells, const float* coords,
+                                       int ld_coords, int dir_coords, int h, int w, int radius, int vol_tile,
+                                       uint32_t* counters, void* stream) {
+  const char* who = "vfml_corr_levels_ensure";
+  VFML_REQUIRE(levels && cells && coords, "%s: null levels / cells / coords", who);
+  return ensure_levels(who, levels, nlevels, in_fmt, k_order, cells, centres, dirs, dir_cells, coords, ld_coords, dir_coords,
+                       h, w, radius, vol_tile, counters, stream);
 }
 
 extern "C" int vfml_corr_level0_ensure(const vfml_conv_desc* d, const void* w_hi, const void* w_lo, int kp, float w_scale,
@@ -114,32 +204,7 @@
                                        int radius, int vol_tile, uint32_t* counter, void* stream) {
   const char* who = "vfml_corr_level0_ensure";
   VFML_REQUIRE(d && cells && coords, "%s: null desc / cells / coords", who);
-  EnsureArgs e;
-  if (const int rc = vfml_detail::prepare_resident_gemm(d, w_hi, w_lo, kp, w_scale, in_fmt, out_fmt, k_order, who, &e.g)) return rc;
-  const SplitArgs& a = e.g;
-  VFML_REQUIRE(!a.bias && !a.out_t && a.epilogue == VFML_EPI_NONE && a.whi_off == 0 && a.d0off == 0 && a.tilebase,
-               "%s: the level-0 call has no bias, twin or activation, its hi plane leads its planes and its rows are one "
-               "split-row source", who);
-  e.tws = vol_tile & 15;
-  e.ths = vol_tile >> 4;
-  VFML_REQUIRE(vol_tile >= 0 && e.ths <= 6 && e.tws + e.ths <= 6, "%s: vol_tile: tiles of at most 64 texels", who);
-  VFML_REQUIRE(h > 0 && w > 0 && radius >= 1 && radius <= 4, "%s: empty level image, or radius outside 1..4", who);
-  const int64_t tiled = (int64_t)(((h - 1) >> e.ths) + 1) * (((w - 1) >> e.tws) + 1) << (e.tws + e.ths);
-  VFML_REQUIRE(tiled == a.M && tiled == a.cout, "%s: the call's rows (%d) and columns (%d) must be the %lld positions of the "
-               "tiled %d x %d level image", who, a.M, a.cout, (long long)tiled, h, w);
-  e.wpr = (a.ntiles + 31) / 32;
-  VFML_REQUIRE(e.wpr <= ENSURE_MASK_WORDS, "%s: at most %d column tiles per volume row", who, ENSURE_MASK_WORDS * 32);
-  VFML_REQUIRE(centres >= 1 && (dirs == 1 || dirs == 2) && dir_cells >= (dirs == 2 ? centres : 0) && ld_coords >= 2 &&
-               dir_coords >= 0, "%s: centres >= 1, one or two directions, the second direction's cells behind the first's", who);
-  VFML_REQUIRE((reinterpret_cast<uintptr_t>(cells) & 7u) == 0 && (!counter || (reinterpret_cast<uintptr_t>(counter) & 3u) == 0),
-               "%s: cells are 8-byte aligned, the counter 4-byte", who);
-  e.cells = cells; e.coords = coords; e.counter = counter;
-  e.ld_coords = ld_coords; e.dir_coords = dir_coords;
-  e.centres = centres; e.dirs = dirs; e.dir_cells = dir_cells;
-  e.q_per_map = h * w; e.h = h; e.w = w; e.radius = radius;
-  if (const int rc = vfml_lds_cap(reinterpret_cast<const void*>(&corr_ensure_kernel), VFML_RESIDENT_LDS, who)) return rc;
-  const int64_t units = (int64_t)centres * dirs * a.mtiles;
-  hipLaunchKernelGGL(corr_ensure_kernel, dim3((int)(units > 512 ? 512 : units)), dim3(256), VFML_RESIDENT_LDS,
-                     reinterpret_cast<hipStream_t>(stream), e);
-  return vfml_check_launch(who);
-}
+  const vfml_corr_level_desc lv = {d, w_hi, w_lo, kp, w_scale, out_fmt, 0, h, w};
+  return ensure_levels(who, &lv, 1, in_fmt, k_order, cells, centres, dirs, dir_cells, coords, ld_coords, dir_coords, h, w,
+                       radius, vol_tile, counter, stream);
+}
diff --git a/video-flow-ml_amd/vfml/csrc/corr_window.h b/video-flow-ml_amd/vfml/csrc/corr_window.h
--- a/video-flow-ml_amd/vfml/csrc/corr_window.h
+++ b/video-flow-ml_amd/vfml/csrc/corr_window.h
@@ -8,6 +8,10 @@
   return ((((y >> ths) * tpr + (x >> tws)) << (tws + ths)) + ((y & ((1 << ths) - 1)) << tws) + (x & ((1 << tws) - 1)));
 }
 
+__device__ __forceinline__ float level_coord(float c, int l) {
+  return c * __builtin_bit_cast(float, (127 - l) << 23);
+}
+
 __device__ __forceinline__ int window_origin(float c, int radius) {
   return (int)fminf(fmaxf(floorf(c), -65536.f), 65536.f) - radius;
 }
diff --git a/video-flow-ml_amd/vfml/csrc/flow_ops.hip b/video-flow-ml_amd/vfml/csrc/flow_ops.hip
--- a/video-flow-ml_amd/vfml/csrc/flow_ops.hip
+++ b/video-flow-ml_amd/vfml/csrc/flow_ops.hip
@@ -70,8 +70,7 @@
       const int l = e / psz;
       const int idx = e - l * psz;
       const int py = idx / side, px = idx - py * side;
-      const float inv = 1.0f / (float)(1 << l);
-      const float x = cx * inv, y = cy * inv;
+      const float x = level_coord(cx, l), y = level_coord(cy, l);
       const float fx0 = floorf(x), fy0 = floorf(y);
       const int x0 = window_origin(x, a.radius);
       const int y0 = window_origin(y, a.radius);
@@ -170,8 +169,7 @@
     const int ES = v16 ? 2 : 4;
     const char* base = reinterpret_cast<const char*>(pl[l]) + (int64_t)qrow * a.ld[ll] * ES;
     const int wl = a.wl[ll], hl = a.hl[ll];
-    const float inv = __builtin_bit_cast(float, (127 - l) << 23);
-    const float x = cx * inv, y = cy * inv;
+    const float x = level_coord(cx, l), y = level_coord(cy, l);
     const int x0 = window_origin(x, R);
     const int y0 = window_origin(y, R);
     auto texel = [&](int px, int py, bool in, float& out, bool& ok) {
@@ -203,8 +201,7 @@
   wave_lds_sync();
   if (lane < a.levels * WIN) {
     const int l = lane / WIN, i = lane - l * WIN;
-    const float inv = __builtin_bit_cast(float, (127 - l) << 23);
-    const float x = cx * inv, y = cy * inv;
+    const float x = level_coord(cx, l), y = level_coord(cy, l);
     const float fx = x - floorf(x), fy = y - floorf(y);
     const float wx0 = 1.f - fx, wy0 = 1.f - fy;
     const float w00 = wx0 * wy0, w10 = fx * wy0, w01 = wx0 * fy, w11 = fx * fy;
diff --git a/video-flow-ml_amd/vfml/hip.py b/video-flow-ml_amd/vfml/hip.py
--- a/video-flow-ml_amd/vfml/hip.py
+++ b/video-flow-ml_amd/vfml/hip.py
@@ -47,6 +47,11 @@
         ("proj_out", c_void_p), ("ld_proj", c_int32),
         ("addend_ind", c_void_p),
     ]
+
+
+class CorrLevelDesc(ctypes.Structure):
+    _fields_ = [("d", POINTER(ConvDesc)), ("w_hi", c_void_p), ("w_lo", c_void_p), ("kp", c_int32), ("w_scale", c_float),
+                ("out_fmt", c_int32), ("level", c_int32), ("h", c_int32), ("w", c_int32)]
 
 
 COMMON_FLAGS = ["-fno-slp-vectorize"]
@@ -151,6 +156,8 @@
     L.vfml_ptr_table_set.argtypes = [c_void_p, POINTER(c_void_p), c_int, c_void_p]
     L.vfml_corr_level0_ensure.argtypes = L.vfml_conv2d_split.argtypes[:5] + [c_int, c_int, c_int] + [
         c_void_p, c_int, c_int, c_int, c_void_p, c_int, c_int, c_int, c_int, c_int, c_int, c_void_p, c_void_p]
+    L.vfml_corr_levels_ensure.argtypes = [POINTER(CorrLevelDesc), c_int, c_int, c_int, c_void_p, c_int, c_int, c_int, c_void_p,
+                                          c_int, c_int, c_int, c_int, c_int, c_int, c_void_p, c_void_p]
     L.vfml_window_seed.argtypes = [c_void_p, c_int, c_int, c_int, c_void_p, c_int, c_int, c_int, c_int, c_void_p]
     L.vfml_tapsum3x3_update.argtypes = [c_void_p, c_int, c_void_p, c_int, c_int, c_int, c_int, ctypes.c_int64, c_void_p, c_void_p,
                                         c_int, c_void_p, c_int, c_int, c_void_p]
@@ -238,7 +245,7 @@
     "vfml_conv2d", "vfml_conv2d_split", "vfml_conv2d_variant", "vfml_conv2d_split_variant", "vfml_conv2d_split_variant_at", "vfml_split_f16", "vfml_to_s16", "vfml_softmax_rows_s16", "vfml_softmax_rows_f16", "vfml_attention_plane_workspace_bytes", "vfml_attention_plane_f16", "vfml_attention_bank_planes_f16", "vfml_axpy_f32", "vfml_dwconv2d", "vfml_gelu_rows", "vfml_layernorm_rows", "vfml_window_attention", "vfml_attention_shared_keys", "vfml_transpose_to_s16", "vfml_add_to_s16",
     "vfml_transpose_split_f16", "vfml_frames_to_nhwc4", "vfml_instnorm_workspace_bytes", "vfml_instnorm_stats",
     "vfml_instnorm_apply", "vfml_instnorm_finalize", "vfml_instnorm_finalize_workspace_bytes", "vfml_avgpool2x2", "vfml_corr_lookup", "vfml_corr_lookup_indirect", "vfml_corr_lookup_indirect_bidir",
-    "vfml_ptr_table_set", "vfml_corr_level0_ensure", "vfml_window_seed", "vfml_coords_update", "vfml_coords_init", "vfml_tapsum3x3", "vfml_tapsum3x3_update", "vfml_flow_rows7", "vfml_flow_half", "vfml_conv3x3_c64",
+    "vfml_ptr_table_set", "vfml_corr_level0_ensure", "vfml_corr_levels_ensure", "vfml_window_seed", "vfml_coords_update", "vfml_coords_init", "vfml_tapsum3x3", "vfml_tapsum3x3_update", "vfml_flow_rows7", "vfml_flow_half", "vfml_conv3x3_c64",
     "vfml_flow_forward_interpolate_workspace_bytes", "vfml_flow_forward_interpolate",
     "vfml_convex_upsample", "vfml_stem7x7s2", "vfml_stem7x7s2_chunks", "vfml_flow_lod", "vfml_flow_encode", "vfml_taa_blend", "vfml_flow_quality_map", "vfml_flow_correct_workspace_bytes", "vfml_flow_correct",
     "vfml_flow_colorize", "vfml_compose_frame", "vfml_flow_decode", "vfml_flow_diff_overlay", "vfml_text_draw",
@@ -608,12 +615,18 @@
                              _stream()), "vfml_to_s16")
 
 
+PTR_TABLE_MAX = 48
+
+
 def ptr_table_set(table, tensors):
     n = len(tensors)
     if not (table.is_cuda and table.dtype == torch.int64 and table.numel() >= n):
         raise ValueError("ptr_table_set: table must be an int64 device tensor with room for the pointers")
-    ptrs = (c_void_p * n)(*[t if isinstance(t, int) else t.data_ptr() for t in tensors])
-    _check(lib().vfml_ptr_table_set(c_void_p(table.data_ptr()), ptrs, n, _stream()), "vfml_ptr_table_set")
+    vals = [t if isinstance(t, int) else t.data_ptr() for t in tensors]
+    for at in range(0, n, PTR_TABLE_MAX):
+        part = vals[at:at + PTR_TABLE_MAX]
+        _check(lib().vfml_ptr_table_set(c_void_p(table.data_ptr() + 8 * at), (c_void_p * len(part))(*part), len(part), _stream()),
+               "vfml_ptr_table_set")
 
 
 def corr_bitmap_words(rows, cols):
@@ -641,6 +654,39 @@
                                          centres, ndirs, dir_cells, _ptr(_dev(coords), coords_off), ld_coords, dir_coords, h, w,
                                          radius, vol_tile, c_void_p(counter.data_ptr()) if counter is not None else None,
                                          _stream()), "vfml_corr_level0_ensure")
+
+
+def corr_levels_ensure(rows, c, n_rows, levels, out_scale, cells, centres, dirs, dir_cells, coords, coords_off, ld_coords,
+                       dir_coords, h, w, radius, vol_tile, counters=None, in_fmt=FMT_S16, mfma=1):
+    ndirs = 2 if dirs == 2 else 1
+    per = 1 + 3 * len(levels)
+    if not levels or any(not isinstance(lv[1], SplitWeight) or lv[1].lo is None for lv in levels):
+        raise ValueError("corr_levels_ensure: every level's target operand is a SplitWeight")
+    if not (cells.is_cuda and cells.dtype == torch.int64 and cells.numel() >= per * ((ndirs - 1) * dir_cells + centres)):
+        raise ValueError("corr_levels_ensure: cells must be an int64 device tensor, 1 + 3 per level for each direction and "
+                         "centre frame")
+    if counters is not None and not (counters.is_cuda and counters.dtype == torch.int32
+                                     and counters.numel() > max(lv[0] for lv in levels)):
+        raise ValueError("corr_levels_ensure: the counters are an int32 device tensor with a cell per pyramid level")
+    descs = (ConvDesc * len(levels))()
+    lvs = (CorrLevelDesc * len(levels))()
+    for i, (level, weight, volume, n_cols, ldo, hl, wl) in enumerate(levels):
+        d = descs[i]
+        d.in0, d.c0, d.ld0 = _ptr(_dev(rows)), c, c
+        d.n, d.h, d.w = 1, 1, n_rows
+        d.cout, d.kh, d.kw, d.stride, d.pad_h, d.pad_w = n_cols, 1, 1, 1, 0, 0
+        d.out, d.ldo = _ptr(_dev(volume)), ldo
+        d.epilogue, d.split, d.out_scale = EPI_NONE, 0, out_scale
+        d.flags = {3: 0, 2: CONV_MFMA2, 1: CONV_MFMA1}[mfma]
+        lv = lvs[i]
+        lv.d = ctypes.pointer(d)
+        lv.w_hi, lv.w_lo, lv.kp, lv.w_scale = weight.hi.data_ptr(), weight.lo.data_ptr(), weight.kp, weight.scale
+        lv.out_fmt, lv.level, lv.h, lv.w = FMT_F32, level, hl, wl
+    order = levels[0][1].order
+    _check(lib().vfml_corr_levels_ensure(lvs, len(levels), in_fmt, order, c_void_p(cells.data_ptr()), centres, ndirs, dir_cells,
+                                         _ptr(_dev(coords), coords_off), ld_coords, dir_coords, h, w, radius, vol_tile,
+                                         c_void_p(counters.data_ptr()) if counters is not None else None, _stream()),
+           "vfml_corr_levels_ensure")
 
 
 SEED_NONE, SEED_LOAD, SEED_STORE = 0, 1, 2
diff --git a/video-flow-ml_amd/vfml/network.py b/video-flow-ml_amd/vfml/network.py
--- a/video-flow-ml_amd/vfml/network.py
+++ b/video-flow-ml_amd/vfml/network.py
@@ -896,6 +896,7 @@
                                      VFl=VFl, ldl=ldl, psz=psz)
 
     corr_on_demand = True
+    corr_on_demand_levels = (1,)
 
     def _corr_scale(self, AF):
         scale = 1.0 / float(self.cfg.feat_dim) ** 0.5
@@ -909,29 +910,48 @@
                 and geo.VT is not None and geo.Pv == geo.Nl[0] and geo.VFl[0] == hip.FMT_F32 and self._nm("corr") == 1
                 and self.cfg.feat_dim <= 256 and 2 * (N - 2) <= 8 and (geo.Nl[0] + 63) // 64 <= 2048)
 
+    def _on_demand_levels(self, on_demand, geo):
+        if not on_demand:
+            return ()
+        more = [l for l in range(1, geo.L) if l in self.corr_on_demand_levels and geo.VFl[l] == hip.FMT_F32
+                and geo.Nl[l] >= 1024 and (geo.Nl[l] + 63) // 64 <= 2048]
+        return (0,) + tuple(more[:2])
+
+    @staticmethod
+    def _bitmap_sections(geo, levels):
+        at, n = {}, 0
+        for l in levels:
+            at[l] = n
+            n += hip.corr_bitmap_words(geo.Pv, geo.Nl[l])
+        return at, n
+
     @staticmethod
     def _pyramid_bitmap(pyr, L):
         return pyr[L].view(torch.int32)
 
-    def corr_tiles_computed(self, reset=True):
+    def corr_level_tiles_computed(self, reset=True):
         count = self._ws.get("ensure_count")
         if count is None:
-            return 0
-        n = int(count.item())
+            return [0, 0, 0, 0]
+        n = [int(v) for v in count.tolist()]
         if reset:
             count.zero_()
         return n
 
-    def _window_pyramids(self, feats, keys, N, geo, dev, on_demand=False):
+    def corr_tiles_computed(self, reset=True):
+        return self.corr_level_tiles_computed(reset)[0]
+
+    def _window_pyramids(self, feats, keys, N, geo, dev, od_levels=()):
         D, L = self.cfg.feat_dim, geo.L
         AF, VFl, Nl, Pv, ldl, psz = geo.AF, geo.VFl, geo.Nl, geo.Pv, geo.ldl, geo.psz
         scale = self._corr_scale(AF)
         lim = 2 * (N - 2) + 2
         pyrs = {"f": [], "b": []}
-        od = ("od",) if on_demand else ()
+        on_demand = bool(od_levels)
+        od = (tuple(od_levels), "od") if on_demand else ()
         if on_demand:
-            psz = psz + [hip.corr_bitmap_words(Pv, Nl[0])]
-        first = 1 if on_demand else 0
+            psz = psz + [self._bitmap_sections(geo, od_levels)[1]]
+        built = [l for l in range(L) if l not in od_levels]
         for c in range(1, N - 1):
             for d, tgt in (("f", c + 1), ("b", c - 1)):
                 pk = ("p", keys[c], keys[tgt]) + od if keys is not None else None
@@ -952,14 +972,14 @@
                         rev = self._pyramid_buffers(psz, dev, limit=lim)
                         self._cache_put("p", rk, rev, limit=lim)
                     cnm = self._nm("corr") if self._split() else 3
-                    for l in range(first, L):
+                    for l in built:
                         hip.conv2d(feats[c][0], D, D, 1, 1, Pv, feats[tgt][1][l], None, Nl[l], 1, 1, pyr[l],
                                    ldl[l], out_scale=scale, in_fmt=AF, out_fmt=VFl[l],
                                    swap_cross=(d == "b" and l == 0 and gemm_form and cnm == 3),
                                    out_t=rev[0] if dual and l == 0 else None, ld_out_t=ldl[0] if dual and l == 0 else 0,
                                    mfma=cnm)
                     if dual:
-                        for l in range(1, L):
+                        for l in built if on_demand else range(1, L):
                             hip.conv2d(feats[tgt][0], D, D, 1, 1, Pv, feats[c][1][l], None, Nl[l], 1, 1, rev[l],
                                        ldl[l], out_scale=scale, in_fmt=AF, out_fmt=VFl[l], mfma=cnm)
                     if on_demand:
@@ -968,17 +988,22 @@
                 pyrs[d].append(pyr)
         return pyrs
 
-    def _ensure_plan(self, pyrs, feats, N, geo, dev):
+    def _ensure_plan(self, pyrs, feats, N, geo, dev, od_levels):
         M = N - 2
-        cells = self._buf("ensure_cells", 64, dev, torch.int64)
+        cells = self._buf("ensure_cells", 128, dev, torch.int64)
+        at, _ = self._bitmap_sections(geo, od_levels)
         ptrs = []
         for d, step in (("f", 1), ("b", -1)):
             for i, c in enumerate(range(1, N - 1)):
                 pyr = pyrs[d][i]
-                ptrs += [feats[c][0], feats[c + step][1][0].hi, pyr[0], self._pyramid_bitmap(pyr, geo.L)]
+                bits = self._pyramid_bitmap(pyr, geo.L)
+                ptrs.append(feats[c][0])
+                for l in od_levels:
+                    ptrs += [feats[c + step][1][l].hi, pyr[l], bits.data_ptr() + 4 * at[l]]
         hip.ptr_table_set(cells, ptrs)
-        count = self._buf("ensure_count", 1, dev, torch.int32, zero=True)
-        return types.SimpleNamespace(cells=cells, M=M, rows=feats[1][0], weight=feats[2][1][0], level0=pyrs["f"][0][0],
+        count = self._buf("ensure_count", 4, dev, torch.int32, zero=True)
+        levels = [(l, feats[2][1][l], pyrs["f"][0][l], geo.Nl[l], geo.ldl[l], geo.hl[l], geo.wl[l]) for l in od_levels]
+        return types.SimpleNamespace(cells=cells, M=M, rows=feats[1][0], levels=levels, per=1 + 3 * len(od_levels),
                                      D=self.cfg.feat_dim, scale=self._corr_scale(geo.AF), counter=count)
 
     def _frame_features(self, src, sel, keys, H, W, P, dev, L, hl, wl, Sl, vt=None):
@@ -1235,7 +1260,8 @@
 
             feats = self._frame_features(src, list(range(N)), keys, H, W, P, dev, L, geo.hl, geo.wl, geo.Sl, vt=geo.VT)
             on_demand = self._level0_on_demand(keys, N, geo, dense_corr)
-            pyrs = self._window_pyramids(feats, keys, N, geo, dev, on_demand)
+            od_levels = self._on_demand_levels(on_demand, geo)
+            pyrs = self._window_pyramids(feats, keys, N, geo, dev, od_levels)
             s = self._window_state(P, dev, M, h, w, geo, R, AF, cor_p)
             ctx = self._frame_context(src, list(range(1, N - 1)), keys, H, W, P, dev, Pn, M)
             win = types.SimpleNamespace(M=M, dev=dev, att_slots=(), readout=None)
@@ -1249,7 +1275,7 @@
             win.gates = self._gate_addends(ctx, dev, Pn, M)
             win.sk_ws = self._sk_workspace(MP, dev) if self.sk else None
             win.tables, win.bidir = self._pyramid_tables(pyrs, dev, M, L, cor_p)
-            win.ensure = self._ensure_plan(pyrs, feats, N, geo, dev) if on_demand else None
+            win.ensure = self._ensure_plan(pyrs, feats, N, geo, dev, od_levels) if on_demand else None
             no, nflows = (1, 1) if short else (M, 2 * M)
             up_fixed = self._buf("up_out", nflows * H * W * 2, dev)
             mask = self._buf("mask", MP * 1152, dev)
@@ -1282,7 +1308,7 @@
                             hip.convex_upsample(s.coords1, c * Pn * 4, 2 * d, mask, c * Pn * 1152 + d * 576, 1152, h, w,
                                                 up_fixed, out_off=(d * M + c) * H * W * 2)
 
-            gkey = (H, W, N, M, bool(tri_batch), bool(pick_only), cfg.decoder_depth, L, R, self._plan_key(), geo.vol16,
+            gkey = (H, W, N, M, bool(tri_batch), bool(pick_only), cfg.decoder_depth, L, R, self._plan_key(), geo.vol16, od_levels,
                     self._packed_serial, str(dev), os.environ.get("VFML_FLOW_BRANCH", "0"), win.warm, win.att_slots, on_demand)
             if self.sk:
                 gkey += ("sk",)
diff --git a/video-flow-ml_amd/vfml/update_block.py b/video-flow-ml_amd/vfml/update_block.py
--- a/video-flow-ml_amd/vfml/update_block.py
+++ b/video-flow-ml_amd/vfml/update_block.py
@@ -36,8 +36,8 @@
 def ensure_level0(s, n, r0, en):
     g = s.geo
     c0 = r0 // s.Pn
-    hip.corr_level0_ensure(en.rows, en.D, en.weight, en.level0, g.Pv, g.Nl[0], g.ldl[0], en.scale, en.cells[4 * c0:], n, 2,
-                           en.M, s.coords1, r0 * 4, 4, 2, g.hl[0], g.wl[0], s.R, g.TILE, counter=en.counter, in_fmt=s.AF)
+    hip.corr_levels_ensure(en.rows, en.D, g.Pv, en.levels, en.scale, en.cells[en.per * c0:], n, 2, en.M, s.coords1, r0 * 4, 4, 2,
+                           g.hl[0], g.wl[0], s.R, g.TILE, counters=en.counter, in_fmt=s.AF)
 
 
 def convc1(s, n, r0):
```
